# quadram-institute-bioscience/tatajuba

Hardware: AMD Instinct MI355X
Metric: reads/s (whole node), 150 bp synthetic FASTQ, homopolymer scan + context histogram (higher is better)
Workload: dtype u8/u64

## Files before the change

tatajuba_amd/csrc/hopo_device.hip:

```cpp

#include <hip/hip_runtime.h>
#include <rccl/rccl.h>
#include <dlfcn.h>
#include <mutex>
#include <string>
#include <new>
#include <stdint.h>
#include <stdio.h>
#include <stdlib.h>
#include <string.h>
#include <stdarg.h>
#include <limits.h>
#include <float.h>
#include <algorithm>
#include <vector>

#include "../../include/tatajuba_amd.h"
#include "../../include/tatajuba_variants.h"
#include "../../include/tatajuba_features.h"

typedef unsigned long long u64;
typedef unsigned int u32;


static thread_local char g_err[512] = "";

static int set_err (int code, const char *fmt, ...)
{
  va_list ap;
  va_start (ap, fmt);
  vsnprintf (g_err, sizeof (g_err), fmt, ap);
  va_end (ap);
  return code;
}

#define HIPCHK(call) do { hipError_t e_ = (call); if (e_ != hipSuccess) \
  return set_err (TJAMD_ERR_HIP, "%s failed: %s (%s:%d)", #call, hipGetErrorString (e_), __FILE__, __LINE__); } while (0)
#define HIPCHK_NULL(call) do { hipError_t e_ = (call); if (e_ != hipSuccess) { \
  set_err (TJAMD_ERR_HIP, "%s failed: %s (%s:%d)", #call, hipGetErrorString (e_), __FILE__, __LINE__); return NULL; } } while (0)

extern "C" const char *tjamd_last_error (void) { return g_err; }
extern "C" void tj_set_last_error (const char *msg) { (void) set_err (TJAMD_ERR_ARG, "%s", msg ? msg : "error"); }

extern "C" int tjamd_device_count (void)
{
  int n = 0;
  if (hipGetDeviceCount (&n) != hipSuccess) return 0;
  return n;
}


#define TJ_HL      64
#define TJ_HR      192

template <int BLOCK, int TILE, int CANDDIV = 2>
struct TileLds
{
  static constexpr int WIN = TJ_HL + TILE + TJ_HR;
  static constexpr int NCHUNK = WIN / 16;
  static constexpr int MASKW = WIN / 32 + 4;
  static constexpr int CODEW = WIN / 16 + 4;
  static constexpr int MAXCAND = TILE / CANDDIV;
  static constexpr int NLOAD = (NCHUNK + BLOCK - 1) / BLOCK;
  static constexpr int NRAW = NCHUNK + NLOAD * (BLOCK / 64);
  u32 code[CODEW];
  u32 start[MASKW];
  u32 sent[MASKW];
  u32 inval[MASKW];
  unsigned short cand[MAXCAND];
  u32 ncand;
  u32 grp[2];
  u32 odd[2];
};

struct DevCounters
{
  u64 n_rec;
  u64 n_fix_unused;
  u64 n_undefined;
  u64 n_null;
  u32 overflow;
  u32 fix_overflow;
  u32 pad[2];
  struct { u64 n_fix; u32 work, n_slow, work_slow, ticket, pad[2]; } lc[2];
};

#define TJ_TILE_GROUP 16

struct FixEntry { long long pos; long long len; };

struct FinCounts { u32 n_seg, n_kept, n_ctx, n_idx; int coverage; u32 overflow, sort_fallback, pad; };
struct FinPlan { long n1; long t; int nbits, nbins, log2t, ok; u32 kept_overflow, cov_direct; long n1_exact; u32 ovf_exact, pad2; };



__device__ __forceinline__ u32 zero_bytes (u32 t)
{
  return ~(((t & 0x7F7F7F7Fu) + 0x7F7F7F7Fu) | t | 0x7F7F7F7Fu);
}

__device__ __forceinline__ u32 gather_bit7 (u32 z)
{
  return ((z >> 7) | (z >> 14) | (z >> 21) | (z >> 28)) & 0xFu;
}

__device__ __forceinline__ void classify_word (u32 x, u32 prev_byte, u32 &code8, u32 &start4, u32 &sent4, u32 &inval4)
{
  u32 a1 = x >> 1, a2 = x >> 2, a3 = x >> 3, a4 = x >> 4, a6 = x >> 6, a7 = x >> 7;
  u32 v = ~a7 & a6 & ~a3 & ((~a4 & x & ~(a2 & ~a1)) | (a4 & a2 & ~a1));
  v &= 0x01010101u;
  u32 c = (a1 ^ a2) & (v * 3u);
  code8 = (c | (c >> 6) | (c >> 12) | (c >> 18)) & 0xFFu;
  u32 iv = v ^ 0x01010101u;
  inval4 = (iv | (iv >> 7) | (iv >> 14) | (iv >> 21)) & 0xFu;
  sent4 = gather_bit7 (zero_bytes (x ^ 0x0A0A0A0Au));
  start4 = gather_bit7 (zero_bytes (x ^ ((x << 8) | prev_byte))) ^ 0xFu;
}

__device__ __forceinline__ void classify_word_fast (u32 x, u32 prev_word, bool hi, u32 &code8, u32 &start4, u32 &sent4, u32 &bad)
{
  const u32 wts = hi ? 0x80402010u : 0x08040201u;
  const u32 c = ((x >> 1) ^ (x >> 2)) & 0x03030303u;
  code8 = __builtin_amdgcn_udot4 (c, 0x40100401u, 0u, false);
  const u32 s = ~(x >> 6) & 0x01010101u;
  sent4 = __builtin_amdgcn_udot4 (s, wts, sent4, false);
  bad = x ^ __builtin_amdgcn_perm (0x0A0A0A0Au, 0x54474341u, c | (s << 2));
  const u32 d = x ^ __builtin_amdgcn_alignbit (x, prev_word, 24);
  const u32 nz = (((d & 0x7F7F7F7Fu) + 0x7F7F7F7Fu) | d) & 0x80808080u;
  start4 = __builtin_amdgcn_udot4 (nz, wts, start4, false);
}

__device__ __forceinline__ u32 wave_inclusive_scan (u32 x)
{
  x += (u32) __builtin_amdgcn_update_dpp (0, (int) x, 0x111, 0xF, 0xF, true);
  x += (u32) __builtin_amdgcn_update_dpp (0, (int) x, 0x112, 0xF, 0xF, true);
  x += (u32) __builtin_amdgcn_update_dpp (0, (int) x, 0x114, 0xF, 0xF, true);
  x += (u32) __builtin_amdgcn_update_dpp (0, (int) x, 0x118, 0xF, 0xF, true);
  x += (u32) __builtin_amdgcn_update_dpp (0, (int) x, 0x142, 0xA, 0xF, true);
  x += (u32) __builtin_amdgcn_update_dpp (0, (int) x, 0x143, 0xC, 0xF, true);
  return x;
}

__device__ __forceinline__ void lds_barrier ()
{
  asm volatile ("s_waitcnt lgkmcnt(0)\n\ts_barrier" ::: "memory");
}

typedef __attribute__((address_space(1))) const void *gptr_t;
typedef __attribute__((address_space(3))) void *lptr_t;
__device__ __forceinline__ void lds_add_issue (u32 lds_addr, u32 value_uniform, u32 &raw_out)
{
  u64 saved; u32 tmp;
  asm volatile ("s_mov_b64 %0, exec\n\ts_mov_b64 exec, 1\n\tv_mov_b32 %1, %4\n\tds_add_rtn_u32 %2, %3, %1\n\ts_mov_b64 exec, %0"
                : "=&s"(saved), "=&v"(tmp), "=&v"(raw_out) : "v"(lds_addr), "s"(value_uniform) : "memory");
}
__device__ __forceinline__ u32 lds_collect (u32 raw)
{
  asm volatile ("s_waitcnt lgkmcnt(0)" : "+v"(raw) :: "memory");
  return (u32) __builtin_amdgcn_readfirstlane ((int) raw);
}

__device__ __forceinline__ u64 bits64 (const u32 *a, int bitpos)
{
  int w = bitpos >> 5, sh = bitpos & 31;
  u32 x0 = a[w], x1 = a[w + 1], x2 = a[w + 2];
  u32 lo = __funnelshift_r (x0, x1, sh);
  u32 hi = __funnelshift_r (x1, x2, sh);
  return ((u64) hi << 32) | lo;
}

__device__ __forceinline__ u32 bits32 (const u32 *a, int bitpos)
{
  const int w = bitpos >> 5;
  return __builtin_amdgcn_alignbit (a[w + 1], a[w], (u32) bitpos & 31u);
}

__device__ __forceinline__ u32 revcomp_k32 (u32 x, int k)
{
  const u32 y = __brev (~x);
  u32 z;
  asm ("v_bfi_b32 %0, %1, %2, %3" : "=v"(z) : "s"(0x55555555u), "v"(y >> 1), "v"(y << 1));
  return z >> (32 - 2 * k);
}

__device__ __forceinline__ u64 kmask (int k) { return (k >= 32) ? ~0ull : ((1ull << (2 * k)) - 1ull); }

__device__ __forceinline__ u64 revcomp_k (u64 x, int k)
{
  const u64 y = __brevll (~x);
  const u32 lo = (u32) y, hi = (u32) (y >> 32);
  u32 zl, zh;
  asm ("v_bfi_b32 %0, %1, %2, %3" : "=v"(zl) : "s"(0x55555555u), "v"(lo >> 1), "v"(lo << 1));
  asm ("v_bfi_b32 %0, %1, %2, %3" : "=v"(zh) : "s"(0x55555555u), "v"(hi >> 1), "v"(hi << 1));
  return (((u64) zh << 32) | zl) >> (64 - 2 * k);
}

__device__ __forceinline__ u32 stream_byte (const uint8_t *seq, long n, long p)
{
  return (p >= 0 && p < n) ? (u32) seq[p] : (u32) '\n';
}

__device__ __forceinline__ bool byte_is_acgtu (u32 b)
{
  u32 l = b | 0x20u;
  return l == 'a' || l == 'c' || l == 'g' || l == 't' || l == 'u';
}

__device__ __forceinline__ u32 byte_code (u32 b) { return byte_is_acgtu (b) ? (((b >> 1) ^ (b >> 2)) & 3u) : 0u; }

__device__ __forceinline__ u64 spread_pairs (u32 x)
{
  u64 v = x;
  v = (v | (v << 16)) & 0x0000FFFF0000FFFFull;
  v = (v | (v << 8)) & 0x00FF00FF00FF00FFull;
  v = (v | (v << 4)) & 0x0F0F0F0F0F0F0F0Full;
  v = (v | (v << 2)) & 0x3333333333333333ull;
  v = (v | (v << 1)) & 0x5555555555555555ull;
  return v | (v << 1);
}

__device__ __forceinline__ void canonicalise (u64 left, u64 right, u32 linv, u32 rinv, u32 cb, int k,
                                              u64 &c0, u64 &c1, u32 &base, u32 &flag)
{
  if (cb < 2u) { c0 = left; c1 = right; base = cb; flag = 1u; }
  else {
    if (linv | rinv) { left |= spread_pairs (linv); right |= spread_pairs (rinv); }
    c0 = revcomp_k (right, k); c1 = revcomp_k (left, k); base = 3u - cb; flag = 2u;
  }
}

__device__ __forceinline__ u64 make_meta (u32 base, long len, u32 flag)
{
  return (u64) base | (((u64) len & 0x3FFull) << TJ_META_LEN_SHIFT) | TJ_META_RAW_CONST | ((u64) flag << TJ_META_FLAG_SHIFT);
}

__device__ bool flanks_from_stream (const uint8_t *seq, long n, long gs, long ge, int k, u64 &left, u64 &right, u32 &linv, u32 &rinv)
{
  left = right = 0; linv = rinv = 0;
  for (int i = 0; i < k; i++) {
    u32 bl = stream_byte (seq, n, gs - k + i), br = stream_byte (seq, n, ge + 1 + i);
    if (bl == '\n' || br == '\n') return false;
    left |= (u64) byte_code (bl) << (2 * i);
    right |= (u64) byte_code (br) << (2 * i);
    linv |= (byte_is_acgtu (bl) ? 0u : 1u) << i;
    rinv |= (byte_is_acgtu (br) ? 0u : 1u) << i;
// ... 1391 lines not shown
  static_assert (RR % 4 == 0, "bins are kept four to a register");
  const u32 tid = threadIdx.x, lane = tid & 63u;
  const u32 wave = (u32) __builtin_amdgcn_readfirstlane ((int) (tid >> 6));
  if (tid < TJ_P) L.hist[tid] = 0;
  u32 cur_j = TJ_EMPTY, cur_chunk = TJ_NOCHUNK;
  lds_barrier ();
  const u32 n_blocks = min (*LG.next, LG.n_blocks);
  u32 b = blockIdx.x;
  if (b >= n_blocks) return;
  u64 w[RR][W];
  u32 n = min (LG.count[b], RB), nn = 0;
  auto load_block = [&] (u32 blk, u32 cnt) {
    const u64 *__restrict__ src = LG.log + ((u64) blk << TJ_LOGB_SHIFT);
    const u32 w0 = tid & ~63u;
#pragma unroll
    for (u32 r = 0; r < RR; r++) {
#pragma unroll
      for (int j = 0; j < W; j++) w[r][j] = 0;
      if (w0 + r * PL_BLOCK < cnt) {
        if constexpr (W == 1) w[r][0] = (src + r * PL_BLOCK)[tid];
        else { const ulonglong2 v = reinterpret_cast<const ulonglong2 *> (src + 2u * r * PL_BLOCK)[tid]; w[r][0] = v.x; w[r][1] = v.y; }
      }
    }
  };
  auto bucket_of = [&] (const u64 *rec) -> u32 {
    if constexpr (W == 1) return bucket_of_rec1 ((u32) rec[0], (u32) (rec[0] >> 32));
    else { u64 c0, c1; u32 base, len10, flag; unpack_raw<W> (rec, k, c0, c1, base, len10, flag); return bucket_of_key (c0, c1, base, len10); }
  };
  load_block (b, n);
  while (true) {
    const u32 bn = b + gridDim.x;
    const bool more = bn < n_blocks;
    if (more) nn = min (LG.count[bn], RB);
    u32 tq = tid;
    asm volatile ("" : "+v"(tq));
    u32 pk[RR / 4];
#pragma unroll
    for (u32 r = 0; r < RR / 4; r++) pk[r] = 0;
    if (n) {
#pragma unroll
      for (u32 r = 0; r < RR; r++) {
        const u32 bin = bucket_of (w[r]);
        pk[r >> 2] |= bin << (8u * (r & 3u));
        if (tid + r * PL_BLOCK < n) atomicAdd (&L.hist[bin], 1u);
      }
      lds_barrier ();
      if (wave < TJ_P / 64) {
        const uint4 h4 = *reinterpret_cast<const uint4 *> (&L.hist[4 * lane]);
        const u32 tot = h4.x + h4.y + h4.z + h4.w;
        const u32 e0 = wave_inclusive_scan (tot) - tot;
        if ((lane >> 4) == wave) *reinterpret_cast<uint4 *> (&L.offs[4 * lane]) = make_uint4 (e0, e0 + h4.x, e0 + h4.x + h4.y, e0 + h4.x + h4.y + h4.z);
        const u32 cnt = L.hist[tid], off = L.offs[tid];
        u64 a1 = 0, a2 = 0;
        u32 thr = off + cnt;
        if (cnt) {
          const u32 p0 = atomicAdd (&BK.cursors[tid * TJ_CSTRIDE], cnt);
          const u32 ch = (u32) TJ_CH0 << BK.ch_shift;
          bucket_claim_ahead_range (BK, tid, p0, cnt, ctr);
          const u32 j0 = chunk_of_pos (BK, p0), j1 = chunk_of_pos (BK, p0 + cnt - 1);
          if (j0 != cur_j) { cur_j = j0; cur_chunk = bucket_chunk_id (BK, tid, j0, true, ctr); }
          if (cur_chunk != TJ_NOCHUNK) a1 = (u64) (size_t) (BK.pool + ((u64) cur_chunk * ch + (p0 - j0 * ch)) * W) - (8ull * W) * off;
          if (j1 != j0) {
            thr = off + ((j0 + 1u) * ch - p0);
            cur_j = j0 + 1u; cur_chunk = bucket_chunk_id (BK, tid, j0 + 1u, true, ctr);
            if (cur_chunk != TJ_NOCHUNK) a2 = (u64) (size_t) (BK.pool + ((u64) cur_chunk * ch) * W) - (8ull * W) * thr;
          }
        }
        reinterpret_cast<uint4 *> (L.gbase)[tid] = make_uint4 ((u32) a1, (u32) (a1 >> 32) | (thr << 16), (u32) a2, (u32) (a2 >> 32));
      }
      lds_barrier ();
      if (tid < TJ_P) L.hist[tid] = 0;
#pragma unroll
      for (u32 r = 0; r < RR; r++)
        if (tid + r * PL_BLOCK < n) {
          const u32 bin = (pk[r >> 2] >> (8u * (r & 3u))) & 255u;
          const u32 d = atomicAdd (&L.offs[bin], 1u);
#pragma unroll
          for (int j = 0; j < W; j++) L.rec[d * W + j] = w[r][j];
          L.bin[d] = (unsigned char) bin;
        }
      lds_barrier ();
      for (u32 r0 = 0; r0 < RR; r0 += 4) {
        if (r0 * PL_BLOCK >= n) break;
        u32 cb[4]; uint4 e[4]; u64 cw[4][W];
#pragma unroll
        for (u32 h = 0; h < 4; h++) cb[h] = L.bin[tq + (r0 + h) * PL_BLOCK];
#pragma unroll
        for (u32 h = 0; h < 4; h++) {
          e[h] = reinterpret_cast<const uint4 *> (L.gbase)[cb[h]];
#pragma unroll
          for (int j = 0; j < W; j++) cw[h][j] = L.rec[(tq + (r0 + h) * PL_BLOCK) * W + j];
        }
#pragma unroll
        for (u32 h = 0; h < 4; h++) {
          const u32 i = tq + (r0 + h) * PL_BLOCK;
          const u64 a = (i < (e[h].y >> 16)) ? (((u64) (e[h].y & 0xFFFFu) << 32) | e[h].x) : (((u64) e[h].w << 32) | e[h].z);
          if (i < n && a != 0ull) {
            typedef __attribute__((address_space(1))) u64 *gwords_t;
            gwords_t q = (gwords_t) (a + (u64) (8u * W * i));
#pragma unroll
            for (int j = 0; j < W; j++) q[j] = cw[h][j];
          }
        }
      }
      lds_barrier ();
    }
    if (!more) break;
    load_block (bn, nn);
    n = nn; b = bn;
  }
}

template <int W>
__global__ void nrun_fixup_bins_kernel (const uint8_t *__restrict__ seq, long n_bytes, int k, int mprime,
                                        Buckets BK, DevCounters *ctr, const FixEntry *fix, u32 fix_cap, int par)
{
  nrun_fixup_entries<W> (seq, n_bytes, k, mprime, BK, ctr, fix, fix_cap, par, blockIdx.x * (u64) blockDim.x + threadIdx.x, (u64) gridDim.x * blockDim.x);
}

template <int W>
__global__ void bin_elems_kernel (const u64 *__restrict__ elems5, long n, int k, Buckets BK, DevCounters *ctr)
{
  for (long i = blockIdx.x * (long) blockDim.x + threadIdx.x; i < n; i += (long) gridDim.x * blockDim.x) {
    const u64 m = elems5[5 * i + 2];
    bucket_insert_slow<W> (elems5[5 * i], elems5[5 * i + 1], (u32) (m & 3ull), (u32) ((m >> TJ_META_LEN_SHIFT) & 0x3FFull),
                           (u32) ((m >> TJ_META_FLAG_SHIFT) & 3ull), k, BK, ctr);
  }
}

template <int W>
__global__ void unpack_buckets_kernel (Buckets BK, int k, u64 *__restrict__ out, u64 cap, u64 *n_out)
{
  const u32 b = blockIdx.x;
  const u32 n = BK.cursors[b * TJ_CSTRIDE];
  for (u32 i = threadIdx.x; i < n; i += blockDim.x) {
    u64 c0, c1; u32 base, len10, flag;
    const u64 at = bucket_slot (BK, b, i, false, nullptr);
    if (at == ~0ull) continue;
    unpack_raw<W> (BK.pool + at * W, k, c0, c1, base, len10, flag);
    if (flag == 3u) continue;
    const u64 o = atomicAdd (n_out, 1ull);
    if (o < cap) { u64 *q = out + 3 * o; q[0] = c0; q[1] = c1; q[2] = make_meta (base, len10, flag); }
  }
}

__global__ void init_table_kernel (u32 *table, u32 maxj, u32 *pool_next)
{
  const u32 b = blockIdx.x * blockDim.x + threadIdx.x;
  if (b < TJ_P) table[(u64) b * maxj] = b;
  if (b == 0) *pool_next = TJ_P;
}

__global__ void clear_buckets_kernel (u32 *cursors, DevCounters *ctr, u32 *table, u32 maxj, int ch_shift, FinCounts *fin, u32 *bins, int nbins,
                                      DevCounters *snap_ctr, u32 *snap_cursors, FinPlan *plan, u32 *__restrict__ fine = nullptr, int fine_bits = 0)
{
  const u32 b = blockIdx.x;
  if (snap_ctr) {
    if (threadIdx.x == 0) {
      snap_cursors[b] = cursors[b * TJ_CSTRIDE];
      if (b == 0) {
        snap_cursors[TJ_P] = cursors[TJ_P * TJ_CSTRIDE];
        if (plan) { plan->n1_exact = (long) fin->n_kept; plan->ovf_exact = fin->overflow; }
      }
    }
    if (b == 0) for (u32 i = threadIdx.x; i < sizeof (DevCounters) / 4; i += blockDim.x) reinterpret_cast<u32 *> (snap_ctr)[i] = reinterpret_cast<const u32 *> (ctr)[i];
    __syncthreads ();
  }
  if (b == 0) for (u32 i = threadIdx.x; i < sizeof (DevCounters) / 4; i += blockDim.x) if (i != offsetof (DevCounters, n_undefined) / 4 && i != offsetof (DevCounters, n_undefined) / 4 + 1) reinterpret_cast<u32 *> (ctr)[i] = 0;
  if (table) {
    u32 used = maxj;
    if (ch_shift >= 0) used = min (maxj, ((cursors[b * TJ_CSTRIDE] / TJ_CH0) >> ch_shift) + 3u);
    for (u32 j = threadIdx.x; j < used; j += blockDim.x) table[(u64) b * maxj + j] = j ? TJ_EMPTY : b;
  }
  if (fine) {
    const int gid = (int) (b * blockDim.x + threadIdx.x), gsz = (int) (gridDim.x * blockDim.x);
    if (plan->ok) {
      const int shift = fine_bits - plan->nbits, run = 1 << shift, nb = plan->nbins;
      for (int i = gid; i < nb; i += gsz) {
        u32 sum = 0;
        if (shift >= 2) {
          uint4 *f4 = reinterpret_cast<uint4 *> (fine) + (size_t) i * (run >> 2);
          for (int j = 0; j < (run >> 2); j++) { const uint4 v = f4[j]; sum += v.x + v.y + v.z + v.w; }
          for (int j = 0; j < (run >> 2); j++) f4[j] = make_uint4 (0, 0, 0, 0);
        }
        else {
          for (int j = 0; j < run; j++) sum += fine[(i << shift) + j];
          for (int j = 0; j < run; j++) fine[(i << shift) + j] = 0;
        }
        bins[i] = sum;
      }
    }
    else for (int i = gid; i < (1 << fine_bits); i += gsz) fine[i] = 0;
  }
  else if (bins) for (int i = (int) (b * blockDim.x + threadIdx.x); i < nbins; i += (int) (gridDim.x * blockDim.x)) bins[i] = 0;
  __syncthreads ();
  if (threadIdx.x == 0) { cursors[b * TJ_CSTRIDE] = 0; if (b == 0) { cursors[TJ_P * TJ_CSTRIDE] = TJ_P; fin->n_kept = 0; fin->overflow = 0; fin->pad = 0; } }
}

__global__ void table_relayout_kernel (const u32 *__restrict__ old, u32 old_maxj, u32 *__restrict__ neu, u32 new_maxj)
{
  const u32 b = blockIdx.x;
  for (u32 j = threadIdx.x; j < old_maxj; j += blockDim.x) neu[(u64) b * new_maxj + j] = old[(u64) b * old_maxj + j];
}


#define AG_BLOCK    1024
#define AG_NCH      512

#define AG1_S        8192
#define AG1_CLOSE_AT 4864
#define AG1_R        4
#define AG1_MARK     (~0ull)

#define BS_MAXBITS   16
__host__ __device__ static inline int cov_table_bits (long n1) { int b = 10; while ((1l << b) < 4 * n1 && b < 31) b++; return b; }
__host__ __device__ static inline int cov_plan_bits (long n1, int k, int *direct)
{
  const int hb = cov_table_bits (n1), kb = 2 * k < 31 ? 2 * k : 31;
  *direct = kb <= hb ? 1 : 0;
  return kb <= hb ? kb : hb;
}
__host__ __device__ static inline int fine_bin_bits (int k) { return BS_MAXBITS < 1 + 4 * k ? BS_MAXBITS : 1 + 4 * k; }
__device__ __forceinline__ u32 bin_of_record (u64 c0, u64 c1, u64 meta, int k, int nbits);
__host__ __device__ static inline int bin_bits_for (long n1, int k)
{
  int nbits = 6;
  while (nbits < BS_MAXBITS && nbits < 1 + 4 * k && (48l << nbits) < n1) nbits++;
  return nbits < 1 + 4 * k ? nbits : 1 + 4 * k;
}
__device__ __forceinline__ void flag_kept_overflow (FinCounts *fin)
{
  u32 old = atomicOr (&fin->overflow, 1u);
  asm volatile ("" :: "v"(old));
}

__device__ __forceinline__ void plan_tail (FinCounts *fin, int k, long cap, FinPlan *plan)
{
  if (!plan) return;
  __syncthreads ();
  if (threadIdx.x == 0) {
    const u32 done = atomicAdd (&fin->pad, 1u);
    if (done == gridDim.x - 1u) {
      const long n1 = (long) __hip_atomic_load (&fin->n_kept, __ATOMIC_RELAXED, __HIP_MEMORY_SCOPE_AGENT);
      const u32 ovf = __hip_atomic_load (&fin->overflow, __ATOMIC_RELAXED, __HIP_MEMORY_SCOPE_AGENT);
      plan->n1 = n1; plan->kept_overflow = ovf;
      plan->nbits = bin_bits_for (n1, k); plan->nbins = 1 << plan->nbits;
      int direct;
      plan->log2t = cov_plan_bits (n1, k, &direct); plan->t = 1l << plan->log2t; plan->cov_direct = (u32) direct;
      plan->ok = (n1 > 0 && n1 <= cap && !ovf) ? 1 : 0;
      fin->pad = 0;
    }
  }
}

__device__ __forceinline__ u32 batch_start (u32 t, u32 n, u32 batch)
{
  const u32 nb = (n + batch - 1u) / batch;
  return t < nb ? (nb - 1u - t) * batch : n;
}

struct Agg1Lds
{
  u64 key[AG1_S];
  u32 cnt[2 * AG1_S];
  u32 chunk[AG_NCH];
  u32 n_claimed, n_ovf, total;
  u32 next_batch;
  u32 wsum[AG_BLOCK / 64];
};

__global__ __launch_bounds__ (AG_BLOCK)
void aggregate1_kernel (Buckets BK, u64 *ovf, int k, int remove_biased, u64 *__restrict__ kept, u64 kept_cap, FinCounts *fin,
                        long plan_cap, FinPlan *plan, u32 *__restrict__ fine, int fine_bits)
{
  __shared__ Agg1Lds L;
  const int tid = threadIdx.x, lane = tid & 63, wave = tid >> 6;
  const u32 bkt = blockIdx.x;
  u32 n = BK.cursors[bkt * TJ_CSTRIDE];
  if (n) for (u32 j = (u32) tid; j <= chunk_of_pos (BK, n - 1u) && j < AG_NCH; j += AG_BLOCK) L.chunk[j] = bucket_chunk_id (BK, bkt, j, false, nullptr);
  auto chunk_id = [&] (u32 j) { return j < AG_NCH ? L.chunk[j] : bucket_chunk_id (BK, bkt, j, false, nullptr); };

  const u64 *src = BK.pool;
  u64 *dst = ovf;
  while (n > 0) {
    for (int i = tid; i < AG1_S; i += AG_BLOCK) { L.key[i] = 0; L.cnt[2 * i] = 0; L.cnt[2 * i + 1] = 0; }
    if (tid == 0) { L.n_claimed = 0; L.n_ovf = 0; L.next_batch = 0; }
    __syncthreads ();

    u64 wn[AG1_R];
    u32 vn = 0;
    auto fetch = [&] (u32 b0) {
      vn = 0;
#pragma unroll
      for (int r = 0; r < AG1_R; r++) wn[r] = 0;
      if (b0 >= n) return;
      const u32 ch = (u32) TJ_CH0 << BK.ch_shift;
      const u32 j0 = chunk_of_pos (BK, b0), bound = (j0 + 1u) * ch;
      if (b0 + 64u * AG1_R <= min (n, bound) && j0 < AG_NCH) {
        const u32 c0s = (u32) __builtin_amdgcn_readfirstlane ((int) L.chunk[j0]);
        if (c0s != TJ_NOCHUNK) {
          const u64 *q = src + ((u64) c0s * ch + (b0 - j0 * ch)) + (u32) lane;
#pragma unroll
          for (int r = 0; r < AG1_R; r++) wn[r] = q[64 * r];
          vn = (1u << AG1_R) - 1u;
          return;
        }
      }
      const u32 c0 = chunk_id (j0), c1 = (bound < n) ? chunk_id (j0 + 1u) : TJ_NOCHUNK;
      const u64 off0 = (u64) c0 * ch - (u64) j0 * ch, off1 = (u64) c1 * ch - (u64) bound;
#pragma unroll
      for (int r = 0; r < AG1_R; r++) {
        const u32 idx = b0 + (u32) r * 64u + (u32) lane;
        const bool hi = idx >= bound;
        if (idx < n && (hi ? c1 : c0) != TJ_NOCHUNK) { vn |= 1u << r; wn[r] = src[(hi ? off1 : off0) + idx]; }
      }
    };
    auto next_batch = [&] () {
      u32 b = 0;
      if (lane == 0) b = atomicAdd (&L.next_batch, 1u);
      return batch_start ((u32) __builtin_amdgcn_readfirstlane ((int) b), n, 64u * AG1_R);
    };
    u32 b_next = next_batch ();
    fetch (b_next);
    while (b_next < n) {
      const u32 b0 = b_next;
      (void) b0;
      asm volatile ("s_waitcnt vmcnt(0)" : "+v"(wn[0]), "+v"(wn[1]), "+v"(wn[2]), "+v"(wn[3]) :: "memory");
      static_assert (AG1_R == 4, "asm operand list");
      u64 w[AG1_R];
#pragma unroll
      for (int r = 0; r < AG1_R; r++) w[r] = wn[r];
      const u32 valid = vn;
      b_next = next_batch ();
      fetch (b_next);
      {
        auto home = [] (u64 key) {
          u32 h = (u32) key ^ __builtin_amdgcn_alignbit ((u32) (key >> 32), (u32) (key >> 32), 17);
          h *= 0x9E3779B1u; h ^= h >> 15;
          return h & (AG1_S / 2 - 1);
        };
        u32 todo = 0;
        u32 hp[AG1_R];
        ulonglong2 hk[AG1_R];
#pragma unroll
        for (int r = 0; r < AG1_R; r++) {
          hp[r] = home (w[r] & R1_KEY_MASK);
          hk[r] = *reinterpret_cast<const ulonglong2 *> (&L.key[2 * hp[r]]);
        }
        asm volatile ("" : "+v"(hk[0].x), "+v"(hk[0].y), "+v"(hk[1].x), "+v"(hk[1].y), "+v"(hk[2].x), "+v"(hk[2].y), "+v"(hk[3].x), "+v"(hk[3].y));
#pragma unroll
        for (int r = 0; r < AG1_R; r++) {
          const u64 cur = w[r];
          if (((valid >> r) & 1u) && ((cur >> R1_FLAG_SHIFT) & 3ull) != 3ull) {
            const u64 key = cur & R1_KEY_MASK;
            const bool hx = hk[r].x == key, hy = hk[r].y == key;
            if (hx | hy) atomicAdd (&L.cnt[4 * hp[r] + (hx ? 0u : 2u) + ((u32) (cur >> (R1_FLAG_SHIFT + 1)) & 1u)], 1u);
            else todo |= 1u << r;
          }
        }
        u32 probes = 0;
        u32 r = todo ? (u32) __ffs ((int) todo) - 1u : 0u;
        u64 cur = (r == 0u) ? w[0] : (r == 1u) ? w[1] : (r == 2u) ? w[2] : w[3];
        u32 pair = home (cur & R1_KEY_MASK);
        while (todo) {
          bool adv = false, left = false;
          {
            const u64 key = cur & R1_KEY_MASK;
            const u32 strand = (u32) (cur >> (R1_FLAG_SHIFT + 1)) & 1u;
            const ulonglong2 kk = *reinterpret_cast<const ulonglong2 *> (&L.key[2 * pair]);
            if (kk.x == key || kk.y == key) { atomicAdd (&L.cnt[4 * pair + (kk.x == key ? 0u : 2u) + strand], 1u); adv = true; }
            else {
              const bool e0 = (kk.x == 0ull) | (kk.x == AG1_MARK), e1 = (kk.y == 0ull) | (kk.y == AG1_MARK);
              if (e0 | e1) {
                const u32 slot = 2 * pair + (e0 ? 0u : 1u);
                if ((e0 ? kk.x : kk.y) == AG1_MARK) { left = true; adv = true; }
                else {
                  const bool closed = __hip_atomic_load (&L.n_claimed, __ATOMIC_RELAXED, __HIP_MEMORY_SCOPE_WORKGROUP) > AG1_CLOSE_AT;
                  const u64 old = atomicCAS ((unsigned long long *) &L.key[slot], 0ull, closed ? AG1_MARK : (unsigned long long) key);
                  if (old == 0ull) {
                    if (closed) left = true;
                    else { atomicAdd (&L.n_claimed, 1u); atomicAdd (&L.cnt[2 * slot + strand], 1u); }
                    adv = true;
                  }
                }
              }
              else if (++probes >= AG1_S / 2) { left = true; adv = true; }
              else pair = (pair + 1u) & (AG1_S / 2 - 1);
            }
          }
          if (left) {
            const u32 o = atomicAdd (&L.n_ovf, 1u);
            const u32 j = chunk_of_pos (BK, o), oc = chunk_id (j);
            if (oc != TJ_NOCHUNK) dst[(((u64) oc * TJ_CH0) << BK.ch_shift) + (o - ((j * TJ_CH0) << BK.ch_shift))] = cur;
          }
          if (adv) {
            todo &= todo - 1u; probes = 0;
            if (todo) {
              r = (u32) __ffs ((int) todo) - 1u;
              cur = (r == 1u) ? w[1] : (r == 2u) ? w[2] : w[3];
              pair = home (cur & R1_KEY_MASK);
            }
          }
        }
      }
    }
    __syncthreads ();

    u32 mine = 0;
    u64 metas[AG1_S / AG_BLOCK];
#pragma unroll
    for (int r = 0; r < AG1_S / AG_BLOCK; r++) {
      const int slot = tid + r * AG_BLOCK;
      metas[r] = 0;
      if (L.key[slot] && L.key[slot] != AG1_MARK) {
        const u32 cf = L.cnt[2 * slot], cr = L.cnt[2 * slot + 1];
        const u64 flag = (cf ? 1ull : 0ull) | (cr ? 2ull : 0ull);
        const u64 cnt = ((u64) cf + (u64) cr) & 0xFFFFFull;
        const int scnt = (cnt & 0x80000ull) ? (int) cnt - 0x100000 : (int) cnt;
        if (remove_biased ? (flag == 3ull) : (scnt > 1)) {
          const u64 key = L.key[slot];
          const u64 len10 = ((key >> 24) & 0xFFull) | (((key >> 56) & 3ull) << 8);
          metas[r] = ((key >> 58) & 1ull) | (len10 << TJ_META_LEN_SHIFT) | (cnt << TJ_META_COUNT_SHIFT) |
                     (0xffeull << TJ_META_MISM_SHIFT) | (flag << TJ_META_FLAG_SHIFT);
          mine++;
        }
      }
    }
    const u32 x = wave_inclusive_scan (mine);
    if (lane == 63) L.wsum[wave] = x;
    __syncthreads ();
    u32 wbase = 0, total = 0;
    for (int wv = 0; wv < AG_BLOCK / 64; wv++) { const u32 sm = L.wsum[wv]; if (wv < wave) wbase += sm; total += sm; }
    if (tid == 0) L.total = total ? atomicAdd (&fin->n_kept, total) : 0u;
    __syncthreads ();
    u64 at = (u64) L.total + wbase + x - mine;
#pragma unroll
    for (int r = 0; r < AG1_S / AG_BLOCK; r++)
      if (metas[r]) {
        const u64 key = L.key[tid + r * AG_BLOCK];
        if (at < kept_cap) {
          u64 *q = kept + 3 * at; q[0] = (key >> 32) & 0xFFFFFFull; q[1] = key & 0xFFFFFFull; q[2] = metas[r];
          if (fine) atomicAdd (&fine[bin_of_record ((key >> 32) & 0xFFFFFFull, key & 0xFFFFFFull, metas[r], k, fine_bits)], 1u);
        }
        else flag_kept_overflow (fin);
        at++;
      }
    __threadfence_block ();
    __syncthreads ();
    n = L.n_ovf;
    { const u64 *t = src; src = dst; dst = (u64 *) t; }
    __syncthreads ();
  }
  plan_tail (fin, k, plan_cap, plan);
}

#define AG2_S        6144
#define AG2_PAIRS    (AG2_S / 2)
#define AG2_CLOSE_AT 2560
#define AG2_R        4
#define AG2_VALID    (1ull << 63)
#define AG2_PENDING  (1ull << 63)
#define AG2_MARK     (1ull << 63)

struct Agg2Lds
{
  ulonglong2 kk[AG2_S];
  u32 cnt[2 * AG2_S];
  u32 chunk[AG_NCH];
  u32 n_claimed, n_ovf, total;
  u32 next_batch;
  u32 wsum[AG_BLOCK / 64];
};

__global__ __launch_bounds__ (AG_BLOCK)
void aggregate2_kernel (Buckets BK, u64 *ovf, int k, int remove_biased, u64 *__restrict__ kept, u64 kept_cap, FinCounts *fin,
                        long plan_cap, FinPlan *plan, u32 *__restrict__ fine, int fine_bits)
{
  __shared__ Agg2Lds L;
  const int tid = threadIdx.x, lane = tid & 63, wave = tid >> 6;
  const u32 bkt = blockIdx.x;
  u32 n = BK.cursors[bkt * TJ_CSTRIDE];
  const u64 m56 = (1ull << 56) - 1ull, fmask = ~(3ull << 61);
  if (n) for (u32 j = (u32) tid; j <= chunk_of_pos (BK, n - 1u) && j < AG_NCH; j += AG_BLOCK) L.chunk[j] = bucket_chunk_id (BK, bkt, j, false, nullptr);
  auto chunk_id = [&] (u32 j) { return j < AG_NCH ? L.chunk[j] : bucket_chunk_id (BK, bkt, j, false, nullptr); };
  const u64 *src = BK.pool;
  u64 *dst = ovf;

  while (n > 0) {
    for (int i = tid; i < AG2_S; i += AG_BLOCK) { L.kk[i] = make_ulonglong2 (0ull, 0ull); L.cnt[2 * i] = 0; L.cnt[2 * i + 1] = 0; }
    if (tid == 0) { L.n_claimed = 0; L.n_ovf = 0; L.next_batch = 0; }
    __syncthreads ();

    u64 wn[2 * AG2_R];
    u32 vn = 0;
    auto fetch = [&] (u32 b0) {
      vn = 0;
#pragma unroll
      for (int r = 0; r < 2 * AG2_R; r++) wn[r] = 0;
      if (b0 >= n) return;
      const u32 ch = (u32) TJ_CH0 << BK.ch_shift;
      const u32 j0 = chunk_of_pos (BK, b0), bound = (j0 + 1u) * ch;
      const u32 c0 = chunk_id (j0), c1 = (bound < n) ? chunk_id (j0 + 1u) : TJ_NOCHUNK;
      const u64 off0 = (u64) c0 * ch - (u64) j0 * ch, off1 = (u64) c1 * ch - (u64) bound;
#pragma unroll
      for (int r = 0; r < AG2_R; r++) {
        const u32 idx = b0 + (u32) r * 64u + (u32) lane;
        const bool hi = idx >= bound;
        if (idx < n && (hi ? c1 : c0) != TJ_NOCHUNK) {
          const ulonglong2 v = *reinterpret_cast<const ulonglong2 *> (src + 2 * ((hi ? off1 : off0) + idx));
          vn |= 1u << r; wn[2 * r] = v.x; wn[2 * r + 1] = v.y;
        }
      }
    };
    auto next_batch = [&] () {
      u32 b = 0;
      if (lane == 0) b = atomicAdd (&L.next_batch, 1u);
      return batch_start ((u32) __builtin_amdgcn_readfirstlane ((int) b), n, 64u * AG2_R);
    };
    u32 b_next = next_batch ();
    fetch (b_next);
    while (b_next < n) {
      asm volatile ("s_waitcnt vmcnt(0)" : "+v"(wn[0]), "+v"(wn[1]), "+v"(wn[2]), "+v"(wn[3]), "+v"(wn[4]), "+v"(wn[5]), "+v"(wn[6]), "+v"(wn[7]) :: "memory");
      static_assert (AG2_R == 4, "asm operand list");
      u64 w[2 * AG2_R];
#pragma unroll
      for (int r = 0; r < 2 * AG2_R; r++) w[r] = wn[r];
      const u32 valid = vn;
      b_next = next_batch ();
      fetch (b_next);
      {
        auto home = [] (u64 a, u64 b) {
          const u64 key1 = b & ~(3ull << 61);
          u32 h = (u32) a ^ __builtin_amdgcn_alignbit ((u32) (a >> 32), (u32) (a >> 32), 19) ^
                  __builtin_amdgcn_alignbit ((u32) key1, (u32) key1, 11) ^ __builtin_amdgcn_alignbit ((u32) (key1 >> 32), (u32) (key1 >> 32), 25);
          h *= 0x9E3779B1u; h ^= h >> 15;
          return __umulhi (h, (u32) AG2_PAIRS);
        };
        auto load_pair = [&] (u32 pair, ulonglong2 &s0, ulonglong2 &s1) {
          s0.x = __hip_atomic_load ((unsigned long long *) &L.kk[2 * pair].x, __ATOMIC_RELAXED, __HIP_MEMORY_SCOPE_WORKGROUP);
          s0.y = __hip_atomic_load ((unsigned long long *) &L.kk[2 * pair].y, __ATOMIC_RELAXED, __HIP_MEMORY_SCOPE_WORKGROUP);
          s1.x = __hip_atomic_load ((unsigned long long *) &L.kk[2 * pair + 1].x, __ATOMIC_RELAXED, __HIP_MEMORY_SCOPE_WORKGROUP);
          s1.y = __hip_atomic_load ((unsigned long long *) &L.kk[2 * pair + 1].y, __ATOMIC_RELAXED, __HIP_MEMORY_SCOPE_WORKGROUP);
        };
        u32 todo = 0, look = 0, cur[AG2_R];
#pragma unroll
        for (int q = 0; q < AG2_R; q++) {
          cur[q] = 0;
          if (((valid >> q) & 1u) && ((w[2 * q + 1] >> 61) & 3ull) != 3ull) { look |= 1u << q; cur[q] = home (w[2 * q], w[2 * q + 1]); }
        }
#pragma unroll
        for (int pass = 0; pass < 3; pass++) {
          if (pass && !look) break;
#pragma unroll
          for (int q = 0; q < AG2_R; q++)
            if ((look >> q) & 1u) {
              const u64 a0 = w[2 * q], a1 = w[2 * q + 1];
              ulonglong2 s0, s1;
              load_pair (cur[q], s0, s1);
              const u64 want = (a1 & fmask) | AG2_VALID;
              const bool m0 = (s0.x == a0) & (s0.y == want), m1 = (s1.x == a0) & (s1.y == want);
              if (m0 | m1) { atomicAdd (&L.cnt[2 * (2 * cur[q] + (m0 ? 0u : 1u)) + ((u32) (a1 >> 62) & 1u)], 1u); look &= ~(1u << q); }
              else {
                const u64 mine = a0 | AG2_PENDING;
                const bool o0 = (s0.x != 0ull) & (s0.x != AG2_MARK) & (s0.x != mine) & ((s0.x & AG2_PENDING) == 0ull) & ((s0.x != a0) | ((s0.y & AG2_VALID) != 0ull));
                const bool o1 = (s1.x != 0ull) & (s1.x != AG2_MARK) & (s1.x != mine) & ((s1.x & AG2_PENDING) == 0ull) & ((s1.x != a0) | ((s1.y & AG2_VALID) != 0ull));
                if (o0 & o1) cur[q] = (cur[q] + 1u == (u32) AG2_PAIRS) ? 0u : cur[q] + 1u;
                else { look &= ~(1u << q); todo |= 1u << q; }
              }
            }
        }
        todo |= look;
        u32 probes = 0;
        u32 r = todo ? (u32) __ffs ((int) todo) - 1u : 0u;
        u64 w0 = (r == 0u) ? w[0] : (r == 1u) ? w[2] : (r == 2u) ? w[4] : w[6];
        u64 w1 = (r == 0u) ? w[1] : (r == 1u) ? w[3] : (r == 2u) ? w[5] : w[7];
        u32 pair = (r == 0u) ? cur[0] : (r == 1u) ? cur[1] : (r == 2u) ? cur[2] : cur[3];
        while (todo) {
          bool adv = false, left = false;
          {
            const u64 key1 = w1 & fmask, want = key1 | AG2_VALID;
            const u32 strand = (u32) (w1 >> 62) & 1u;
            ulonglong2 s0, s1;
            load_pair (pair, s0, s1);
            const bool m0 = (s0.x == w0) & (s0.y == want), m1 = (s1.x == w0) & (s1.y == want);
            const bool again = (s0.x == (w0 | AG2_PENDING)) | (s1.x == (w0 | AG2_PENDING)) |
                               ((s0.x == w0) & !(s0.y & AG2_VALID)) | ((s1.x == w0) & !(s1.y & AG2_VALID));
            if (m0 | m1) { atomicAdd (&L.cnt[2 * (2 * pair + (m0 ? 0u : 1u)) + strand], 1u); adv = true; }
            else if (!again) {
              const bool e0 = (s0.x == 0ull) | (s0.x == AG2_MARK), e1 = (s1.x == 0ull) | (s1.x == AG2_MARK);
              if (e0 | e1) {
                const u32 slot = 2 * pair + (e0 ? 0u : 1u);
                if ((e0 ? s0.x : s1.x) == AG2_MARK) { left = true; adv = true; }
                else {
                  const bool closed = __hip_atomic_load (&L.n_claimed, __ATOMIC_RELAXED, __HIP_MEMORY_SCOPE_WORKGROUP) > AG2_CLOSE_AT;
                  const u64 old = atomicCAS ((unsigned long long *) &L.kk[slot].x, 0ull, closed ? AG2_MARK : (unsigned long long) (w0 | AG2_PENDING));
                  if (old == 0ull) {
                    if (closed) left = true;
                    else {
                      __hip_atomic_store ((unsigned long long *) &L.kk[slot].y, (unsigned long long) want, __ATOMIC_RELAXED, __HIP_MEMORY_SCOPE_WORKGROUP);
                      atomicAdd (&L.n_claimed, 1u);
                      __hip_atomic_store ((unsigned long long *) &L.kk[slot].x, (unsigned long long) w0, __ATOMIC_RELEASE, __HIP_MEMORY_SCOPE_WORKGROUP);
                      atomicAdd (&L.cnt[2 * slot + strand], 1u);
                    }
                    adv = true;
                  }
                }
              }
              else if (++probes >= AG2_PAIRS) { left = true; adv = true; }
              else pair = (pair + 1u == (u32) AG2_PAIRS) ? 0u : pair + 1u;
            }
          }
          if (left) {
            const u32 o = atomicAdd (&L.n_ovf, 1u);
            const u32 j = chunk_of_pos (BK, o), oc = chunk_id (j);
            if (oc != TJ_NOCHUNK) {
              const u64 at = (((u64) oc * TJ_CH0) << BK.ch_shift) + (o - ((j * TJ_CH0) << BK.ch_shift));
              dst[2 * at] = w0; dst[2 * at + 1] = w1;
            }
          }
          if (adv) {
            todo &= todo - 1u; probes = 0;
            if (todo) {
              r = (u32) __ffs ((int) todo) - 1u;
              w0 = (r == 1u) ? w[2] : (r == 2u) ? w[4] : w[6];
              w1 = (r == 1u) ? w[3] : (r == 2u) ? w[5] : w[7];
              pair = (r == 1u) ? cur[1] : (r == 2u) ? cur[2] : cur[3];
            }
          }
        }
      }
    }
    __syncthreads ();

    u32 mine = 0;
    u64 metas[AG2_S / AG_BLOCK];
#pragma unroll
    for (int r = 0; r < AG2_S / AG_BLOCK; r++) {
      const int slot = tid + r * AG_BLOCK;
      metas[r] = 0;
      if (L.kk[slot].x && L.kk[slot].x != AG2_MARK) {
        const u32 cf = L.cnt[2 * slot], cr = L.cnt[2 * slot + 1];
        const u64 flag = (cf ? 1ull : 0ull) | (cr ? 2ull : 0ull);
        const u64 cnt = ((u64) cf + (u64) cr) & 0xFFFFFull;
        const int scnt = (cnt & 0x80000ull) ? (int) cnt - 0x100000 : (int) cnt;
        if (remove_biased ? (flag == 3ull) : (scnt > 1)) {
          const u64 a = L.kk[slot].x, b = L.kk[slot].y;
          const u64 len10 = ((a >> 2) & 31ull) | (((b >> 56) & 31ull) << 5);
          metas[r] = ((a >> 1) & 1ull) | (len10 << TJ_META_LEN_SHIFT) | (cnt << TJ_META_COUNT_SHIFT) |
                     (0xffeull << TJ_META_MISM_SHIFT) | (flag << TJ_META_FLAG_SHIFT);
          mine++;
        }
      }
    }
    const u32 x = wave_inclusive_scan (mine);
    if (lane == 63) L.wsum[wave] = x;
    __syncthreads ();
    u32 wbase = 0, total = 0;
    for (int wv = 0; wv < AG_BLOCK / 64; wv++) { const u32 sm = L.wsum[wv]; if (wv < wave) wbase += sm; total += sm; }
    if (tid == 0) L.total = total ? atomicAdd (&fin->n_kept, total) : 0u;
    __syncthreads ();
    u64 at = (u64) L.total + wbase + x - mine;
#pragma unroll
    for (int r = 0; r < AG2_S / AG_BLOCK; r++)
      if (metas[r]) {
        const int slot = tid + r * AG_BLOCK;
        if (at < kept_cap) {
          u64 *q = kept + 3 * at; q[0] = (L.kk[slot].x >> 7) & m56; q[1] = L.kk[slot].y & m56; q[2] = metas[r];
          if (fine) atomicAdd (&fine[bin_of_record ((L.kk[slot].x >> 7) & m56, L.kk[slot].y & m56, metas[r], k, fine_bits)], 1u);
        }
        else flag_kept_overflow (fin);
        at++;
      }
    __threadfence_block ();
    __syncthreads ();
    n = L.n_ovf;
    { const u64 *t = src; src = dst; dst = (u64 *) t; }
    __syncthreads ();
  }
  plan_tail (fin, k, plan_cap, plan);
}

#define AG4_S        4096
#define AG4_CLOSE_AT 2560
#define AG4_R        2
#define AG4_PENDING  (1ull << 63)
#define AG4_MARK     (1ull << 63)

struct Agg4Lds
{
  u64 cw[AG4_S], c0[AG4_S], c1[AG4_S];
  u32 cnt[2 * AG4_S];
  u32 chunk[AG_NCH];
  u32 n_claimed, n_ovf, total;
  u32 next_batch;
  u32 wsum[AG_BLOCK / 64];
};

__global__ __launch_bounds__ (AG_BLOCK)
void aggregate4_kernel (Buckets BK, u64 *ovf, int k, int remove_biased, u64 *__restrict__ kept, u64 kept_cap, FinCounts *fin,
                        long plan_cap, FinPlan *plan, u32 *__restrict__ fine, int fine_bits)
{
  __shared__ Agg4Lds L;
  const int tid = threadIdx.x, lane = tid & 63, wave = tid >> 6;
  const u32 bkt = blockIdx.x;
  u32 n = BK.cursors[bkt * TJ_CSTRIDE];
  if (n) for (u32 j = (u32) tid; j <= chunk_of_pos (BK, n - 1u) && j < AG_NCH; j += AG_BLOCK) L.chunk[j] = bucket_chunk_id (BK, bkt, j, false, nullptr);
  auto chunk_id = [&] (u32 j) { return j < AG_NCH ? L.chunk[j] : bucket_chunk_id (BK, bkt, j, false, nullptr); };
  const u64 *src = BK.pool;
  u64 *dst = ovf;
  auto ld = [] (u64 *p) { return (u64) __hip_atomic_load ((unsigned long long *) p, __ATOMIC_RELAXED, __HIP_MEMORY_SCOPE_WORKGROUP); };

  while (n > 0) {
    for (int i = tid; i < AG4_S; i += AG_BLOCK) { L.cw[i] = 0; L.c0[i] = 0; L.c1[i] = 0; L.cnt[2 * i] = 0; L.cnt[2 * i + 1] = 0; }
    if (tid == 0) { L.n_claimed = 0; L.n_ovf = 0; L.next_batch = 0; }
    __syncthreads ();

    u64 wn[3 * AG4_R];
    u32 vn = 0;
    auto fetch = [&] (u32 b0) {
      vn = 0;
#pragma unroll
      for (int r = 0; r < 3 * AG4_R; r++) wn[r] = 0;
      if (b0 >= n) return;
      const u32 ch = (u32) TJ_CH0 << BK.ch_shift;
      const u32 j0 = chunk_of_pos (BK, b0), bound = (j0 + 1u) * ch;
      const u32 c0 = chunk_id (j0), c1 = (bound < n) ? chunk_id (j0 + 1u) : TJ_NOCHUNK;
      const u64 off0 = (u64) c0 * ch - (u64) j0 * ch, off1 = (u64) c1 * ch - (u64) bound;
#pragma unroll
      for (int r = 0; r < AG4_R; r++) {
        const u32 idx = b0 + (u32) r * 64u + (u32) lane;
        const bool hi = idx >= bound;
        if (idx < n && (hi ? c1 : c0) != TJ_NOCHUNK) {
          const u64 *p = src + 4 * ((hi ? off1 : off0) + idx);
          const ulonglong2 v = *reinterpret_cast<const ulonglong2 *> (p);
          vn |= 1u << r; wn[3 * r] = v.x; wn[3 * r + 1] = v.y; wn[3 * r + 2] = p[2];
        }
      }
    };
    auto next_batch = [&] () {
      u32 b = 0;
      if (lane == 0) b = atomicAdd (&L.next_batch, 1u);
      return batch_start ((u32) __builtin_amdgcn_readfirstlane ((int) b), n, 64u * AG4_R);
    };
    u32 b_next = next_batch ();
    fetch (b_next);
    while (b_next < n) {
      asm volatile ("s_waitcnt vmcnt(0)" : "+v"(wn[0]), "+v"(wn[1]), "+v"(wn[2]), "+v"(wn[3]), "+v"(wn[4]), "+v"(wn[5]) :: "memory");
      static_assert (AG4_R == 2, "asm operand list");
      u64 w[3 * AG4_R];
#pragma unroll
      for (int r = 0; r < 3 * AG4_R; r++) w[r] = wn[r];
      const u32 valid = vn;
      b_next = next_batch ();
      fetch (b_next);
      u32 todo = 0;
#pragma unroll
      for (int q = 0; q < AG4_R; q++) if (((valid >> q) & 1u) && ((w[3 * q + 2] >> 12) & 3ull) != 3ull) todo |= 1u << q;
      u32 probes = 0;
      while (todo) {
        const u32 r = (u32) __ffs ((int) todo) - 1u;
        const u64 c0 = r ? w[3] : w[0], c1 = r ? w[4] : w[1], m2 = r ? w[5] : w[2];
        const u32 k2 = (u32) m2 & 0xFFFu, strand = (u32) (m2 >> 13) & 1u;
        const u64 hk = hash_key (c0, c1, k2 & 3u, k2 >> 2);
        const u64 cw = 1ull | ((u64) k2 << 1) | ((hk >> 14) << 13);
        u32 slot = ((u32) hk + probes) & (AG4_S - 1);
        bool adv = false, left = false;
        const u64 a = ld (&L.cw[slot]);
        u64 x0 = ld (&L.c0[slot]), x1 = ld (&L.c1[slot]);
        if (a == cw) {
          bool eq = (x0 == c0) & (x1 == c1);
          if (!eq || (c0 | c1) == 0ull) { x0 = ld (&L.c0[slot]); x1 = ld (&L.c1[slot]); eq = (x0 == c0) & (x1 == c1); }
          if (eq) { atomicAdd (&L.cnt[2 * slot + strand], 1u); adv = true; }
          else if (++probes >= AG4_S) { left = true; adv = true; }
        }
        else if (a == AG4_MARK) { left = true; adv = true; }
        else if (a == 0ull) {
          const bool closed = __hip_atomic_load (&L.n_claimed, __ATOMIC_RELAXED, __HIP_MEMORY_SCOPE_WORKGROUP) > AG4_CLOSE_AT;
          const u64 old = atomicCAS ((unsigned long long *) &L.cw[slot], 0ull, closed ? AG4_MARK : (unsigned long long) (cw | AG4_PENDING));
          if (old == 0ull) {
            if (closed) left = true;
            else {
              __hip_atomic_store ((unsigned long long *) &L.c0[slot], (unsigned long long) c0, __ATOMIC_RELAXED, __HIP_MEMORY_SCOPE_WORKGROUP);
              __hip_atomic_store ((unsigned long long *) &L.c1[slot], (unsigned long long) c1, __ATOMIC_RELAXED, __HIP_MEMORY_SCOPE_WORKGROUP);
              atomicAdd (&L.n_claimed, 1u);
              __hip_atomic_store ((unsigned long long *) &L.cw[slot], (unsigned long long) cw, __ATOMIC_RELEASE, __HIP_MEMORY_SCOPE_WORKGROUP);
              atomicAdd (&L.cnt[2 * slot + strand], 1u);
            }
            adv = true;
          }
        }
        else if (a != (cw | AG4_PENDING)) {
          if (++probes >= AG4_S) { left = true; adv = true; }
        }
        if (left) {
          const u32 o = atomicAdd (&L.n_ovf, 1u);
          const u32 j = chunk_of_pos (BK, o), oc = chunk_id (j);
          if (oc != TJ_NOCHUNK) {
            u64 *q = dst + 4 * ((((u64) oc * TJ_CH0) << BK.ch_shift) + (o - ((j * TJ_CH0) << BK.ch_shift)));
            q[0] = c0; q[1] = c1; q[2] = m2; q[3] = 0;
          }
        }
        if (adv) { todo &= todo - 1u; probes = 0; }
      }
    }
    __syncthreads ();

    u32 mine = 0;
    u64 metas[AG4_S / AG_BLOCK];
#pragma unroll
    for (int r = 0; r < AG4_S / AG_BLOCK; r++) {
      const int slot = tid + r * AG_BLOCK;
      metas[r] = 0;
      const u64 cw = L.cw[slot];
      if (cw && cw != AG4_MARK) {
        const u32 cf = L.cnt[2 * slot], cr = L.cnt[2 * slot + 1];
        const u64 flag = (cf ? 1ull : 0ull) | (cr ? 2ull : 0ull);
        const u64 cnt = ((u64) cf + (u64) cr) & 0xFFFFFull;
        const int scnt = (cnt & 0x80000ull) ? (int) cnt - 0x100000 : (int) cnt;
        if (remove_biased ? (flag == 3ull) : (scnt > 1)) {
          const u32 k2 = (u32) (cw >> 1) & 0xFFFu;
          metas[r] = (u64) (k2 & 3u) | ((u64) (k2 >> 2) << TJ_META_LEN_SHIFT) | (cnt << TJ_META_COUNT_SHIFT) |
                     (0xffeull << TJ_META_MISM_SHIFT) | (flag << TJ_META_FLAG_SHIFT);
          mine++;
        }
      }
    }
    const u32 x = wave_inclusive_scan (mine);
    if (lane == 63) L.wsum[wave] = x;
    __syncthreads ();
    u32 wbase = 0, total = 0;
    for (int wv = 0; wv < AG_BLOCK / 64; wv++) { const u32 sm = L.wsum[wv]; if (wv < wave) wbase += sm; total += sm; }
    if (tid == 0) L.total = total ? atomicAdd (&fin->n_kept, total) : 0u;
    __syncthreads ();
    u64 at = (u64) L.total + wbase + x - mine;
#pragma unroll
    for (int r = 0; r < AG4_S / AG_BLOCK; r++)
      if (metas[r]) {
        const int slot = tid + r * AG_BLOCK;
        if (at < kept_cap) {
          u64 *q = kept + 3 * at; q[0] = L.c0[slot]; q[1] = L.c1[slot]; q[2] = metas[r];
          if (fine) atomicAdd (&fine[bin_of_record (L.c0[slot], L.c1[slot], metas[r], k, fine_bits)], 1u);
        }
        else flag_kept_overflow (fin);
        at++;
      }
    __threadfence_block ();
    __syncthreads ();
    n = L.n_ovf;
    { const u64 *t = src; src = dst; dst = (u64 *) t; }
    __syncthreads ();
  }
  plan_tail (fin, k, plan_cap, plan);
}


__device__ __forceinline__ u32 key_digit (u64 c0, u64 c1, u64 meta, int pass, int k)
{
  const int o = 8 * pass;
  const u32 v12 = (u32) ((((meta >> TJ_META_LEN_SHIFT) & 0x3FFull) ^ 0x200ull) << 2) | (u32) ((meta >> TJ_META_FLAG_SHIFT) & 3ull);
  const u64 base = meta & 1ull;
  u32 d = 0;
  int lo;
  lo = o;                      if (lo < 12)                       d |= (u32) (v12 >> lo);
  lo = o - 12;                 if (lo < 2 * k && lo > -8)         d |= (u32) (lo >= 0 ? (c1 >> lo) : (c1 << -lo));
  lo = o - 12 - 2 * k;         if (lo < 2 * k && lo > -8)         d |= (u32) (lo >= 0 ? (c0 >> lo) : (c0 << -lo));
  lo = o - 12 - 4 * k;         if (lo < 1 && lo > -8)             d |= (u32) (base << -lo);
  return (~d) & 0xFFu;
}

__host__ int key_passes (int k) { return (13 + 4 * k + 7) / 8; }

#define RS_ITEMS      1024
#define RS_WAVE_ITEMS 256

__device__ __forceinline__ u64 match_digit (u32 d, bool active)
{
  u64 peers = __ballot (active);
#pragma unroll
  for (int b = 0; b < 8; b++) {
    u64 bal = __ballot ((d >> b) & 1u);
    peers &= ((d >> b) & 1u) ? bal : ~bal;
  }
  return active ? peers : 0ull;
}

__global__ __launch_bounds__ (256)
void radix_count_kernel (const u64 *__restrict__ in, long n, int pass, int k, u32 *__restrict__ hist, int nblk)
{
  __shared__ u32 h[256];
  const int tid = threadIdx.x, lane = tid & 63;
  const u64 lt = (1ull << lane) - 1ull;
  h[tid] = 0;
  __syncthreads ();
  const long base = (long) blockIdx.x * RS_ITEMS;
  for (int i = tid; i < RS_ITEMS; i += 256) {
    long r = base + i;
    bool active = r < n;
    u32 d = 0;
    if (active) { const u64 *p = in + 3 * r; d = key_digit (p[0], p[1], p[2], pass, k); }
    u64 peers = match_digit (d, active);
    if (active && (peers & lt) == 0ull) atomicAdd (&h[d], (u32) __popcll (peers));
  }
  __syncthreads ();
  hist[(long) tid * nblk + blockIdx.x] = h[tid];
}

__global__ __launch_bounds__ (256)
void radix_scatter_kernel (const u64 *__restrict__ in, u64 *__restrict__ out, long n, int pass, int k,
                           const u32 *__restrict__ offs, int nblk)
{
  __shared__ u32 wcnt[4][256];
  const int tid = threadIdx.x, wave = tid >> 6, lane = tid & 63;
  for (int i = tid; i < 1024; i += 256) (&wcnt[0][0])[i] = 0;
  __syncthreads ();
  const long wbase = (long) blockIdx.x * RS_ITEMS + (long) wave * RS_WAVE_ITEMS;
  const u64 lt = (1ull << lane) - 1ull;

  for (int r = 0; r < RS_WAVE_ITEMS / 64; r++) {
    long idx = wbase + r * 64 + lane;
    bool active = idx < n;
    u32 d = 0;
    if (active) { const u64 *p = in + 3 * idx; d = key_digit (p[0], p[1], p[2], pass, k); }
    u64 peers = match_digit (d, active);
    if (active && (peers & lt) == 0ull) atomicAdd (&wcnt[wave][d], (u32) __popcll (peers));
  }
  __syncthreads ();
  {
    u32 run = offs[(long) tid * nblk + blockIdx.x];
    for (int w = 0; w < 4; w++) { u32 c = wcnt[w][tid]; wcnt[w][tid] = run; run += c; }
  }
  __syncthreads ();
  for (int r = 0; r < RS_WAVE_ITEMS / 64; r++) {
    long idx = wbase + r * 64 + lane;
    bool active = idx < n;
    u32 d = 0;
    u64 a = 0, b = 0, m = 0;
    if (active) { const u64 *p = in + 3 * idx; a = p[0]; b = p[1]; m = p[2]; d = key_digit (a, b, m, pass, k); }
    u64 peers = match_digit (d, active);
    int leader = active ? (__ffsll ((long long) peers) - 1) : 0;
    u32 old = 0;
    if (active && lane == leader) old = atomicAdd (&wcnt[wave][d], (u32) __popcll (peers));
    old = __shfl (old, leader);
    if (active) {
      u64 *q = out + 3 * ((u64) old + (u64) __popcll (peers & lt));
      q[0] = a; q[1] = b; q[2] = m;
    }
  }
}


#define BS_RANK_MAX  256

__device__ __forceinline__ u32 bin_of_record (u64 c0, u64 c1, u64 meta, int k, int nbits)
{
  const int kb = nbits - 1;
  const u64 v = (2 * k >= kb) ? (c0 >> (2 * k - kb)) : ((c0 << (kb - 2 * k)) | (c1 >> (4 * k - kb)));
  const u32 x = ((u32) (meta & 1ull) << kb) | (u32) v;
  return ((1u << nbits) - 1u) - x;
}

__device__ __forceinline__ bool record_before (u64 a0, u64 a1, u64 am, u32 ai, u64 b0, u64 b1, u64 bm, u32 bi)
{
  const u32 ab = (u32) am & 1u, bb = (u32) bm & 1u;
  if (ab != bb) return ab > bb;
  if (a0 != b0) return a0 > b0;
  if (a1 != b1) return a1 > b1;
  const u32 al = ((u32) (am >> TJ_META_LEN_SHIFT) & 0x3FFu) ^ 0x200u, bl = ((u32) (bm >> TJ_META_LEN_SHIFT) & 0x3FFu) ^ 0x200u;
  if (al != bl) return al > bl;
  return ai < bi;
}

__device__ __forceinline__ u32 bin_reserve (u32 *__restrict__ cursors, u32 bin, bool active, int grouped)
{
  if (!grouped) return active ? atomicAdd (&cursors[bin], 1u) : 0u;
  const int lane = threadIdx.x & 63;
  u64 todo = __ballot (active);
  u32 pos = 0;
  while (todo) {
    const int leader = __ffsll ((long long) todo) - 1;
    const u32 lb = (u32) __builtin_amdgcn_readlane ((int) bin, leader);
    const u64 grp = __ballot (active && bin == lb) & todo;
    u32 base = 0;
    if (lane == leader) base = atomicAdd (&cursors[lb], (u32) __popcll (grp));
    base = (u32) __builtin_amdgcn_readlane ((int) base, leader);
    if ((grp >> lane) & 1ull) pos = base + (u32) __popcll (grp & ((1ull << lane) - 1ull));
    todo &= ~grp;
  }
  return pos;
}

__global__ __launch_bounds__ (256)
void bin_count_kernel (const u64 *__restrict__ in, long n, int k, int nbits, u32 *__restrict__ bins, uint4 *__restrict__ cov, long cov_vec, int grouped,
                       const FinPlan *__restrict__ plan = nullptr)
{
  if (plan) { if (!plan->ok) return; n = plan->n1; nbits = plan->nbits; cov_vec = plan->t / 2; }
  for (long i = (long) blockIdx.x * 256 + threadIdx.x; i < cov_vec; i += (long) gridDim.x * 256) cov[i] = make_uint4 (0, 0, 0, 0);
  for (long i0 = (long) blockIdx.x * 256; i0 < n; i0 += (long) gridDim.x * 256) {
    const long i = i0 + threadIdx.x;
    u32 bin = 0;
    if (i < n) { const u64 *p = in + 3 * i; bin = bin_of_record (p[0], p[1], p[2], k, nbits); }
    (void) bin_reserve (bins, bin, i < n, grouped);
  }
}

#define BS_MAXBINS (1 << BS_MAXBITS)
#define WGS_CHUNK  16384

#define WGS_PAD(i) ((i) + ((i) >> 5))
struct WgScanLds { u32 a[WGS_CHUNK + WGS_CHUNK / 32 + 1]; u32 wsum[16]; u32 vmax; };

__device__ __forceinline__ u32 wg_exclusive_scan (const u32 *__restrict__ in, int n_all, u32 *__restrict__ out, u32 *__restrict__ out2, WgScanLds &L, u32 &vmax)
{
  const int tid = threadIdx.x, lane = tid & 63, wave = tid >> 6;
  if (tid == 0) L.vmax = 0;
  u32 carry = 0;
  for (int base = 0; base < n_all; base += WGS_CHUNK) {
    const int n = min (WGS_CHUNK, n_all - base);
    const int per = (n + 1023) / 1024;
    for (int i = tid; i < n; i += 1024) L.a[WGS_PAD (i)] = in[base + i];
    __syncthreads ();
    u32 sum = 0, mx = 0;
    for (int j = 0; j < per; j++) { const int b = tid * per + j; if (b < n) { const u32 v = L.a[WGS_PAD (b)]; sum += v; mx = max (mx, v); } }
    const u32 incl = wave_inclusive_scan (sum);
    if (lane == 63) L.wsum[wave] = incl;
    for (int o = 32; o > 0; o >>= 1) mx = max (mx, (u32) __shfl_down ((int) mx, o));
    if (lane == 0 && mx) atomicMax (&L.vmax, mx);
    __syncthreads ();
    u32 run = carry + incl - sum, total = 0;
    for (int w = 0; w < 16; w++) { const u32 x = L.wsum[w]; if (w < wave) run += x; total += x; }
    for (int j = 0; j < per; j++) { const int b = tid * per + j; if (b < n) { const u32 v = L.a[WGS_PAD (b)]; L.a[WGS_PAD (b)] = run; run += v; } }
    __syncthreads ();
    for (int i = tid; i < n; i += 1024) { const u32 v = L.a[WGS_PAD (i)]; out[base + i] = v; if (out2) out2[base + i] = v; }
    carry += total;
    __syncthreads ();
  }
  vmax = L.vmax;
  return carry;
}

__global__ __launch_bounds__ (1024)
void bin_scan_kernel (u32 *__restrict__ bins, int nbins, u32 *__restrict__ binstart, u32 rank_max, FinCounts *fin, const FinPlan *__restrict__ plan = nullptr)
{
  __shared__ WgScanLds L;
  u32 vmax;
  if (plan) { if (!plan->ok) return; nbins = plan->nbins; }
  const u32 total = wg_exclusive_scan (bins, nbins, binstart, bins, L, vmax);
  if (threadIdx.x == 0) { binstart[nbins] = total; fin->sort_fallback = vmax > rank_max ? 1u : 0u; }
}

__global__ __launch_bounds__ (256)
void bin_scatter_kernel (const u64 *__restrict__ in, u64 *__restrict__ out, long n, int k, int nbits, u32 *__restrict__ cursors,
                         const FinPlan *__restrict__ plan = nullptr, uint4 *__restrict__ cov = nullptr)
{
  if (plan) { if (!plan->ok) return; n = plan->n1; nbits = plan->nbits; }
  if (cov) for (long i = (long) blockIdx.x * 256 + threadIdx.x; i < plan->t / 2; i += (long) gridDim.x * 256) cov[i] = make_uint4 (0, 0, 0, 0);
  for (long i = (long) blockIdx.x * 256 + threadIdx.x; i < n; i += (long) gridDim.x * 256) {
    const u64 *p = in + 3 * i;
    const u64 a = p[0], b = p[1], m = p[2];
    u64 *q = out + 3 * (u64) atomicAdd (&cursors[bin_of_record (a, b, m, k, nbits)], 1u);
    q[0] = a; q[1] = b; q[2] = m;
  }
}


#define SC_ITEMS 4096

__device__ __forceinline__ u32 block_exclusive_scan_256 (u32 v, u32 *s_tmp, u32 &total)
{
  const int tid = threadIdx.x, lane = tid & 63, wave = tid >> 6;
  u32 x = v;
#pragma unroll
  for (int o = 1; o < 64; o <<= 1) { u32 y = __shfl_up (x, o); if (lane >= o) x += y; }
  if (lane == 63) s_tmp[wave] = x;
  __syncthreads ();
  u32 wbase = 0;
  for (int w = 0; w < wave; w++) wbase += s_tmp[w];
  total = s_tmp[0] + s_tmp[1] + s_tmp[2] + s_tmp[3];
  __syncthreads ();
  return wbase + x - v;
}

__global__ __launch_bounds__ (256)
void scan_reduce_kernel (const u32 *__restrict__ in, long n, u32 *__restrict__ bsum)
{
  __shared__ u32 s_tmp[4];
  const long base = (long) blockIdx.x * SC_ITEMS + (long) threadIdx.x * 16;
  u32 s = 0;
  for (int i = 0; i < 16; i++) if (base + i < n) s += in[base + i];
  u32 total;
  block_exclusive_scan_256 (s, s_tmp, total);
  if (threadIdx.x == 0) bsum[blockIdx.x] = total;
}

__global__ __launch_bounds__ (256)
void scan_apply_kernel (const u32 *__restrict__ in, u32 *__restrict__ out, long n, const u32 *__restrict__ boff, u32 *total_out)
{
  __shared__ u32 s_tmp[4];
  const long base = (long) blockIdx.x * SC_ITEMS + (long) threadIdx.x * 16;
  u32 v[16], s = 0;
  for (int i = 0; i < 16; i++) { v[i] = (base + i < n) ? in[base + i] : 0u; s += v[i]; }
  u32 total;
  u32 ex = block_exclusive_scan_256 (s, s_tmp, total) + (boff ? boff[blockIdx.x] : 0u);
  for (int i = 0; i < 16; i++) { if (base + i < n) out[base + i] = ex; ex += v[i]; }
  if (total_out && base <= n - 1 && n - 1 < base + 16) *total_out = ex;
}


__device__ __forceinline__ bool same_key (const u64 *a, const u64 *b)
{
  const u64 km = (3ull << TJ_META_BASE_SHIFT) | (0x3FFull << TJ_META_LEN_SHIFT);
  return a[0] == b[0] && a[1] == b[1] && ((a[2] ^ b[2]) & km) == 0ull;
}

__device__ __forceinline__ bool same_context (const u64 *a, const u64 *b)
{
  return a[0] == b[0] && a[1] == b[1] && ((a[2] ^ b[2]) & 3ull) == 0ull;
}

__device__ __forceinline__ int meta_count (u64 meta)
{
  int c = (int) ((meta >> TJ_META_COUNT_SHIFT) & 0xFFFFFull);
  return (c & 0x80000) ? c - 0x100000 : c;
}

__device__ __forceinline__ int meta_len (u64 meta)
{
  int l = (int) ((meta >> TJ_META_LEN_SHIFT) & 0x3FFull);
  return (l & 0x200) ? l - 0x400 : l;
}

__device__ __forceinline__ bool same_context_rows (const u64 *rec, long i, long j) { return same_context (rec + 3 * i, rec + 3 * j); }

__global__ void seg_heads_kernel (const u64 *__restrict__ rec, long n, u32 *__restrict__ flags, int context_only)
{
  for (long i = blockIdx.x * (long) blockDim.x + threadIdx.x; i < n; i += (long) gridDim.x * blockDim.x) {
    bool head = (i == 0);
    if (!head) head = context_only ? !same_context (rec + 3 * i, rec + 3 * (i - 1)) : !same_key (rec + 3 * i, rec + 3 * (i - 1));
    flags[i] = head ? 1u : 0u;
  }
}

__global__ void seg_headpos_kernel (const u32 *__restrict__ flags, const u32 *__restrict__ segid, long n, u32 *__restrict__ headpos)
{
  for (long i = blockIdx.x * (long) blockDim.x + threadIdx.x; i < n; i += (long) gridDim.x * blockDim.x)
    if (flags[i]) headpos[segid[i]] = (u32) i;
}

__global__ void ctx_decide_kernel (const u64 *__restrict__ kept, long n1, const u32 *__restrict__ ctxpos, const u32 *n_ctx_p,
                                   int min_coverage, u32 *__restrict__ keep)
{
  const u32 n_ctx = *n_ctx_p;
  for (u32 j = blockIdx.x * blockDim.x + threadIdx.x; j < n_ctx; j += gridDim.x * blockDim.x) {
    const long s = ctxpos[j], e = (j + 1 < n_ctx) ? (long) ctxpos[j + 1] : n1;
    int depth = 0;
    for (long i = s; i < e; i++) depth += meta_count (kept[3 * i + 2]);
    keep[j] = depth >= min_coverage;
  }
}

__global__ void ctx_write_kernel (long n1, const u32 *__restrict__ ctxpos, const u32 *n_ctx_p, const u32 *__restrict__ keep,
                                  const u32 *__restrict__ outpos, int *__restrict__ idx_initial, int *__restrict__ idx_final)
{
  const u32 n_ctx = *n_ctx_p;
  for (u32 j = blockIdx.x * blockDim.x + threadIdx.x; j < n_ctx; j += gridDim.x * blockDim.x)
    if (keep[j]) {
      idx_initial[outpos[j]] = (int) ctxpos[j];
      idx_final[outpos[j]] = (j + 1 < n_ctx) ? (int) ctxpos[j + 1] : (int) n1;
    }
}

__device__ __forceinline__ u64 cov_word (u32 key31, int w) { return ((u64) (key31 + 1u) << 32) | (u64) (u32) w; }

__device__ __forceinline__ void cov_direct_add (u32 key31, int w, u64 *__restrict__ tab)
{
  atomicAdd ((unsigned long long *) &tab[key31], (unsigned long long) (long long) w + (1ull << 33));
}

__device__ __forceinline__ void cov_add_from (u32 key31, u32 slot, int w, u64 *__restrict__ tab, int log2t)
{
  const u32 tmask = (1u << log2t) - 1u;
  for (u32 probe = 0; probe <= tmask; probe++) {
    const u64 old = atomicCAS ((unsigned long long *) &tab[slot], 0ull, (unsigned long long) cov_word (key31, w));
    if (old == 0ull) break;
    if ((u32) (old >> 32) == key31 + 1u) { atomicAdd (reinterpret_cast<u32 *> (&tab[slot]), (u32) w); break; }
    slot = (slot + 1u) & tmask;
  }
}

__device__ __forceinline__ void cov_add (u32 key31, int w, u64 *__restrict__ tab, int log2t)
{
  cov_add_from (key31, (key31 * 2654435761u) >> (32 - log2t), w, tab, log2t);
}

__device__ __forceinline__ void cov_add2 (u32 ka, u32 kb, int w, u64 *__restrict__ tab, int log2t)
{
  const u32 tmask = (1u << log2t) - 1u;
  const u32 pa = (ka * 2654435761u) >> (32 - log2t), pb = (kb * 2654435761u) >> (32 - log2t);
  const u64 oa = atomicCAS ((unsigned long long *) &tab[pa], 0ull, (unsigned long long) cov_word (ka, w));
  const u64 ob = atomicCAS ((unsigned long long *) &tab[pb], 0ull, (unsigned long long) cov_word (kb, w));
  if (oa != 0ull) {
    if ((u32) (oa >> 32) == ka + 1u) atomicAdd (reinterpret_cast<u32 *> (&tab[pa]), (u32) w);
    else cov_add_from (ka, (pa + 1u) & tmask, w, tab, log2t);
  }
  if (ob != 0ull) {
    if ((u32) (ob >> 32) == kb + 1u) atomicAdd (reinterpret_cast<u32 *> (&tab[pb]), (u32) w);
    else cov_add_from (kb, (pb + 1u) & tmask, w, tab, log2t);
  }
}

__device__ __forceinline__ void cov_add2_issue (u32 ka, u32 kb, int w, u64 *__restrict__ tab, int log2t, u64 &oa, u64 &ob)
{
  const u32 pa = (ka * 2654435761u) >> (32 - log2t), pb = (kb * 2654435761u) >> (32 - log2t);
  oa = atomicCAS ((unsigned long long *) &tab[pa], 0ull, (unsigned long long) cov_word (ka, w));
  ob = atomicCAS ((unsigned long long *) &tab[pb], 0ull, (unsigned long long) cov_word (kb, w));
}
__device__ __forceinline__ void cov_add2_finish (u32 ka, u32 kb, int w, u64 *__restrict__ tab, int log2t, u64 oa, u64 ob)
{
  const u32 tmask = (1u << log2t) - 1u;
  const u32 pa = (ka * 2654435761u) >> (32 - log2t), pb = (kb * 2654435761u) >> (32 - log2t);
  if (oa != 0ull) {
    if ((u32) (oa >> 32) == ka + 1u) atomicAdd (reinterpret_cast<u32 *> (&tab[pa]), (u32) w);
    else cov_add_from (ka, (pa + 1u) & tmask, w, tab, log2t);
  }
  if (ob != 0ull) {
    if ((u32) (ob >> 32) == kb + 1u) atomicAdd (reinterpret_cast<u32 *> (&tab[pb]), (u32) w);
    else cov_add_from (kb, (pb + 1u) & tmask, w, tab, log2t);
  }
}

__global__ void cov_insert_kernel (const u64 *__restrict__ kept, long n1, u64 *__restrict__ tab, int log2t)
{
  for (long i = blockIdx.x * (long) blockDim.x + threadIdx.x; i < 2 * n1; i += (long) gridDim.x * blockDim.x) {
    const long r = (i < n1) ? i : i - n1;
    cov_add ((u32) (kept[3 * r + (i < n1 ? 0 : 1)] & 0x7FFFFFFFull), meta_count (kept[3 * r + 2]), tab, log2t);
  }
}

__device__ __forceinline__ void cov_max_part (const u64 *__restrict__ tab, long t, int *result, int *s_best)
{
  int best = INT_MIN;
  for (long i = blockIdx.x * (long) blockDim.x + threadIdx.x; i < t; i += (long) gridDim.x * blockDim.x) {
    const u64 v = tab[i];
    if (v >> 32) best = max (best, (int) (u32) v);
  }
  for (int o = 32; o > 0; o >>= 1) best = max (best, __shfl_down (best, o));
  if ((threadIdx.x & 63) == 0) s_best[threadIdx.x >> 6] = best;
  __syncthreads ();
  if (threadIdx.x == 0) {
    for (int w = 1; w < (int) blockDim.x / 64; w++) best = max (best, s_best[w]);
    if (best != INT_MIN) atomicMax (result, best);
  }
}

__global__ __launch_bounds__ (256)
void cov_max_kernel (const u64 *__restrict__ tab, long t, int *result)
{
  __shared__ int s_best[4];
  cov_max_part (tab, t, result, s_best);
}

#define BSI_WAVES 1

template <int J>
__device__ __forceinline__ u32 lane_xor (u32 v, int lane)
{
  if constexpr (J == 1) return (u32) __builtin_amdgcn_update_dpp (0, (int) v, 0xB1, 0xF, 0xF, false);
  else if constexpr (J == 2) return (u32) __builtin_amdgcn_update_dpp (0, (int) v, 0x4E, 0xF, 0xF, false);
  else if constexpr (J == 4 || J == 8) {
    const u32 up = (u32) __builtin_amdgcn_update_dpp (0, (int) v, 0x100 + J, 0xF, 0xF, false);
    const u32 dn = (u32) __builtin_amdgcn_update_dpp (0, (int) v, 0x110 + J, 0xF, 0xF, false);
    return (lane & J) ? dn : up;
  }
  else if constexpr (J == 16) { const auto r = __builtin_amdgcn_permlane16_swap (v, v, false, false); return (lane & 16) ? r[0] : r[1]; }
  else { const auto r = __builtin_amdgcn_permlane32_swap (v, v, false, false); return (lane & 32) ? r[0] : r[1]; }
}

__global__ __launch_bounds__ (64 * BSI_WAVES)
void bin_sort_index_kernel (const u64 *__restrict__ in, u64 *__restrict__ out, const u32 *__restrict__ binstart, int nbins, const FinCounts *fin,
                            int min_coverage, u64 *__restrict__ cov_tab, int log2t,
                            u32 *__restrict__ binctx, u32 *__restrict__ tstart, u32 *__restrict__ tend, const FinPlan *__restrict__ plan = nullptr,
                            int cov_direct = 0)
{
  __shared__ alignas (16) u32 hd[BSI_WAVES][BS_RANK_MAX];
  __shared__ u32 sz[BSI_WAVES][BS_RANK_MAX];
  const int lane = threadIdx.x & 63, wave = threadIdx.x >> 6;
  const int bin0 = (int) blockIdx.x * BSI_WAVES + wave;
  u32 st0 = 0, en0 = 0;
  if (bin0 < nbins) { st0 = binstart[bin0]; en0 = binstart[bin0 + 1]; }
  if (plan) { if (!plan->ok) return; nbins = plan->nbins; log2t = plan->log2t; cov_direct = (int) plan->cov_direct; }
  if (fin->sort_fallback) return;
  u32 *H = hd[wave], *E = sz[wave];
  for (int bin = bin0; bin < nbins; bin += gridDim.x * BSI_WAVES) {
    const u32 st = (bin == bin0) ? st0 : binstart[bin], s = ((bin == bin0) ? en0 : binstart[bin + 1]) - st;
    if (s == 0) { if (lane == 0) binctx[bin] = 0; continue; }
    const u64 *R = in + 3 * (u64) st;
    u32 nkeep = 0;
    if (s <= 64u) {
      const bool valid = (u32) lane < s;
      u64 a0 = 0, a1 = 0, am = 0;
      if (valid) { a0 = R[3 * lane]; a1 = R[3 * lane + 1]; am = R[3 * lane + 2]; }
      const int w = meta_count (am);
      u64 cas_a = 0, cas_b = 0;
      if (!cov_direct && valid) cov_add2_issue ((u32) (a0 & 0x7FFFFFFFull), (u32) (a1 & 0x7FFFFFFFull), w, cov_tab, log2t, cas_a, cas_b);
      u32 kh = valid ? 2u | ((u32) am & 1u) : 0u;
      u32 kl = ((((u32) (am >> TJ_META_LEN_SHIFT) & 0x3FFu) ^ 0x200u) << 6) | (63u - (u32) lane);
      u32 x0 = (u32) a0, x1 = (u32) (a0 >> 32), y0 = (u32) a1, y1 = (u32) (a1 >> 32), m0 = (u32) am, m1 = (u32) (am >> 32);
      auto step = [&] (auto jc, int kk) {
        constexpr int J = decltype (jc)::value;
        const u32 ox0 = lane_xor<J> (x0, lane), ox1 = lane_xor<J> (x1, lane), oy0 = lane_xor<J> (y0, lane), oy1 = lane_xor<J> (y1, lane);
        const u32 om0 = lane_xor<J> (m0, lane), om1 = lane_xor<J> (m1, lane), okh = lane_xor<J> (kh, lane), okl = lane_xor<J> (kl, lane);
        const u64 mx = ((u64) x1 << 32) | x0, my = ((u64) y1 << 32) | y0, ox = ((u64) ox1 << 32) | ox0, oy = ((u64) oy1 << 32) | oy0;
        const bool mine_first = (kh > okh) | ((kh == okh) & ((mx > ox) | ((mx == ox) & ((my > oy) | ((my == oy) & (kl > okl))))));
        const bool want_first = ((lane & kk) == 0) == ((lane & J) == 0);
        const bool take = mine_first != want_first;
        x0 = take ? ox0 : x0; x1 = take ? ox1 : x1; y0 = take ? oy0 : y0; y1 = take ? oy1 : y1;
        m0 = take ? om0 : m0; m1 = take ? om1 : m1; kh = take ? okh : kh; kl = take ? okl : kl;
      };
#pragma unroll
      for (int kk = 2; kk <= 64; kk <<= 1) {
        if (kk >= 64) step (std::integral_constant<int, 32> (), kk);
        if (kk >= 32) step (std::integral_constant<int, 16> (), kk);
        if (kk >= 16) step (std::integral_constant<int, 8> (), kk);
        if (kk >= 8) step (std::integral_constant<int, 4> (), kk);
        if (kk >= 4) step (std::integral_constant<int, 2> (), kk);
        step (std::integral_constant<int, 1> (), kk);
      }
      const bool have = kh >= 2u;
      const u64 b0 = ((u64) x1 << 32) | x0, b1 = ((u64) y1 << 32) | y0, bm = ((u64) m1 << 32) | m0;
      if (have) { u64 *q = out + 3 * ((u64) st + (u32) lane); q[0] = b0; q[1] = b1; q[2] = bm; }
      const u32 px0 = (u32) __builtin_amdgcn_update_dpp (0, (int) x0, 0x138, 0xF, 0xF, false), px1 = (u32) __builtin_amdgcn_update_dpp (0, (int) x1, 0x138, 0xF, 0xF, false);
      const u32 py0 = (u32) __builtin_amdgcn_update_dpp (0, (int) y0, 0x138, 0xF, 0xF, false), py1 = (u32) __builtin_amdgcn_update_dpp (0, (int) y1, 0x138, 0xF, 0xF, false);
      const u32 pkh = (u32) __builtin_amdgcn_update_dpp (0, (int) kh, 0x138, 0xF, 0xF, false);
      const bool head = have & ((lane == 0) | (px0 != x0) | (px1 != x1) | (py0 != y0) | (py1 != y1) | (pkh != kh));
      const u64 heads = __ballot (head);
      const int cnt = have ? meta_count (bm) : 0;
      const u32 incl = wave_inclusive_scan ((u32) cnt);
      const u64 above = (lane == 63) ? 0ull : (heads >> (lane + 1));
      const u32 next_head = above ? (u32) lane + (u32) __ffsll ((long long) above) : s;
      const u32 last_incl = (u32) __builtin_amdgcn_ds_bpermute ((int) ((next_head - 1u) << 2), (int) incl);
      const int depth = (int) (last_incl - (incl - (u32) cnt));
      const bool keep = head & (depth >= min_coverage);
      const u64 keeps = __ballot (keep);
      if (keep) {
        const u32 o = (u32) __popcll (keeps & ((1ull << lane) - 1ull));
        tstart[st + o] = st + (u32) lane;
        tend[st + o] = st + next_head;
      }
      nkeep = (u32) __popcll (keeps);
      if (cov_direct) {
        if (head) { cov_direct_add ((u32) (b0 & 0x7FFFFFFFull), depth, cov_tab); cov_direct_add ((u32) (b1 & 0x7FFFFFFFull), depth, cov_tab); }
      }
      else if (valid) {
        asm volatile ("" : "+v"(cas_a), "+v"(cas_b));
        cov_add2_finish ((u32) (a0 & 0x7FFFFFFFull), (u32) (a1 & 0x7FFFFFFFull), w, cov_tab, log2t, cas_a, cas_b);
      }
      if (lane == 0) binctx[bin] = nkeep;
      asm volatile ("s_waitcnt lgkmcnt(0)" ::: "memory");
      __builtin_amdgcn_wave_barrier ();
      continue;
    }
    for (u32 t0 = 0; t0 < s; t0 += 64) {
      const u32 t = t0 + lane;
      bool keep = false;
      if (t < s) {
        const u64 a0 = R[3 * t], a1 = R[3 * t + 1], am = R[3 * t + 2];
        u32 rank = 0, ctx_before = 0, ctx_size = 0;
        int depth = 0;
        const u32 abase = (u32) am & 1u, alen = ((u32) (am >> TJ_META_LEN_SHIFT) & 0x3FFu) ^ 0x200u;
        for (u32 j0 = 0; j0 < s; j0 += 4) {
          u64 b0[4], b1[4], bm[4];
#pragma unroll
          for (int i = 0; i < 4; i++) {
            const u32 jj = (j0 + (u32) i < s) ? j0 + (u32) i : s - 1u;
            b0[i] = R[3 * jj]; b1[i] = R[3 * jj + 1]; bm[i] = R[3 * jj + 2];
          }
#pragma unroll
          for (int i = 0; i < 4; i++) {
            const u32 j = j0 + (u32) i;
            const bool live = j < s;
            const u32 bbase = (u32) bm[i] & 1u, blen = ((u32) (bm[i] >> TJ_META_LEN_SHIFT) & 0x3FFu) ^ 0x200u;
            const bool e0 = b0[i] == a0, e1 = b1[i] == a1, eb = bbase == abase;
            const bool before = live & ((bbase > abase) | (eb & ((b0[i] > a0) | (e0 & ((b1[i] > a1) | (e1 & ((blen > alen) | ((blen == alen) & (j < t)))))))));
            const bool same = live & e0 & e1 & (((u32) (bm[i] ^ am) & 3u) == 0u);
            rank += before ? 1u : 0u;
            ctx_size += same ? 1u : 0u;
            depth += same ? meta_count (bm[i]) : 0;
            ctx_before += (same & before) ? 1u : 0u;
          }
        }
        u64 *q = out + 3 * ((u64) st + rank);
        q[0] = a0; q[1] = a1; q[2] = am;
        keep = (ctx_before == 0u) && depth >= min_coverage;
        H[t] = rank | (keep ? 0x80000000u : 0u);
        E[t] = ctx_size;
        if (ctx_before == 0u) {
          if (cov_direct) { cov_direct_add ((u32) (a0 & 0x7FFFFFFFull), depth, cov_tab); cov_direct_add ((u32) (a1 & 0x7FFFFFFFull), depth, cov_tab); }
          else cov_add2 ((u32) (a0 & 0x7FFFFFFFull), (u32) (a1 & 0x7FFFFFFFull), depth, cov_tab, log2t);
        }
      }
      nkeep += (u32) __popcll (__ballot (keep));
    }
    asm volatile ("s_waitcnt lgkmcnt(0)" ::: "memory");
    __builtin_amdgcn_wave_barrier ();
    for (u32 t = lane; t < s; t += 64) {
      const u32 h = H[t];
      if (h & 0x80000000u) {
        const u32 rank = h & 0x7FFFFFFFu;
        u32 o = 0;
        for (u32 j = 0; j < s; j += 4) {
          const uint4 g = *reinterpret_cast<const uint4 *> (&H[j]);
          o += ((g.x & 0x80000000u) && (g.x & 0x7FFFFFFFu) < rank) ? 1u : 0u;
          o += (j + 1u < s && (g.y & 0x80000000u) && (g.y & 0x7FFFFFFFu) < rank) ? 1u : 0u;
          o += (j + 2u < s && (g.z & 0x80000000u) && (g.z & 0x7FFFFFFFu) < rank) ? 1u : 0u;
          o += (j + 3u < s && (g.w & 0x80000000u) && (g.w & 0x7FFFFFFFu) < rank) ? 1u : 0u;
        }
        tstart[st + o] = st + rank;
        tend[st + o] = st + rank + E[t];
      }
    }
    if (lane == 0) binctx[bin] = nkeep;
    asm volatile ("s_waitcnt lgkmcnt(0)" ::: "memory");
    __builtin_amdgcn_wave_barrier ();
  }
}

__global__ __launch_bounds__ (1024)
void bin_ctx_scan_kernel (const u32 *__restrict__ binctx, int nbins, u32 *__restrict__ binout, FinCounts *fin, const FinPlan *__restrict__ plan = nullptr)
{
  __shared__ WgScanLds L;
  u32 vmax;
  if (plan) { if (!plan->ok) return; nbins = plan->nbins; }
  const u32 total = wg_exclusive_scan (binctx, nbins, binout, nullptr, L, vmax);
  if (threadIdx.x == 0 && !fin->sort_fallback) { fin->n_idx = total; fin->coverage = INT_MIN; }
}

__global__ __launch_bounds__ (256)
void bin_ctx_write_kernel (const u32 *__restrict__ binstart, const u32 *__restrict__ binctx, const u32 *__restrict__ binout, int nbins,
                           const u32 *__restrict__ tstart, const u32 *__restrict__ tend, int *__restrict__ idx_initial, int *__restrict__ idx_final,
                           const u64 *__restrict__ cov_tab, long t, FinCounts *fin, const FinPlan *__restrict__ plan = nullptr)
{
  __shared__ int s_best[4];
  if (plan) { if (!plan->ok) return; nbins = plan->nbins; t = plan->t; }
  if (fin->sort_fallback) return;
  const int lane = threadIdx.x & 63, wave = threadIdx.x >> 6;
  for (int bin = blockIdx.x * 4 + wave; bin < nbins; bin += gridDim.x * 4) {
    const u32 cnt = binctx[bin], st = binstart[bin], o0 = binout[bin];
    for (u32 o = lane; o < cnt; o += 64) { idx_initial[o0 + o] = (int) tstart[st + o]; idx_final[o0 + o] = (int) tend[st + o]; }
  }
  cov_max_part (cov_tab, t, &fin->coverage, s_best);
}

#define MG_RANK_MAX 256
#define TJ_META_SAMPLE_SHIFT 52

__global__ __launch_bounds__ (256)
void merge_scatter_kernel (const u64 *__restrict__ in, u64 *__restrict__ out, long n, int k, int nbits, u32 *__restrict__ cursors,
                           const long *__restrict__ starts, int n_samples)
{
  for (long i0 = (long) blockIdx.x * 256; i0 < n; i0 += (long) gridDim.x * 256) {
    const long i = i0 + threadIdx.x;
    const bool active = i < n;
    u64 a = 0, b = 0, m = 0;
    int lo = 0;
    if (active) {
      int hi = n_samples;
      while (hi - lo > 1) { const int mid = (lo + hi) >> 1; if (starts[mid] <= i) lo = mid; else hi = mid; }
      const u64 *p = in + 3 * i;
      a = p[0]; b = p[1]; m = p[2];
    }
    const u32 pos = bin_reserve (cursors, active ? bin_of_record (a, b, m, k, nbits) : 0u, active, 1);
    if (active) {
      u64 *q = out + 3 * (u64) pos;
      q[0] = a; q[1] = b; q[2] = (m & ((1ull << TJ_META_SAMPLE_SHIFT) - 1ull)) | ((u64) lo << TJ_META_SAMPLE_SHIFT);
    }
  }
}

__device__ __forceinline__ bool merge_same_key (u64 a0, u64 a1, u64 am, u64 b0, u64 b1, u64 bm)
{
  const u64 km = (3ull << TJ_META_BASE_SHIFT) | (0x3FFull << TJ_META_LEN_SHIFT);
  return a0 == b0 && a1 == b1 && ((am ^ bm) & km) == 0ull;
}

__global__ __launch_bounds__ (64)
void bin_merge_kernel (const u64 *__restrict__ rec, const u32 *__restrict__ binstart, int nbins, const FinCounts *fin,
                       u32 *__restrict__ binctx, u32 *__restrict__ tpos, u32 *__restrict__ ttot)
{
  __shared__ u64 R[3 * MG_RANK_MAX];
  __shared__ alignas (16) u32 H[MG_RANK_MAX];
  if (fin->sort_fallback) return;
  const int lane = threadIdx.x;
  for (int bin = blockIdx.x; bin < nbins; bin += gridDim.x) {
    const u32 st = binstart[bin], s = binstart[bin + 1] - st;
    if (s == 0) { if (lane == 0) binctx[bin] = 0; continue; }
    for (u32 t = lane; t < s; t += 64) {
      const u64 *p = rec + 3 * (u64) (st + t);
      const u64 v0 = p[0], v1 = p[1], v2 = p[2];
      R[3 * t] = v0; R[3 * t + 1] = v1;
      R[3 * t + 2] = (v2 & ~(0x3FFull << TJ_META_LEN_SHIFT)) | ((((v2 >> TJ_META_LEN_SHIFT) & 0x3FFull) ^ 0x200ull) << TJ_META_LEN_SHIFT);
    }
    asm volatile ("s_waitcnt vmcnt(0) lgkmcnt(0)" ::: "memory");
    __builtin_amdgcn_wave_barrier ();
    const u64 lmask = 0x3FFull << TJ_META_LEN_SHIFT;
    u32 nrep = 0;
    for (u32 t0 = 0; t0 < s; t0 += 64) {
      const u32 t = t0 + lane;
      bool rep = false;
      if (t < s) {
        const u64 a0 = R[3 * t], a1 = R[3 * t + 1], al = R[3 * t + 2] & lmask;
        rep = true;
        u32 tot = 0, r = 0, fl = 0;
        for (u32 j0 = 0; j0 < s; j0 += 4) {
          u64 b0[4], b1[4], bm[4];
#pragma unroll
          for (int i = 0; i < 4; i++) {
            const u32 jj = (j0 + (u32) i < s) ? j0 + (u32) i : s - 1u;
            b0[i] = R[3 * jj]; b1[i] = R[3 * jj + 1]; bm[i] = R[3 * jj + 2];
          }
#pragma unroll
          for (int i = 0; i < 4; i++) {
            const u32 j = j0 + (u32) i;
            const bool live = j < s;
            const u64 bl = bm[i] & lmask;
            const bool same = live & (b0[i] == a0) & (b1[i] == a1) & (bl == al);
            const bool before = live & ((b0[i] > a0) | ((b0[i] == a0) & ((b1[i] > a1) | ((b1[i] == a1) & (bl > al)))));
            r += before ? 1u : 0u;
            rep = rep & !(same & (j < t));
            tot += same ? (u32) meta_count (bm[i]) : 0u;
            fl |= same ? (u32) (bm[i] >> TJ_META_FLAG_SHIFT) & 7u : 0u;
          }
        }
        H[t] = r | (rep ? 0x80000000u : 0u);
        ttot[st + t] = rep ? ((tot & 0xFFFFFu) | (fl << 28)) : 0xFFFFFFFFu;
      }
      nrep += (u32) __popcll (__ballot (rep));
    }
    asm volatile ("s_waitcnt lgkmcnt(0)" ::: "memory");
    __builtin_amdgcn_wave_barrier ();
    for (u32 t = lane; t < s; t += 64) {
      const u32 r = H[t] & 0x7FFFFFFFu;
      u32 d = 0;
      for (u32 j = 0; j < s; j += 4) {
        const uint4 h = *reinterpret_cast<const uint4 *> (&H[j]);
        d += ((h.x & 0x80000000u) && (h.x & 0x7FFFFFFFu) < r) ? 1u : 0u;
        d += (j + 1u < s && (h.y & 0x80000000u) && (h.y & 0x7FFFFFFFu) < r) ? 1u : 0u;
        d += (j + 2u < s && (h.z & 0x80000000u) && (h.z & 0x7FFFFFFFu) < r) ? 1u : 0u;
        d += (j + 3u < s && (h.w & 0x80000000u) && (h.w & 0x7FFFFFFFu) < r) ? 1u : 0u;
      }
      tpos[st + t] = d;
    }
    if (lane == 0) binctx[bin] = nrep;
    asm volatile ("s_waitcnt lgkmcnt(0)" ::: "memory");
    __builtin_amdgcn_wave_barrier ();
  }
}

__global__ __launch_bounds__ (256)
void bin_merge_write_kernel (const u64 *__restrict__ rec, const u32 *__restrict__ binstart, const u32 *__restrict__ binout, int nbins, const FinCounts *fin,
                             const u32 *__restrict__ tpos, const u32 *__restrict__ ttot, int n_samples,
                             u64 *__restrict__ keys, int *__restrict__ counts, long cap)
{
  if (fin->sort_fallback) return;
  const int lane = threadIdx.x & 63, wave = threadIdx.x >> 6;
  for (int bin = blockIdx.x * 4 + wave; bin < nbins; bin += gridDim.x * 4) {
    const u32 st = binstart[bin], s = binstart[bin + 1] - st, o0 = binout[bin];
    for (u32 t0 = 0; t0 < s; t0 += 64) {
      const u32 t = t0 + lane;
      if (t < s) {
        const long u = (long) o0 + tpos[st + t];
        if (u < cap) {
          const u64 a0 = rec[3 * (u64) (st + t)], a1 = rec[3 * (u64) (st + t) + 1], am = rec[3 * (u64) (st + t) + 2];
          const u32 tot = ttot[st + t];
          if (tot != 0xFFFFFFFFu) {
            for (int q = 0; q < n_samples; q++) counts[u * n_samples + q] = 0;
            u64 m = am & ((1ull << TJ_META_SAMPLE_SHIFT) - 1ull);
            m = (m & ~(0xFFFFFull << TJ_META_COUNT_SHIFT)) | (((u64) tot & 0xFFFFFull) << TJ_META_COUNT_SHIFT);
            m = (m & ~(7ull << TJ_META_FLAG_SHIFT)) | ((u64) ((tot >> 28) & 7u) << TJ_META_FLAG_SHIFT);
            keys[3 * u] = a0; keys[3 * u + 1] = a1; keys[3 * u + 2] = m;
          }
        }
      }
      __builtin_amdgcn_wave_barrier ();
      asm volatile ("s_waitcnt vmcnt(0)" ::: "memory");
      if (t < s) {
        const long u = (long) o0 + tpos[st + t];
        if (u < cap) {
          const u64 am = rec[3 * (u64) (st + t) + 2];
          counts[u * n_samples + (int) (am >> TJ_META_SAMPLE_SHIFT)] = meta_count (am);
        }
      }
    }
  }
}

__global__ void set_int_kernel (int *p, int v) { *p = v; }


__global__ void merge_tag_kernel (const u64 *__restrict__ in, u64 *__restrict__ out, long n, const long *__restrict__ starts, int n_samples)
{
  for (long i = blockIdx.x * (long) blockDim.x + threadIdx.x; i < n; i += (long) gridDim.x * blockDim.x) {
    int lo = 0, hi = n_samples;
    while (hi - lo > 1) { const int mid = (lo + hi) >> 1; if (starts[mid] <= i) lo = mid; else hi = mid; }
    out[3 * i] = in[3 * i]; out[3 * i + 1] = in[3 * i + 1];
    out[3 * i + 2] = (in[3 * i + 2] & ((1ull << TJ_META_SAMPLE_SHIFT) - 1ull)) | ((u64) lo << TJ_META_SAMPLE_SHIFT);
  }
}

__global__ void merge_write_kernel (const u64 *__restrict__ rec, long n, const u32 *__restrict__ flags, const u32 *__restrict__ segid,
                                    int n_samples, u64 *__restrict__ keys, int *__restrict__ counts, u32 *__restrict__ totals, u32 *__restrict__ orflags, long cap)
{
  for (long i = blockIdx.x * (long) blockDim.x + threadIdx.x; i < n; i += (long) gridDim.x * blockDim.x) {
    const u32 seg = segid[i] + flags[i] - 1u;
    if ((long) seg >= cap) continue;
    const u64 meta = rec[3 * i + 2];
    const int sample = (int) (meta >> TJ_META_SAMPLE_SHIFT);
    const int cnt = meta_count (meta);
    counts[(long) seg * n_samples + sample] = cnt;
    atomicAdd (&totals[seg], (u32) cnt);
    atomicOr (&orflags[seg], (u32) (meta >> TJ_META_FLAG_SHIFT) & 7u);
    if (flags[i]) { keys[3 * (long) seg] = rec[3 * i]; keys[3 * (long) seg + 1] = rec[3 * i + 1]; keys[3 * (long) seg + 2] = meta; }
  }
}

__global__ void merge_totals_kernel (u64 *__restrict__ keys, const u32 *__restrict__ totals, const u32 *__restrict__ orflags, const u32 *n_seg_p, long cap)
{
  const long n_seg = min ((long) *n_seg_p, cap);
  for (long j = blockIdx.x * (long) blockDim.x + threadIdx.x; j < n_seg; j += (long) gridDim.x * blockDim.x) {
    u64 m = keys[3 * j + 2] & ((1ull << TJ_META_SAMPLE_SHIFT) - 1ull);
    m = (m & ~(0xFFFFFull << TJ_META_COUNT_SHIFT)) | (((u64) totals[j] & 0xFFFFFull) << TJ_META_COUNT_SHIFT);
    m = (m & ~(7ull << TJ_META_FLAG_SHIFT)) | ((u64) (orflags[j] & 7u) << TJ_META_FLAG_SHIFT);
    keys[3 * j + 2] = m;
  }
}



struct DevBuf
{
  void *p = nullptr;
  size_t cap = 0;
};

#define TJ_SCAN_PIECE_TARGET (1ull << 30)

struct DevState { alignas (256) DevCounters ctr; alignas (256) FinCounts fin; alignas (256) u32 cursors[TJ_P + 1]; alignas (256) FinPlan plan;
                  alignas (256) DevCounters snap_ctr; alignas (256) u32 snap_cursors[TJ_P + 1]; alignas (256) u32 pad[4]; };

struct StageTimer
{
  hipEvent_t e0 = nullptr, e1 = nullptr;
  bool timed = false;
  hipError_t create () { const hipError_t e = hipEventCreate (&e0); return e != hipSuccess ? e : hipEventCreate (&e1); }
  void destroy () { if (e0) (void) hipEventDestroy (e0); if (e1) (void) hipEventDestroy (e1); }
  hipError_t begin (hipStream_t stream) { return hipEventRecord (e0, stream); }
  hipError_t end (hipStream_t stream) { return hipEventRecord (e1, stream); }
  bool elapsed (int device, float &ms) const
  { return timed && hipSetDevice (device) == hipSuccess && hipEventSynchronize (e1) == hipSuccess && hipEventElapsedTime (&ms, e0, e1) == hipSuccess; }
  double ms (int device) const { float f = 0.f; return elapsed (device, f) ? (double) f : -1.0; }
};
enum { T_SCAN, T_FIN, T_MERGE, T_TRACT, T_UNION, T_UNION_STATS, T_REF, T_LOCATE, T_LOCATED_TRACTS, T_VARIANTS, T_ANNOTATION, T_TRACT_FEATURES, TJ_N_TIMERS };

struct tjamd_counter
{
  int device = 0, k = 0, W = 4, n_cu = 256;
  hipStream_t own_stream = nullptr, stream = nullptr;
  DevCounters *d_ctr = nullptr, *h_ctr = nullptr;
  DevCounters *d_lctr = nullptr;
  u32 *d_cursors = nullptr, *h_cursors = nullptr;
  DevBuf pool, table, stage, fix, loc, prefix, rawlist, slow;
  DevBuf log, logmeta;
  int log_mode = 1;
  bool log_next_clean[2] = {false, false};
  hipEvent_t ev_p1 = nullptr;
#define TJ_PIECE_EVENTS 64
  hipEvent_t ev_pa[TJ_PIECE_EVENTS] = {}, ev_pb[TJ_PIECE_EVENTS] = {};
  int n_piece_ev = 0;
  StageTimer timer[TJ_N_TIMERS];
  DevBuf ts_cov, ts_aux;
  long union_cand = -1;
  DevBuf ut_tot, ut_lev, ut_fb, ut_slots;
  DevBuf lc_work;
  bool part_timed = false;
  int fast_mode = 1;
  u32 pool_chunks = 0, maxj = 0;
  int ch_shift = -1;
  u64 bucket_bound = 0;
  u64 chunk_bound = 0;
  long n_raw_known = 0;
  u64 raw_bound = 0;
  long n_undefined = 0;
  double slack = 1.0;
  DevBuf alt, hist, flags, segid, headpos, keep, outpos, scan_tmp, kept, idx_i, idx_f, cov, bins, binstart, binctx, ovf, grp_jt, grp_hist, fine;
  u32 bin_rank_max = BS_RANK_MAX;
  FinCounts *d_fin = nullptr, *h_fin = nullptr;
  struct DevState *d_state = nullptr, *h_state = nullptr;
  void *h_kept = nullptr; size_t h_kept_cap = 0;
  bool bins_zeroed = false;
  bool fine_dirty = false;
  bool bins_counted = false;
  long n_kept = 0; int n_idx = 0, coverage = 0, status = -1;
  hipEvent_t ev_done = nullptr;
  hipEvent_t ev_agg = nullptr;
  hipStream_t order_stream = nullptr;
  int fin_pending = 0;
  int fin_rb = 0, fin_mc = 0; bool fin_speculative = false, fin_plan_ahead = false; u64 fin_kept_cap = 0;
  hipEvent_t marks[8] = {nullptr, nullptr, nullptr, nullptr, nullptr, nullptr, nullptr, nullptr};
  unsigned mark_seq = 0;
  long last_scan_launches = 0;
  unsigned scan_seq = 0;
  size_t piece_target = TJ_SCAN_PIECE_TARGET;
  int scan_grid_cap = 0;
  bool buckets_clean = false;
  long plan_mismatches = 0;
  bool ctr_clean = false;
};

static int ensure (DevBuf &b, size_t bytes, hipStream_t stream, size_t keep_bytes = 0)
{
  if (bytes <= b.cap) return TJAMD_OK;
  size_t want = std::max (bytes, b.cap + b.cap / 2);
  void *np = nullptr;
  hipError_t e = hipMalloc (&np, want);
  if (e != hipSuccess && want > bytes) { want = bytes; e = hipMalloc (&np, want); }
  if (e != hipSuccess) return set_err (TJAMD_ERR_HIP, "hipMalloc of %zu bytes failed: %s", want, hipGetErrorString (e));
  if (b.p) {
    if (keep_bytes) HIPCHK (hipMemcpyAsync (np, b.p, keep_bytes, hipMemcpyDeviceToDevice, stream));
    HIPCHK (hipStreamSynchronize (stream));
    HIPCHK (hipFree (b.p));
  }
  b.p = np; b.cap = want;
  return TJAMD_OK;
}

static void release (DevBuf &b) { if (b.p) (void) hipFree (b.p); b.p = nullptr; b.cap = 0; }

extern "C" tjamd_counter *tjamd_counter_create (int device, int kmer_size)
{
  int n = tjamd_device_count ();
  if (n <= 0) { set_err (TJAMD_ERR_NO_DEVICE, "no HIP device visible: the homopolymer-tract engine needs an MI355X (no CPU fallback)"); return NULL; }
  if (device < 0 || device >= n) { set_err (TJAMD_ERR_ARG, "device %d out of range [0,%d)", device, n); return NULL; }
  if (kmer_size < 2 || kmer_size > 32) { set_err (TJAMD_ERR_ARG, "kmer_size %d outside [2,32] (reference clamp: src/main.c:184-185)", kmer_size); return NULL; }
  HIPCHK_NULL (hipSetDevice (device));
  tjamd_counter *c = new tjamd_counter ();
  c->device = device; c->k = kmer_size;
  c->W = (kmer_size <= 12) ? 1 : (kmer_size <= 28) ? 2 : 4;
  hipDeviceProp_t prop;
  HIPCHK_NULL (hipGetDeviceProperties (&prop, device));
  c->n_cu = prop.multiProcessorCount > 0 ? prop.multiProcessorCount : 256;
  const char *bm = getenv ("TATAJUBA_AMD_BIN_MAX");
  if (bm && atoi (bm) >= 1 && atoi (bm) <= BS_RANK_MAX) c->bin_rank_max = (u32) atoi (bm);
  const char *pc = getenv ("TATAJUBA_AMD_SCAN_PIECE");
  if (pc && atol (pc) >= 4096) c->piece_target = (size_t) atol (pc);
  const char *sk = getenv ("TATAJUBA_AMD_SINK");
  if (sk && !strcmp (sk, "fused")) c->log_mode = 0;
  if (sk && !strcmp (sk, "log")) c->log_mode = 2;
  const char *fm = getenv ("TATAJUBA_AMD_FAST");
  if (fm && atoi (fm) >= 0 && atoi (fm) <= 2) c->fast_mode = atoi (fm);
  const char *sg = getenv ("TATAJUBA_AMD_SCAN_GRID");
  if (sg && atoi (sg) >= 1) c->scan_grid_cap = atoi (sg);
  const char *sl = getenv ("TATAJUBA_AMD_BUCKET_SLACK");
  if (sl && atof (sl) >= 1.0) c->slack = atof (sl);
  HIPCHK_NULL (hipStreamCreateWithFlags (&c->own_stream, hipStreamNonBlocking));
  c->stream = c->own_stream;
  HIPCHK_NULL (hipMalloc ((void **) &c->d_state, sizeof (DevState)));
  HIPCHK_NULL (hipMalloc ((void **) &c->d_lctr, sizeof (DevCounters)));
  HIPCHK_NULL (hipHostMalloc ((void **) &c->h_state, sizeof (DevState), hipHostMallocDefault));
  c->d_ctr = &c->d_state->ctr; c->d_fin = &c->d_state->fin;
  HIPCHK_NULL (hipMalloc ((void **) &c->d_cursors, (size_t) (TJ_P + 1) * TJ_CSTRIDE * 4));
  HIPCHK_NULL (hipMemsetAsync (c->d_cursors, 0, (size_t) (TJ_P + 1) * TJ_CSTRIDE * 4, c->stream));
  c->h_ctr = &c->h_state->ctr; c->h_fin = &c->h_state->fin; c->h_cursors = c->h_state->cursors;
  memset (c->h_state, 0, sizeof (DevState));
  HIPCHK_NULL (hipMemsetAsync (c->d_state, 0, sizeof (DevState), c->stream));
  HIPCHK_NULL (hipMemsetAsync (c->d_lctr, 0, sizeof (DevCounters), c->stream));
  for (StageTimer &t : c->timer) HIPCHK_NULL (t.create ());
  HIPCHK_NULL (hipEventCreate (&c->ev_p1));
  HIPCHK_NULL (hipEventCreateWithFlags (&c->ev_done, hipEventDisableTiming));
  HIPCHK_NULL (hipEventCreateWithFlags (&c->ev_agg, hipEventDisableTiming));
  HIPCHK_NULL (hipStreamSynchronize (c->stream));
  return c;
}

extern "C" void tjamd_counter_destroy (tjamd_counter *c)
{
  if (!c) return;
  (void) hipSetDevice (c->device);
  (void) hipStreamSynchronize (c->stream);
  DevBuf *all[] = {&c->log, &c->logmeta, &c->pool, &c->table, &c->stage, &c->fix, &c->loc, &c->prefix, &c->rawlist, &c->slow, &c->alt, &c->hist, &c->flags, &c->segid, &c->headpos,
                   &c->keep, &c->outpos, &c->scan_tmp, &c->kept, &c->idx_i, &c->idx_f, &c->cov, &c->bins, &c->binstart, &c->binctx, &c->ovf, &c->grp_jt, &c->grp_hist, &c->fine,
                   &c->ts_cov, &c->ts_aux, &c->ut_tot, &c->ut_lev, &c->ut_fb, &c->ut_slots, &c->lc_work};
  for (DevBuf *b : all) release (*b);
  for (hipEvent_t ev : c->marks) if (ev) (void) hipEventDestroy (ev);
  if (c->d_state) (void) hipFree (c->d_state);
  if (c->d_lctr) (void) hipFree (c->d_lctr);
  if (c->d_cursors) (void) hipFree (c->d_cursors);
  if (c->h_state) (void) hipHostFree (c->h_state);
  if (c->h_kept) (void) hipHostFree (c->h_kept);
  for (StageTimer &t : c->timer) t.destroy ();
  if (c->ev_p1) (void) hipEventDestroy (c->ev_p1);
  for (int i = 0; i < TJ_PIECE_EVENTS; i++) { if (c->ev_pa[i]) (void) hipEventDestroy (c->ev_pa[i]); if (c->ev_pb[i]) (void) hipEventDestroy (c->ev_pb[i]); }
  if (c->ev_done) (void) hipEventDestroy (c->ev_done);
  if (c->ev_agg) (void) hipEventDestroy (c->ev_agg);
  if (c->own_stream) (void) hipStreamDestroy (c->own_stream);
  delete c;
}

extern "C" int tjamd_counter_device (const tjamd_counter *c) { return c ? c->device : -1; }

extern "C" int tjamd_counter_set_stream (tjamd_counter *c, void *hip_stream)
{
  if (!c) return set_err (TJAMD_ERR_ARG, "null counter");
  HIPCHK (hipSetDevice (c->device));
  HIPCHK (hipStreamSynchronize (c->stream));
  c->stream = hip_stream ? (hipStream_t) hip_stream : c->own_stream;
  return TJAMD_OK;
}

extern "C" int tjamd_counter_set_order_stream (tjamd_counter *c, void *hip_stream)
{
  if (!c) return set_err (TJAMD_ERR_ARG, "null counter");
  HIPCHK (hipSetDevice (c->device));
  HIPCHK (hipStreamSynchronize (c->stream));
  if (c->order_stream) HIPCHK (hipStreamSynchronize (c->order_stream));
  c->order_stream = (hipStream_t) hip_stream;
  return TJAMD_OK;
}

static Buckets make_buckets (const tjamd_counter *c)
{
  Buckets B;
  B.pool = (u64 *) c->pool.p; B.table = (u32 *) c->table.p; B.cursors = c->d_cursors; B.pool_next = c->d_cursors + TJ_P * TJ_CSTRIDE;
  B.pool_chunks = c->pool_chunks; B.maxj = c->maxj; B.ch_shift = (u32) std::max (c->ch_shift, 0);
  return B;
}

static int clear_buckets (tjamd_counter *c, bool snapshot = false)
{
  if (!c->buckets_clean || snapshot) {
    const bool fused = snapshot && c->fine_dirty && c->bins.p != nullptr;
    hipLaunchKernelGGL (clear_buckets_kernel, dim3 (TJ_P), dim3 (256), 0, c->stream, c->d_cursors, c->d_ctr,
                        (u32 *) (c->maxj ? c->table.p : nullptr), c->maxj, c->ch_shift, c->d_fin, (u32 *) c->bins.p, c->bins.p ? BS_MAXBINS : 0,
                        snapshot ? &c->d_state->snap_ctr : (DevCounters *) nullptr, snapshot ? c->d_state->snap_cursors : (u32 *) nullptr,
                        snapshot ? &c->d_state->plan : (FinPlan *) nullptr, fused ? (u32 *) c->fine.p : (u32 *) nullptr, fine_bin_bits (c->k));
    HIPCHK (hipGetLastError ());
    c->buckets_clean = true;
    c->ctr_clean = true;
    c->bins_zeroed = c->bins.p != nullptr && !fused;
    if (fused) { c->fine_dirty = false; c->bins_counted = true; }
  }
  c->n_raw_known = 0; c->raw_bound = 0; c->bucket_bound = 0; c->chunk_bound = TJ_P; c->ch_shift = -1;
  return TJAMD_OK;
}

extern "C" int tjamd_counter_reset (tjamd_counter *c)
{
  if (!c) return set_err (TJAMD_ERR_ARG, "null counter");
  HIPCHK (hipSetDevice (c->device));
  if (!(c->ctr_clean && c->fin_pending == 0 && c->n_undefined == 0)) HIPCHK (hipMemsetAsync (c->d_ctr, 0, sizeof (DevCounters), c->stream));
  int rc = clear_buckets (c);
  c->ctr_clean = true;
  if (rc) return rc;
  c->n_undefined = 0;
  c->n_kept = 0; c->n_idx = 0; c->coverage = 0; c->status = -1;
  return TJAMD_OK;
}

extern "C" void *tjamd_host_alloc (size_t bytes)
{
  void *p = nullptr;
  if (hipHostMalloc (&p, bytes, hipHostMallocPortable) != hipSuccess) { set_err (TJAMD_ERR_HIP, "hipHostMalloc of %zu bytes failed", bytes); return NULL; }
  return p;
}

extern "C" void tjamd_host_free (void *p) { if (p) (void) hipHostFree (p); }

extern "C" void *tjamd_device_alloc (tjamd_counter *c, size_t bytes)
{
  void *p = nullptr;
  if (!c || hipSetDevice (c->device) != hipSuccess || hipMalloc (&p, bytes ? bytes : 1) != hipSuccess) { set_err (TJAMD_ERR_HIP, "hipMalloc of %zu bytes failed", bytes); return NULL; }
  return p;
}
extern "C" void tjamd_device_free (tjamd_counter *c, void *p) { if (c && p && hipSetDevice (c->device) == hipSuccess) (void) hipFree (p); }
extern "C" int tjamd_device_download (tjamd_counter *c, void *host, const void *dev, size_t bytes)
{
  if (!c || (bytes && (!host || !dev))) return set_err (TJAMD_ERR_ARG, "bad arguments");
  HIPCHK (hipSetDevice (c->device));
  HIPCHK (hipStreamSynchronize (c->stream));
  if (bytes) HIPCHK (hipMemcpy (host, dev, bytes, hipMemcpyDeviceToHost));
  return TJAMD_OK;
}

extern "C" int tjamd_sync (tjamd_counter *c)
{
  if (!c) return set_err (TJAMD_ERR_ARG, "null counter");
  HIPCHK (hipSetDevice (c->device));
  HIPCHK (hipStreamSynchronize (c->stream));
  return TJAMD_OK;
}

extern "C" int tjamd_mark (tjamd_counter *c)
{
  if (!c) return -set_err (TJAMD_ERR_ARG, "null counter");
  if (hipSetDevice (c->device) != hipSuccess) return -set_err (TJAMD_ERR_HIP, "hipSetDevice failed");
  const int slot = (int) (c->mark_seq++ & 7u);
  if (!c->marks[slot] && hipEventCreateWithFlags (&c->marks[slot], hipEventDisableTiming) != hipSuccess) return -set_err (TJAMD_ERR_HIP, "hipEventCreate failed");
  if (hipEventRecord (c->marks[slot], c->stream) != hipSuccess) return -set_err (TJAMD_ERR_HIP, "hipEventRecord failed");
  return slot;
}

extern "C" int tjamd_wait_mark (tjamd_counter *c, int mark)
{
  if (!c || mark < 0 || mark > 7 || !c->marks[mark]) return set_err (TJAMD_ERR_ARG, "bad mark");
  HIPCHK (hipSetDevice (c->device));
  HIPCHK (hipEventSynchronize (c->marks[mark]));
  return TJAMD_OK;
}

__global__ void pack_cursors_kernel (const u32 *__restrict__ cursors, u32 *__restrict__ packed)
{
  if (threadIdx.x <= TJ_P) packed[threadIdx.x] = cursors[threadIdx.x * TJ_CSTRIDE];
}

static int queue_counter_copies (tjamd_counter *c)
{
  hipLaunchKernelGGL (pack_cursors_kernel, dim3 (1), dim3 (320), 0, c->stream, (const u32 *) c->d_cursors, c->d_state->cursors);
  HIPCHK (hipGetLastError ());
  HIPCHK (hipMemcpyAsync (c->h_state, c->d_state, sizeof (DevState), hipMemcpyDeviceToHost, c->stream));
  return TJAMD_OK;
}

static int apply_counter_copies (tjamd_counter *c, bool from_snapshot = false)
{
  long total = 0;
  u64 mx = 0;
  struct View { const DevCounters *h_ctr; const u32 *h_cursors; } v = {c->h_ctr, c->h_cursors};
  if (from_snapshot) { v.h_ctr = &c->h_state->snap_ctr; v.h_cursors = c->h_state->snap_cursors; }
  for (int b = 0; b < TJ_P; b++) { total += v.h_cursors[b]; mx = std::max<u64> (mx, v.h_cursors[b]); }
  if (v.h_ctr->overflow == 2u)
    return set_err (TJAMD_ERR_HIP, "a chunk of raw record storage was claimed but its id was never published (waited %u polls): "
                    "the claiming workgroup did not make progress -- please report; scanning again usually succeeds", (unsigned) TJ_SPIN_MAX);
  if (v.h_ctr->overflow)
    return set_err (TJAMD_ERR_CAPACITY, "raw record storage exhausted (%u of %u chunks handed out, fullest bucket %llu records): "
                    "raise TATAJUBA_AMD_BUCKET_SLACK (now %.1f) and scan again", v.h_cursors[TJ_P], c->pool_chunks, (unsigned long long) mx, c->slack);
  if (v.h_ctr->fix_overflow) return set_err (TJAMD_ERR_CAPACITY, "too many non-ACGTU tract candidates in one batch (%llu)",
                                             (unsigned long long) std::max (v.h_ctr->lc[0].n_fix, v.h_ctr->lc[1].n_fix));
  c->n_raw_known = total - (long) v.h_ctr->n_null;
  c->raw_bound = (u64) c->n_raw_known;
  c->bucket_bound = mx;
  c->chunk_bound = v.h_cursors[TJ_P];
  c->n_undefined = (long) v.h_ctr->n_undefined;
  return TJAMD_OK;
}

static int sync_counters (tjamd_counter *c)
{
  int rc = queue_counter_copies (c);
  if (rc) return rc;
  HIPCHK (hipStreamSynchronize (c->stream));
  return apply_counter_copies (c);
}

static void choose_chunk_size (tjamd_counter *c, u64 records)
{
  if (c->ch_shift >= 0) return;
  const u64 units = records / (16384ull * TJ_CH0);
  int sft = 3;
  static_assert ((TJ_CH0 << 3) > (int) TJ_LOGB, "a run of one log block crosses at most one chunk boundary");
  while ((1ull << sft) < units) sft++;
  c->ch_shift = sft;
}

static int ensure_table (tjamd_counter *c, u64 need_maxj)
{
  if (need_maxj > c->maxj) {
    const u32 nmaxj = (u32) std::max<u64> (need_maxj, (u64) c->maxj + c->maxj / 2);
    void *np = nullptr;
    hipError_t e = hipMalloc (&np, (size_t) TJ_P * nmaxj * 4);
    if (e != hipSuccess) return set_err (TJAMD_ERR_HIP, "hipMalloc of the chunk table failed: %s", hipGetErrorString (e));
    HIPCHK (hipMemsetAsync (np, 0xFF, (size_t) TJ_P * nmaxj * 4, c->stream));
    if (!c->table.p || !c->maxj) {
      hipLaunchKernelGGL (init_table_kernel, dim3 (1), dim3 (TJ_P), 0, c->stream, (u32 *) np, nmaxj, c->d_cursors + TJ_P * TJ_CSTRIDE);
      HIPCHK (hipGetLastError ());
    }
    if (c->table.p) {
      if (c->maxj) {
        hipLaunchKernelGGL (table_relayout_kernel, dim3 (TJ_P), dim3 (256), 0, c->stream, (const u32 *) c->table.p, c->maxj, (u32 *) np, nmaxj);
        HIPCHK (hipGetLastError ());
      }
      HIPCHK (hipStreamSynchronize (c->stream));
      HIPCHK (hipFree (c->table.p));
    }
    c->table.p = np; c->table.cap = (size_t) TJ_P * nmaxj * 4; c->maxj = nmaxj;
  }
  return TJAMD_OK;
}

// ... 104 lines not shown
      hipLaunchKernelGGL (scan_bins_kernel<WW>, dim3 (capped (grid)), dim3 (TJ_SB_BLOCK), 0, c->stream, seq, (long) n_bytes, n_tiles, c->k, mprime, BK, c->d_ctr, fix, (u32) TJ_FIX_CAP, par, plain); \
      hipLaunchKernelGGL (nrun_fixup_bins_kernel<WW>, dim3 (64), dim3 (256), 0, c->stream, seq, (long) n_bytes, c->k, mprime, BK, c->d_ctr, (const FixEntry *) fix, (u32) TJ_FIX_CAP, par); \
    } \
  } while (0)
  switch (c->W) {
    case 1: TJ_LAUNCH_SCAN (1); break;
    case 2: TJ_LAUNCH_SCAN (2); break;
    default: TJ_LAUNCH_SCAN (4); break;
  }
#undef TJ_LAUNCH_SCAN
  HIPCHK (hipGetLastError ());
  if (last) HIPCHK (c->timer[T_SCAN].end (c->stream));
  if (first) c->n_piece_ev = 0;
  const bool mid_events = use_log && !last && c->n_piece_ev < TJ_PIECE_EVENTS;
  if (mid_events) {
    const int i = c->n_piece_ev;
    if (!c->ev_pa[i]) { HIPCHK (hipEventCreate (&c->ev_pa[i])); HIPCHK (hipEventCreate (&c->ev_pb[i])); }
    HIPCHK (hipEventRecord (c->ev_pa[i], c->stream));
  }
  if (use_log) {
    if (c->W == 1) hipLaunchKernelGGL (partition_log_kernel<1>, dim3 (capped ((long) c->n_cu * PL_WG_PER_CU)), dim3 (PL_BLOCK), 0, c->stream, LG, BK, c->d_ctr, c->k);
    else hipLaunchKernelGGL (partition_log_kernel<2>, dim3 (capped ((long) c->n_cu * PL_WG_PER_CU)), dim3 (PL_BLOCK), 0, c->stream, LG, BK, c->d_ctr, c->k);
    HIPCHK (hipGetLastError ());
  }
  if (mid_events) { HIPCHK (hipEventRecord (c->ev_pb[c->n_piece_ev], c->stream)); c->n_piece_ev++; }
  if (last) { HIPCHK (hipEventRecord (c->ev_p1, c->stream)); c->part_timed = use_log; }
  c->timer[T_SCAN].timed = true;
  c->last_scan_launches = first ? 1 : c->last_scan_launches + 1;
  c->status = -1;
  return TJAMD_OK;
}


__global__ __launch_bounds__ (1024)
void find_cut_kernel (const uint8_t *__restrict__ seq, unsigned long long first_from, unsigned long long step, unsigned long long n, unsigned long long *out)
{
  __shared__ unsigned long long best;
  const unsigned long long from = first_from + (unsigned long long) blockIdx.x * step;
  if (threadIdx.x == 0) best = ~0ull;
  __syncthreads ();
  for (unsigned long long base = from & ~15ull; base < n; base += 1024ull * 16ull) {
    const unsigned long long p = base + 16ull * threadIdx.x + 15ull;
    if (p >= from && p < n && seq[p] == (uint8_t) '\n') atomicMin (&best, p);
    __syncthreads ();
    if (best != ~0ull) break;
    __syncthreads ();
  }
  if (threadIdx.x == 0) out[blockIdx.x] = best;
}

extern "C" int tjamd_scan_device (tjamd_counter *c, const void *d_stream, size_t n_bytes, int min_tract_size)
{
  int rc = check_scan_args (c, min_tract_size);
  if (rc) return rc;
  if (n_bytes == 0) return TJAMD_OK;
  if (!d_stream || ((uintptr_t) d_stream & 15u)) return set_err (TJAMD_ERR_ARG, "device stream pointer must be non-null and 16-byte aligned");
  HIPCHK (hipSetDevice (c->device));
  const size_t piece_target = c->piece_target, piece_max = piece_target + piece_target / 2;
  if (n_bytes <= piece_max) return scan_device_piece (c, d_stream, n_bytes, min_tract_size, true, true);
  const uint8_t *seq = (const uint8_t *) d_stream;
  const size_t n_cuts = (n_bytes - 1) / piece_target;
  std::vector<unsigned long long> cuts (n_cuts);
  rc = ensure (c->prefix, 64 + 8 * n_cuts, c->stream);
  if (rc) return rc;
  hipLaunchKernelGGL (find_cut_kernel, dim3 ((unsigned) n_cuts), dim3 (1024), 0, c->stream, seq, (unsigned long long) piece_target, (unsigned long long) piece_target,
                      (unsigned long long) n_bytes, (unsigned long long *) c->prefix.p);
  HIPCHK (hipMemcpyAsync (cuts.data (), c->prefix.p, 8 * n_cuts, hipMemcpyDeviceToHost, c->stream));
  HIPCHK (hipStreamSynchronize (c->stream));
  size_t off = 0, next_cut = 0;
  bool first = true;
  while (off < n_bytes) {
    size_t end = n_bytes;
    if (n_bytes - off > piece_max) {
      while (next_cut < n_cuts && (cuts[next_cut] == ~0ull || cuts[next_cut] + 1 < off + piece_target / 2)) next_cut++;
      if (next_cut < n_cuts && cuts[next_cut] + 1 < n_bytes) end = (size_t) cuts[next_cut] + 1;
    }
    rc = scan_device_piece (c, seq + off, end - off, min_tract_size, first, end == n_bytes);
    if (rc) return rc;
    if (end < n_bytes && (rc = sync_counters (c))) return rc;
    off = end;
    first = false;
  }
  return TJAMD_OK;
}

extern "C" int tjamd_scan_host (tjamd_counter *c, const void *h_stream, size_t n_bytes, int min_tract_size)
{
  if (!c) return set_err (TJAMD_ERR_ARG, "null counter");
  if (n_bytes == 0) return TJAMD_OK;
  if (!h_stream) return set_err (TJAMD_ERR_ARG, "null host stream");
  HIPCHK (hipSetDevice (c->device));
  int rc = ensure (c->stage, (n_bytes + 255) & ~(size_t) 255, c->stream);
  if (rc) return rc;
  HIPCHK (hipMemcpyAsync (c->stage.p, h_stream, n_bytes, hipMemcpyHostToDevice, c->stream));
  return tjamd_scan_device (c, c->stage.p, n_bytes, min_tract_size);
}

extern "C" long tjamd_scan_host_located (tjamd_counter *c, const void *h_stream, size_t n_bytes, int min_tract_size,
                                          tjamd_located_record *out, long capacity)
{
  int rc = (min_tract_size == 0 && c) ? TJAMD_OK : check_scan_args (c, min_tract_size);
  if (rc) return -rc;
  if (n_bytes == 0) return 0;
  if (hipSetDevice (c->device) != hipSuccess) return -set_err (TJAMD_ERR_HIP, "hipSetDevice failed");
  const int mprime = min_tract_size == 0 ? 0 : std::max (min_tract_size, 2);
  const long bound = (long) (n_bytes / (size_t) (mprime ? mprime : 1)) + 1;
  rc = ensure (c->stage, (n_bytes + 255) & ~(size_t) 255, c->stream);
  if (!rc) rc = ensure (c->loc, (size_t) bound * 32, c->stream);
  if (!rc) rc = ensure (c->fix, (size_t) TJ_FIX_CAP * sizeof (FixEntry), c->stream);
  if (rc) return -rc;
  if (hipMemcpyAsync (c->stage.p, h_stream, n_bytes, hipMemcpyHostToDevice, c->stream) != hipSuccess ||
      hipMemsetAsync (c->d_lctr, 0, sizeof (DevCounters), c->stream) != hipSuccess) return -set_err (TJAMD_ERR_HIP, "copy to device failed");
  const long n_tiles = (long) ((n_bytes + 4095) / 4096);
  hipLaunchKernelGGL (scan_list_kernel, dim3 ((unsigned) std::min<long> (n_tiles, 2048)), dim3 (256), 0, c->stream, (const uint8_t *) c->stage.p, (long) n_bytes,
                      n_tiles, c->k, mprime, (u64 *) c->loc.p, (u64) bound, c->d_lctr, (FixEntry *) c->fix.p, (u32) TJ_FIX_CAP, 0);
  hipLaunchKernelGGL (nrun_fixup_list_kernel, dim3 (64), dim3 (256), 0, c->stream, (const uint8_t *) c->stage.p, (long) n_bytes, c->k, mprime,
                      (u64 *) c->loc.p, (u64) bound, c->d_lctr, (const FixEntry *) c->fix.p, (u32) TJ_FIX_CAP, 0);
  if (hipGetLastError () != hipSuccess) return -set_err (TJAMD_ERR_HIP, "located scan launch failed");
  if (hipMemcpyAsync (c->h_ctr, c->d_lctr, sizeof (DevCounters), hipMemcpyDeviceToHost, c->stream) != hipSuccess ||
      hipStreamSynchronize (c->stream) != hipSuccess) return -set_err (TJAMD_ERR_HIP, "located scan failed: %s", hipGetErrorString (hipGetLastError ()));
  const DevCounters h = *c->h_ctr;
  if (h.overflow || h.fix_overflow) return -set_err (TJAMD_ERR_CAPACITY, "located scan overflow");
  c->n_undefined += (long) h.n_undefined;
  const long n = (long) h.n_rec;
  if (n > capacity) return -set_err (TJAMD_ERR_CAPACITY, "located scan produced %ld records, caller capacity %ld", n, capacity);
  if (n) {
    if (hipMemcpy (out, c->loc.p, (size_t) n * 32, hipMemcpyDeviceToHost) != hipSuccess) return -set_err (TJAMD_ERR_HIP, "download failed");
    std::sort (out, out + n, [] (const tjamd_located_record &a, const tjamd_located_record &b) { return a.pos < b.pos; });
  }
  return n;
}

extern "C" long tjamd_raw_count (tjamd_counter *c)
{
  if (!c) return -set_err (TJAMD_ERR_ARG, "null counter");
  if (hipSetDevice (c->device) != hipSuccess) return -set_err (TJAMD_ERR_HIP, "hipSetDevice failed");
  int rc = sync_counters (c);
  return rc ? -rc : c->n_raw_known;
}

extern "C" long tjamd_debug_bucket_counts (tjamd_counter *c, unsigned *out, int n)
{
  if (tjamd_raw_count (c) < 0) return -1;
  for (int b = 0; b < n && b < TJ_P; b++) out[b] = c->h_cursors[b];
  return TJ_P;
}

extern "C" long tjamd_debug_slow_tiles (tjamd_counter *c)
{
  if (tjamd_raw_count (c) < 0) return -1;
  return (long) c->h_ctr->lc[(c->scan_seq - 1u) & 1u].n_slow;
}

extern "C" long tjamd_undefined_runs (tjamd_counter *c)
{
  if (tjamd_raw_count (c) < 0) return -1;
  return c->n_undefined;
}

extern "C" long tjamd_download_raw (tjamd_counter *c, tjamd_record *out, long capacity)
{
  long n = tjamd_raw_count (c);
  if (n < 0) return n;
  if (n > capacity) return -set_err (TJAMD_ERR_CAPACITY, "%ld raw records, caller capacity %ld", n, capacity);
  if (n == 0) return 0;
  int rc = ensure (c->prefix, 64, c->stream);
  if (!rc) rc = ensure (c->rawlist, (size_t) n * 24, c->stream);
  if (rc) return -rc;
  if (hipMemsetAsync (c->prefix.p, 0, 8, c->stream) != hipSuccess) return -set_err (TJAMD_ERR_HIP, "memset failed");
  const Buckets BK = make_buckets (c);
  switch (c->W) {
    case 1: hipLaunchKernelGGL (unpack_buckets_kernel<1>, dim3 (TJ_P), dim3 (256), 0, c->stream, BK, c->k, (u64 *) c->rawlist.p, (u64) n, (u64 *) c->prefix.p); break;
    case 2: hipLaunchKernelGGL (unpack_buckets_kernel<2>, dim3 (TJ_P), dim3 (256), 0, c->stream, BK, c->k, (u64 *) c->rawlist.p, (u64) n, (u64 *) c->prefix.p); break;
    default: hipLaunchKernelGGL (unpack_buckets_kernel<4>, dim3 (TJ_P), dim3 (256), 0, c->stream, BK, c->k, (u64 *) c->rawlist.p, (u64) n, (u64 *) c->prefix.p); break;
  }
  u64 n_out = 0;
  if (hipGetLastError () != hipSuccess || hipStreamSynchronize (c->stream) != hipSuccess ||
      hipMemcpy (&n_out, c->prefix.p, 8, hipMemcpyDeviceToHost) != hipSuccess ||
      hipMemcpy (out, c->rawlist.p, (size_t) n * 24, hipMemcpyDeviceToHost) != hipSuccess) return -set_err (TJAMD_ERR_HIP, "raw download failed");
  if ((long) n_out != n) return -set_err (TJAMD_ERR_STATE, "raw download found %llu records, cursors say %ld", (unsigned long long) n_out, n);
  return n;
}

extern "C" int tjamd_upload_raw (tjamd_counter *c, const hopo_element *elems, long n)
{
  if (!c || (n && !elems) || n < 0) return set_err (TJAMD_ERR_ARG, "bad arguments");
  if (n == 0) return TJAMD_OK;
  HIPCHK (hipSetDevice (c->device));
  int rc = sync_counters (c);
  if (!rc) rc = ensure_buckets (c, (u64) n, 0);
  c->raw_bound += (u64) n;
  if (!rc) rc = ensure (c->stage, (size_t) n * 40, c->stream);
  if (rc) return rc;
  HIPCHK (hipMemcpyAsync (c->stage.p, elems, (size_t) n * 40, hipMemcpyHostToDevice, c->stream));
  const unsigned grid = (unsigned) std::min<long> ((n + 255) / 256, 2048);
  const Buckets BK = make_buckets (c);
  switch (c->W) {
    case 1: hipLaunchKernelGGL (bin_elems_kernel<1>, dim3 (grid), dim3 (256), 0, c->stream, (const u64 *) c->stage.p, n, c->k, BK, c->d_ctr); break;
    case 2: hipLaunchKernelGGL (bin_elems_kernel<2>, dim3 (grid), dim3 (256), 0, c->stream, (const u64 *) c->stage.p, n, c->k, BK, c->d_ctr); break;
    default: hipLaunchKernelGGL (bin_elems_kernel<4>, dim3 (grid), dim3 (256), 0, c->stream, (const u64 *) c->stage.p, n, c->k, BK, c->d_ctr); break;
  }
  HIPCHK (hipGetLastError ());
  c->status = -1;
  return sync_counters (c);
}


static int exclusive_scan (tjamd_counter *c, const u32 *in, u32 *out, long n, u32 *total_out, u32 *tmp, size_t tmp_words)
{
  if (n <= 0) return TJAMD_OK;
  long nblk = (n + SC_ITEMS - 1) / SC_ITEMS;
  if (nblk == 1) {
    hipLaunchKernelGGL (scan_apply_kernel, dim3 (1), dim3 (256), 0, c->stream, in, out, n, (const u32 *) nullptr, total_out);
    HIPCHK (hipGetLastError ());
    return TJAMD_OK;
  }
  if ((size_t) nblk > tmp_words) return set_err (TJAMD_ERR_STATE, "scan scratch too small");
  hipLaunchKernelGGL (scan_reduce_kernel, dim3 ((unsigned) nblk), dim3 (256), 0, c->stream, in, n, tmp);
  HIPCHK (hipGetLastError ());
  int rc = exclusive_scan (c, tmp, tmp, nblk, nullptr, tmp + nblk, tmp_words - (size_t) nblk);
  if (rc) return rc;
  hipLaunchKernelGGL (scan_apply_kernel, dim3 ((unsigned) nblk), dim3 (256), 0, c->stream, in, out, n, (const u32 *) tmp, total_out);
  HIPCHK (hipGetLastError ());
  return TJAMD_OK;
}

static size_t scan_tmp_words (long n)
{
  size_t w = 8;
  while (n > SC_ITEMS) { n = (n + SC_ITEMS - 1) / SC_ITEMS; w += (size_t) n; }
  return w;
}

static int radix_sort_records (tjamd_counter *c, u64 *&a, u64 *&b, long n)
{
  const int passes = key_passes (c->k);
  const int nblk = (int) ((n + RS_ITEMS - 1) / RS_ITEMS);
  const long nh = 256l * nblk;
  int rc = ensure (c->hist, (size_t) nh * 4, c->stream);
  if (!rc) rc = ensure (c->scan_tmp, std::max (scan_tmp_words (nh), scan_tmp_words (n)) * 4, c->stream);
  if (rc) return rc;
  for (int p = 0; p < passes; p++) {
    hipLaunchKernelGGL (radix_count_kernel, dim3 (nblk), dim3 (256), 0, c->stream, (const u64 *) a, n, p, c->k, (u32 *) c->hist.p, nblk);
    HIPCHK (hipGetLastError ());
    rc = exclusive_scan (c, (const u32 *) c->hist.p, (u32 *) c->hist.p, nh, nullptr, (u32 *) c->scan_tmp.p, c->scan_tmp.cap / 4);
    if (rc) return rc;
    hipLaunchKernelGGL (radix_scatter_kernel, dim3 (nblk), dim3 (256), 0, c->stream, (const u64 *) a, b, n, p, c->k, (const u32 *) c->hist.p, nblk);
    HIPCHK (hipGetLastError ());
    std::swap (a, b);
  }
  return TJAMD_OK;
}

static unsigned grid_for (long n) { return (unsigned) std::max<long> (1, std::min<long> ((n + 255) / 256, 4096)); }



static int finalise_radix (tjamd_counter *c, long n1, int min_coverage)
{
  int rc = ensure (c->alt, (size_t) n1 * 24, c->stream);
  if (!rc) rc = ensure (c->flags, (size_t) n1 * 4, c->stream);
  if (!rc) rc = ensure (c->segid, (size_t) n1 * 4, c->stream);
  if (!rc) rc = ensure (c->headpos, (size_t) n1 * 4, c->stream);
  if (!rc) rc = ensure (c->keep, (size_t) n1 * 4, c->stream);
  if (!rc) rc = ensure (c->outpos, (size_t) n1 * 4, c->stream);
  if (!rc) rc = ensure (c->scan_tmp, scan_tmp_words (n1) * 4, c->stream);
  if (rc) return rc;
  u64 *a = (u64 *) c->kept.p, *b = (u64 *) c->alt.p;
  rc = radix_sort_records (c, a, b, n1);
  if (rc) return rc;
  if (a != (u64 *) c->kept.p) std::swap (c->kept, c->alt);

  const u64 *kept = (const u64 *) c->kept.p;
  u32 *flags = (u32 *) c->flags.p, *segid = (u32 *) c->segid.p, *headpos = (u32 *) c->headpos.p;
  u32 *keep = (u32 *) c->keep.p, *outpos = (u32 *) c->outpos.p;
  hipLaunchKernelGGL (seg_heads_kernel, dim3 (grid_for (n1)), dim3 (256), 0, c->stream, kept, n1, flags, 1);
  HIPCHK (hipGetLastError ());
  rc = exclusive_scan (c, flags, segid, n1, &c->d_fin->n_ctx, (u32 *) c->scan_tmp.p, c->scan_tmp.cap / 4);
  if (rc) return rc;
  hipLaunchKernelGGL (seg_headpos_kernel, dim3 (grid_for (n1)), dim3 (256), 0, c->stream, (const u32 *) flags, (const u32 *) segid, n1, headpos);
  HIPCHK (hipGetLastError ());
  hipLaunchKernelGGL (ctx_decide_kernel, dim3 (grid_for (n1)), dim3 (256), 0, c->stream, kept, n1, (const u32 *) headpos,
                      (const u32 *) &c->d_fin->n_ctx, min_coverage, keep);
  HIPCHK (hipGetLastError ());
  HIPCHK (hipMemcpyAsync (c->h_fin, c->d_fin, sizeof (FinCounts), hipMemcpyDeviceToHost, c->stream));
  HIPCHK (hipStreamSynchronize (c->stream));
  const long n_ctx = c->h_fin->n_ctx;
  rc = exclusive_scan (c, keep, outpos, n_ctx, &c->d_fin->n_idx, (u32 *) c->scan_tmp.p, c->scan_tmp.cap / 4);
  if (!rc) rc = ensure (c->idx_i, (size_t) n_ctx * 4, c->stream);
  if (!rc) rc = ensure (c->idx_f, (size_t) n_ctx * 4, c->stream);
  if (rc) return rc;
  hipLaunchKernelGGL (ctx_write_kernel, dim3 (grid_for (n_ctx)), dim3 (256), 0, c->stream, n1, (const u32 *) headpos, (const u32 *) &c->d_fin->n_ctx,
                      (const u32 *) keep, (const u32 *) outpos, (int *) c->idx_i.p, (int *) c->idx_f.p);
  HIPCHK (hipGetLastError ());

  const int log2t = cov_table_bits (n1);
  const long t = 1l << log2t;
  rc = ensure (c->cov, (size_t) t * 8, c->stream);
  if (rc) return rc;
  u64 *ctab = (u64 *) c->cov.p;
  HIPCHK (hipMemsetAsync (c->cov.p, 0, (size_t) t * 8, c->stream));
  hipLaunchKernelGGL (set_int_kernel, dim3 (1), dim3 (1), 0, c->stream, &c->d_fin->coverage, INT_MIN);
  hipLaunchKernelGGL (cov_insert_kernel, dim3 (grid_for (2 * n1)), dim3 (256), 0, c->stream, kept, n1, ctab, log2t);
  HIPCHK (hipGetLastError ());
  hipLaunchKernelGGL (cov_max_kernel, dim3 (std::min<unsigned> (grid_for (t), 256u)), dim3 (256), 0, c->stream, (const u64 *) ctab, t, &c->d_fin->coverage);
  HIPCHK (hipGetLastError ());
  HIPCHK (c->timer[T_FIN].end (c->stream));
  c->timer[T_FIN].timed = true;
  HIPCHK (hipMemcpyAsync (c->h_fin, c->d_fin, sizeof (FinCounts), hipMemcpyDeviceToHost, c->stream));
  HIPCHK (hipStreamSynchronize (c->stream));
  return TJAMD_OK;
}

static int finalise_binned (tjamd_counter *c, long n1, int min_coverage, long cap = 0, bool wait = true)
{
  const bool planned = n1 == 0;
  const bool aside = planned && !wait && c->order_stream != nullptr && c->order_stream != c->stream;
  const hipStream_t st = aside ? c->order_stream : c->stream;
  const FinPlan *plan = planned ? &c->d_state->plan : nullptr;
  if (planned) n1 = cap;
  const int nbits = bin_bits_for (n1, c->k);
  const int nbins = planned ? BS_MAXBINS : 1 << nbits;
  int cov_direct = 0;
  const int log2t = planned ? cov_table_bits (n1) : cov_plan_bits (n1, c->k, &cov_direct);
  const long t = 1l << log2t;
  const bool fused = planned && c->bins_counted;
  c->bins_counted = false;
  int rc = ensure (c->alt, (size_t) n1 * 24, c->stream);
  if (!rc && !c->bins.p) { rc = ensure (c->bins, (size_t) (BS_MAXBINS + 1) * 4, c->stream); c->bins_zeroed = false; }
  if (!rc) rc = ensure (c->binstart, (size_t) (nbins + 1) * 4, c->stream);
  if (!rc) rc = ensure (c->binctx, (size_t) nbins * 8, c->stream);
  if (!rc) rc = ensure (c->headpos, (size_t) n1 * 4, c->stream);
  if (!rc) rc = ensure (c->outpos, (size_t) n1 * 4, c->stream);
  if (!rc) rc = ensure (c->idx_i, (size_t) n1 * 4, c->stream);
  if (!rc) rc = ensure (c->idx_f, (size_t) n1 * 4, c->stream);
  if (!rc) rc = ensure (c->cov, (size_t) t * 8, c->stream);
  if (rc) return rc;
  u32 *bins = (u32 *) c->bins.p, *binstart = (u32 *) c->binstart.p, *binctx = (u32 *) c->binctx.p, *binout = binctx + nbins;
  u32 *tstart = (u32 *) c->headpos.p, *tend = (u32 *) c->outpos.p;
  u64 *ctab = (u64 *) c->cov.p;
  if (!fused && !c->bins_zeroed) HIPCHK (hipMemsetAsync (bins, 0, (size_t) BS_MAXBINS * 4, c->stream));
  c->bins_zeroed = false;
  if (aside) { HIPCHK (hipEventRecord (c->ev_agg, c->stream)); HIPCHK (hipStreamWaitEvent (st, c->ev_agg, 0)); }
  const unsigned g1 = planned ? std::min<unsigned> (grid_for (n1), 2048u) : grid_for (n1);
  if (!fused) hipLaunchKernelGGL (bin_count_kernel, dim3 (g1), dim3 (256), 0, st, (const u64 *) c->kept.p, n1, c->k, nbits, bins,
                                  (uint4 *) c->cov.p, (long) (t / 2), 0, plan);
  hipLaunchKernelGGL (bin_scan_kernel, dim3 (1), dim3 (1024), 0, st, bins, nbins, binstart, c->bin_rank_max, c->d_fin, plan);
  hipLaunchKernelGGL (bin_scatter_kernel, dim3 (g1), dim3 (256), 0, st, (const u64 *) c->kept.p, (u64 *) c->alt.p, n1, c->k, nbits, bins, plan,
                      fused ? (uint4 *) c->cov.p : (uint4 *) nullptr);
  hipLaunchKernelGGL (bin_sort_index_kernel, dim3 ((unsigned) std::min (nbins / BSI_WAVES + 1, 16384)), dim3 (64 * BSI_WAVES), 0, st,
                      (const u64 *) c->alt.p, (u64 *) c->kept.p, (const u32 *) binstart, nbins, (const FinCounts *) c->d_fin, min_coverage,
                      ctab, log2t, binctx, tstart, tend, plan, cov_direct);
  hipLaunchKernelGGL (bin_ctx_scan_kernel, dim3 (1), dim3 (1024), 0, st, (const u32 *) binctx, nbins, binout, c->d_fin, plan);
  hipLaunchKernelGGL (bin_ctx_write_kernel, dim3 (256), dim3 (256), 0, st, (const u32 *) binstart, (const u32 *) binctx, (const u32 *) binout, nbins,
                      (const u32 *) tstart, (const u32 *) tend, (int *) c->idx_i.p, (int *) c->idx_f.p, (const u64 *) ctab, t, c->d_fin, plan);
  HIPCHK (hipGetLastError ());
  HIPCHK (c->timer[T_FIN].end (st));
  c->timer[T_FIN].timed = true;
  if (planned) HIPCHK (hipMemcpyAsync (c->h_state, c->d_state, sizeof (DevState), hipMemcpyDeviceToHost, st));
  else HIPCHK (hipMemcpyAsync (c->h_fin, c->d_fin, sizeof (FinCounts), hipMemcpyDeviceToHost, c->stream));
  if (wait) HIPCHK (hipStreamSynchronize (c->stream));
  else HIPCHK (hipEventRecord (c->ev_done, st));
  return TJAMD_OK;
}

static int finalise_impl (tjamd_counter *c, int remove_biased, int min_coverage, int *status, int phase);

extern "C" int tjamd_finalise (tjamd_counter *c, int remove_biased, int min_coverage, int *status)
{
  int rc = finalise_impl (c, remove_biased, min_coverage, status, 0);
  return rc;
}
extern "C" int tjamd_finalise_begin (tjamd_counter *c, int remove_biased, int min_coverage)
{
  const int rc = finalise_impl (c, remove_biased, min_coverage, nullptr, 1);
  if (!rc && c->fin_pending == 0) c->fin_pending = 3;
  return rc;
}
extern "C" int tjamd_finalise_end (tjamd_counter *c, int *status)
{
  if (!c) return set_err (TJAMD_ERR_ARG, "null counter");
  if (!c->fin_pending) return set_err (TJAMD_ERR_STATE, "tjamd_finalise_end without tjamd_finalise_begin");
  if (c->fin_pending == 3) { c->fin_pending = 0; if (status) *status = c->status; return TJAMD_OK; }
  return finalise_impl (c, c->fin_rb, c->fin_mc, status, 2);
}

static int finalise_impl (tjamd_counter *c, int remove_biased, int min_coverage, int *status, int phase)
{
  if (!c) return set_err (TJAMD_ERR_ARG, "null counter");
  HIPCHK (hipSetDevice (c->device));
  bool speculative = c->fin_speculative, plan_ahead = c->fin_plan_ahead;
  u64 kept_cap = c->fin_kept_cap;
  int rc = TJAMD_OK;
  if (phase == 2) goto second_half;
  c->fin_pending = 0;
  {
  c->n_kept = 0; c->n_idx = 0; c->coverage = 0; c->timer[T_FIN].timed = false;
  speculative = (c->raw_bound / 2 + 1) * 24 <= (8ull << 30);
  kept_cap = c->raw_bound / 2 + 1;
  if (!speculative) {
    rc = sync_counters (c);
    if (rc) return rc;
    if (c->n_raw_known == 0) { c->status = 1; if (status) *status = 1; return TJAMD_OK; }
    if (c->n_raw_known >= (1l << 31)) return set_err (TJAMD_ERR_CAPACITY, "%ld raw records exceed the reference's int n_elem", c->n_raw_known);
    kept_cap = (u64) c->n_raw_known / 2 + 1;
  }

  rc = ensure (c->kept, (size_t) kept_cap * 24, c->stream);
  if (!rc) rc = ensure (c->ovf, c->pool.cap, c->stream);
  if (rc) return rc;
  HIPCHK (c->timer[T_FIN].begin (c->stream));
  const Buckets BK = make_buckets (c);
  long plan_cap = (long) std::min<u64> (kept_cap, std::max<u64> (kept_cap / 8, 1u << 16));
  if (const char *pc = getenv ("TATAJUBA_AMD_PLAN_CAP")) plan_cap = std::max (1l, std::min (plan_cap, atol (pc)));
  plan_ahead = speculative && getenv ("TATAJUBA_AMD_NO_PLAN") == nullptr;
  FinPlan *const d_plan = plan_ahead ? &c->d_state->plan : nullptr;
  u32 *fine = nullptr;
  if (plan_ahead && getenv ("TATAJUBA_AMD_NO_FUSED_BINS") == nullptr) {
    const bool fresh = c->fine.p == nullptr;
    rc = ensure (c->fine, (size_t) BS_MAXBINS * 4, c->stream);
    if (rc) return rc;
    if (fresh || c->fine_dirty) HIPCHK (hipMemsetAsync (c->fine.p, 0, (size_t) BS_MAXBINS * 4, c->stream));
    if (!c->bins.p) { rc = ensure (c->bins, (size_t) (BS_MAXBINS + 1) * 4, c->stream); c->bins_zeroed = false; if (rc) return rc; }
    fine = (u32 *) c->fine.p;
    c->fine_dirty = true;
  }
  const int fbits = fine_bin_bits (c->k);
  switch (c->W) {
    case 1: hipLaunchKernelGGL (aggregate1_kernel, dim3 (TJ_P), dim3 (AG_BLOCK), 0, c->stream, BK, (u64 *) c->ovf.p, c->k, remove_biased, (u64 *) c->kept.p, kept_cap, c->d_fin, plan_cap, d_plan, fine, fbits); break;
    case 2: hipLaunchKernelGGL (aggregate2_kernel, dim3 (TJ_P), dim3 (AG_BLOCK), 0, c->stream, BK, (u64 *) c->ovf.p, c->k, remove_biased, (u64 *) c->kept.p, kept_cap, c->d_fin, plan_cap, d_plan, fine, fbits); break;
    default: hipLaunchKernelGGL (aggregate4_kernel, dim3 (TJ_P), dim3 (AG_BLOCK), 0, c->stream, BK, (u64 *) c->ovf.p, c->k, remove_biased, (u64 *) c->kept.p, kept_cap, c->d_fin, plan_cap, d_plan, fine, fbits); break;
  }
  HIPCHK (hipGetLastError ());
  rc = plan_ahead ? TJAMD_OK : queue_counter_copies (c);
  if (!rc) rc = clear_buckets (c, plan_ahead);
  if (rc) return rc;
  c->fin_rb = remove_biased; c->fin_mc = min_coverage; c->fin_speculative = speculative; c->fin_plan_ahead = plan_ahead; c->fin_kept_cap = kept_cap;
  if (plan_ahead) { rc = finalise_binned (c, 0, min_coverage, plan_cap, phase != 1); if (rc) return rc; }
  else HIPCHK (hipStreamSynchronize (c->stream));
  }
  if (phase == 1) { c->fin_pending = plan_ahead ? 1 : 2; return TJAMD_OK; }
second_half:
  if (phase == 2) {
    if (c->fin_pending == 1) HIPCHK (hipEventSynchronize (c->ev_done));
    c->fin_pending = 0;
  }
  if (speculative) {
    rc = apply_counter_copies (c, plan_ahead);
    const long n = c->n_raw_known;
    c->n_raw_known = 0; c->raw_bound = 0; c->bucket_bound = 0; c->chunk_bound = TJ_P;
    if (rc) return rc;
    if (n == 0) { c->status = 1; if (status) *status = 1; return TJAMD_OK; }
    if (n >= (1l << 31)) return set_err (TJAMD_ERR_CAPACITY, "%ld raw records exceed the reference's int n_elem", n);
  }
  if (plan_ahead) {
    FinPlan &pl = c->h_state->plan;
    if (pl.n1 != pl.n1_exact || pl.kept_overflow != pl.ovf_exact) {
      c->plan_mismatches++;
      pl.n1 = pl.n1_exact; pl.kept_overflow = pl.ovf_exact; pl.ok = 0;
    }
  }
  if (plan_ahead ? c->h_state->plan.kept_overflow : c->h_fin->overflow) return set_err (TJAMD_ERR_CAPACITY, "kept list overflow");
  const long n1 = plan_ahead ? c->h_state->plan.n1 : (long) c->h_fin->n_kept;
  if (n1 == 0) {
    HIPCHK (c->timer[T_FIN].end (c->stream)); c->timer[T_FIN].timed = true;
    c->status = 2; if (status) *status = 2; return TJAMD_OK;
  }

  c->n_kept = n1;
  if (!(plan_ahead && c->h_state->plan.ok)) rc = finalise_binned (c, n1, min_coverage);
  if (!rc && c->h_fin->sort_fallback) rc = finalise_radix (c, n1, min_coverage);
  if (rc) return rc;
  c->n_idx = (int) c->h_fin->n_idx;
  if (c->n_idx == 0) { c->status = 3; if (status) *status = 3; return TJAMD_OK; }
  c->coverage = c->h_fin->coverage;
  c->status = 0;
  if (status) *status = 0;
  return TJAMD_OK;
}

extern "C" long tjamd_kept_count (tjamd_counter *c) { return c ? c->n_kept : -1; }
extern "C" int tjamd_n_idx (tjamd_counter *c) { return c ? c->n_idx : -1; }
extern "C" int tjamd_coverage (tjamd_counter *c) { return c ? c->coverage : -1; }
extern "C" const void *tjamd_kept_device_ptr (tjamd_counter *c) { return c ? c->kept.p : NULL; }

extern "C" long tjamd_download_kept (tjamd_counter *c, hopo_element *out, long capacity)
{
  if (!c) return -set_err (TJAMD_ERR_ARG, "null counter");
  if (c->status < 0) return -set_err (TJAMD_ERR_STATE, "counter not finalised");
  const long n1 = c->n_kept;
  if (n1 > capacity) return -set_err (TJAMD_ERR_CAPACITY, "%ld kept records, caller capacity %ld", n1, capacity);
  if (n1 == 0) return 0;
  if (hipSetDevice (c->device) != hipSuccess) return -set_err (TJAMD_ERR_HIP, "hipSetDevice failed");
  if ((size_t) n1 * 24 > c->h_kept_cap) {
    if (c->h_kept) (void) hipHostFree (c->h_kept);
    c->h_kept = nullptr; c->h_kept_cap = 0;
    const size_t want = (size_t) n1 * 24 + ((size_t) n1 * 24 >> 2) + 4096;
    if (hipHostMalloc (&c->h_kept, want, hipHostMallocDefault) != hipSuccess) { c->h_kept = nullptr; return -set_err (TJAMD_ERR_HIP, "hipHostMalloc of %zu bytes failed", want); }
    c->h_kept_cap = want;
  }
  const tjamd_record *tmp = (const tjamd_record *) c->h_kept;
  if (hipMemcpyAsync (c->h_kept, c->kept.p, (size_t) n1 * 24, hipMemcpyDeviceToHost, c->stream) != hipSuccess ||
      hipStreamSynchronize (c->stream) != hipSuccess) return -set_err (TJAMD_ERR_HIP, "download failed");
  for (long i = 0; i < n1; i++) {
    out[i].context[0] = tmp[i].ctx0; out[i].context[1] = tmp[i].ctx1;
    memcpy ((char *) &out[i] + 16, &tmp[i].meta, 8);
    out[i].read_offset = -1;
    out[i].loc_ref_id = out[i].loc_pos = out[i].loc_last = -1;
  }
  return n1;
}

extern "C" long tjamd_download_idx (tjamd_counter *c, int *idx_initial, int *idx_final, long capacity)
{
  if (!c) return -set_err (TJAMD_ERR_ARG, "null counter");
  if (c->status < 0) return -set_err (TJAMD_ERR_STATE, "counter not finalised");
  const long n = c->n_idx;
  if (n > capacity) return -set_err (TJAMD_ERR_CAPACITY, "%ld index ranges, caller capacity %ld", n, capacity);
  if (n == 0) return 0;
  if (hipSetDevice (c->device) != hipSuccess) return -set_err (TJAMD_ERR_HIP, "hipSetDevice failed");
  if (hipMemcpy (idx_initial, c->idx_i.p, (size_t) n * 4, hipMemcpyDeviceToHost) != hipSuccess ||
      hipMemcpy (idx_final, c->idx_f.p, (size_t) n * 4, hipMemcpyDeviceToHost) != hipSuccess) return -set_err (TJAMD_ERR_HIP, "download failed");
  return n;
}

extern "C" double tjamd_last_scan_ms (tjamd_counter *c)
{
  float ms = 0.f;
  if (!c || !c->timer[T_SCAN].elapsed (c->device, ms)) return -1.0;
  for (int i = 0; i < c->n_piece_ev; i++) { float p = 0.f; if (hipEventElapsedTime (&p, c->ev_pa[i], c->ev_pb[i]) == hipSuccess) ms -= p; }
  return (double) ms;
}

extern "C" double tjamd_last_merge_ms (tjamd_counter *c) { return c ? c->timer[T_MERGE].ms (c->device) : -1.0; }

extern "C" int tjamd_counter_uses_log (const tjamd_counter *c) { return (c && c->W <= c->log_mode && c->fast_mode) ? 1 : 0; }

extern "C" double tjamd_last_partition_ms (tjamd_counter *c)
{
  if (!c || !c->timer[T_SCAN].timed) return -1.0;
  if (!c->part_timed) return 0.0;
  float ms = 0.f;
  if (hipSetDevice (c->device) != hipSuccess || hipEventSynchronize (c->ev_p1) != hipSuccess || hipEventElapsedTime (&ms, c->timer[T_SCAN].e1, c->ev_p1) != hipSuccess) return -1.0;
  for (int i = 0; i < c->n_piece_ev; i++) { float p = 0.f; if (hipEventElapsedTime (&p, c->ev_pa[i], c->ev_pb[i]) == hipSuccess) ms += p; }
  return (double) ms;
}

extern "C" double tjamd_last_finalise_ms (tjamd_counter *c) { return c ? c->timer[T_FIN].ms (c->device) : -1.0; }

extern "C" long tjamd_last_scan_launches (tjamd_counter *c) { return c ? c->last_scan_launches : -1; }
extern "C" long tjamd_plan_mismatches (tjamd_counter *c) { return c ? c->plan_mismatches : -1; }

static long merge_samples_radix (tjamd_counter *c, const void *d_records, long n, int n_samples, void *d_out_keys, void *d_out_counts, long capacity);


__device__ __forceinline__ int flank_hamming (u64 a, u64 b)
{
  const u64 d = a ^ b;
  return __popcll ((d | (d >> 1)) & 0x5555555555555555ull);
}

__global__ void group_back_kernel (const u64 *__restrict__ kept, long n, int maxd, int *__restrict__ back)
{
  for (long i = blockIdx.x * (long) blockDim.x + threadIdx.x; i < n; i += (long) gridDim.x * blockDim.x) {
    const u64 c0 = kept[3 * i], c1 = kept[3 * i + 1], base = kept[3 * i + 2] & 3ull;
    long j = i - 1;
    while (j >= 0 && (kept[3 * j + 2] & 3ull) == base && flank_hamming (kept[3 * j], c0) + flank_hamming (kept[3 * j + 1], c1) < maxd) j--;
    back[i] = (int) j;
  }
}

__global__ void group_resolve_kernel (const int *__restrict__ back, long n, u32 *__restrict__ head)
{
  for (long i = blockIdx.x * (long) blockDim.x + threadIdx.x; i < n; i += (long) gridDim.x * blockDim.x) {
    if (back[i] != (int) i - 1) continue;
    head[i] = 1u;
    long start = i;
    for (long j = i + 1; j < n && back[j] != (int) j - 1; j++) {
      if (start > (long) back[j]) head[j] = 0u;
      else { head[j] = 1u; start = j; }
    }
  }
}

struct GroupOut { int first, n_elem, n_context, mode; long long integral; };

__global__ void group_summary_kernel (const u64 *__restrict__ kept, long n, const u32 *__restrict__ head, const u32 *__restrict__ gid_excl,
                                      int *__restrict__ group_of, GroupOut *__restrict__ groups)
{
  for (long i = blockIdx.x * (long) blockDim.x + threadIdx.x; i < n; i += (long) gridDim.x * blockDim.x) {
    if (!head[i]) continue;
    const int g = (int) gid_excl[i];
    GroupOut o = {(int) i, 0, 0, (int) i, 0};
    int mode_count = 0;
    for (long j = i; j < n && (j == i || !head[j]); j++) {
      const u64 m = kept[3 * j + 2];
      const int cnt = meta_count (m);
      if (j == i || kept[3 * j] != kept[3 * (j - 1)] || kept[3 * j + 1] != kept[3 * (j - 1) + 1]) o.n_context++;
      if (j == i || mode_count < cnt) { mode_count = cnt; o.mode = (int) j; }
      o.integral += cnt; o.n_elem++;
      group_of[j] = g;
    }
    groups[g] = o;
  }
}


__device__ __forceinline__ u32 name_symbol (u64 c0, u64 c1, u32 base, int k, int t)
{
  if (t < k) return (u32) (c0 >> (2 * t)) & 3u;
  if (t == k + 1) return base;
  if (t < k + 3) return 4u;
  return (u32) (c1 >> (2 * (t - k - 3))) & 3u;
}

__device__ int name_edit_distance (const u64 *__restrict__ kept, long a, long b, int k, int free_end)
{
  const u64 a0 = kept[3 * a], a1 = kept[3 * a + 1], b0 = kept[3 * b], b1 = kept[3 * b + 1];
  const u32 ab = (u32) (kept[3 * a + 2] & 3ull), bb = (u32) (kept[3 * b + 2] & 3ull);
  const int n = 2 * k + 3;
  unsigned char row[2 * 32 + 4];
  for (int y = 0; y <= n; y++) row[y] = (unsigned char) y;
  int early = n;
  for (int x = 1; x <= n; x++) {
// ... 2271 lines not shown
```

Before: 11.37 billion.

## Write kept records into per-fine-bin slabs during aggregation, skipping bin scatter

During aggregation, each kept record's fine-bin atomicAdd now returns a rank, and the record is also written into a fixed-capacity slab for that fine bin. Bin sort then gathers records straight from the slabs through an LDS index list, so the separate bin_scatter pass over all kept records is no longer launched. The coverage-table clear moves into extra blocks of bin_scan, and a copy of the fine counts is saved when bins are reduced. In exchange the code adds a larger alt buffer, an extra record write per kept record, and indirect gathers in the sort. If any slab overflows it falls back to the normal binned path.

```diff
diff --git a/tatajuba_amd/csrc/hopo_device.hip b/tatajuba_amd/csrc/hopo_device.hip
--- a/tatajuba_amd/csrc/hopo_device.hip
+++ b/tatajuba_amd/csrc/hopo_device.hip
@@ -89,8 +89,8 @@
 
 struct FixEntry { long long pos; long long len; };
 
-struct FinCounts { u32 n_seg, n_kept, n_ctx, n_idx; int coverage; u32 overflow, sort_fallback, pad; };
-struct FinPlan { long n1; long t; int nbits, nbins, log2t, ok; u32 kept_overflow, cov_direct; long n1_exact; u32 ovf_exact, pad2; };
+struct FinCounts { u32 n_seg, n_kept, n_ctx, n_idx; int coverage; u32 overflow, sort_fallback, pad; u32 slab_overflow; };
+struct FinPlan { long n1; long t; int nbits, nbins, log2t, ok; u32 kept_overflow, cov_direct; long n1_exact; u32 ovf_exact, slab_ovf; };
 
 
 
@@ -1788,7 +1788,8 @@
 }
 
 __global__ void clear_buckets_kernel (u32 *cursors, DevCounters *ctr, u32 *table, u32 maxj, int ch_shift, FinCounts *fin, u32 *bins, int nbins,
-                                      DevCounters *snap_ctr, u32 *snap_cursors, FinPlan *plan, u32 *__restrict__ fine = nullptr, int fine_bits = 0)
+                                      DevCounters *snap_ctr, u32 *snap_cursors, FinPlan *plan, u32 *__restrict__ fine = nullptr, int fine_bits = 0,
+                                      u32 *__restrict__ fine_copy = nullptr)
 {
   const u32 b = blockIdx.x;
   if (snap_ctr) {
@@ -1796,7 +1797,7 @@
       snap_cursors[b] = cursors[b * TJ_CSTRIDE];
       if (b == 0) {
         snap_cursors[TJ_P] = cursors[TJ_P * TJ_CSTRIDE];
-        if (plan) { plan->n1_exact = (long) fin->n_kept; plan->ovf_exact = fin->overflow; }
+        if (plan) { plan->n1_exact = (long) fin->n_kept; plan->ovf_exact = fin->overflow; plan->slab_ovf = fin->slab_overflow; }
       }
     }
     if (b == 0) for (u32 i = threadIdx.x; i < sizeof (DevCounters) / 4; i += blockDim.x) reinterpret_cast<u32 *> (snap_ctr)[i] = reinterpret_cast<const u32 *> (ctr)[i];
@@ -1816,11 +1817,12 @@
         u32 sum = 0;
         if (shift >= 2) {
           uint4 *f4 = reinterpret_cast<uint4 *> (fine) + (size_t) i * (run >> 2);
-          for (int j = 0; j < (run >> 2); j++) { const uint4 v = f4[j]; sum += v.x + v.y + v.z + v.w; }
+          uint4 *c4 = reinterpret_cast<uint4 *> (fine_copy) + (size_t) i * (run >> 2);
+          for (int j = 0; j < (run >> 2); j++) { const uint4 v = f4[j]; sum += v.x + v.y + v.z + v.w; if (fine_copy) c4[j] = v; }
           for (int j = 0; j < (run >> 2); j++) f4[j] = make_uint4 (0, 0, 0, 0);
         }
         else {
-          for (int j = 0; j < run; j++) sum += fine[(i << shift) + j];
+          for (int j = 0; j < run; j++) { const u32 v = fine[(i << shift) + j]; sum += v; if (fine_copy) fine_copy[(i << shift) + j] = v; }
           for (int j = 0; j < run; j++) fine[(i << shift) + j] = 0;
         }
         bins[i] = sum;
@@ -1830,7 +1832,7 @@
   }
   else if (bins) for (int i = (int) (b * blockDim.x + threadIdx.x); i < nbins; i += (int) (gridDim.x * blockDim.x)) bins[i] = 0;
   __syncthreads ();
-  if (threadIdx.x == 0) { cursors[b * TJ_CSTRIDE] = 0; if (b == 0) { cursors[TJ_P * TJ_CSTRIDE] = TJ_P; fin->n_kept = 0; fin->overflow = 0; fin->pad = 0; } }
+  if (threadIdx.x == 0) { cursors[b * TJ_CSTRIDE] = 0; if (b == 0) { cursors[TJ_P * TJ_CSTRIDE] = TJ_P; fin->n_kept = 0; fin->overflow = 0; fin->pad = 0; fin->slab_overflow = 0; } }
 }
 
 __global__ void table_relayout_kernel (const u32 *__restrict__ old, u32 old_maxj, u32 *__restrict__ neu, u32 new_maxj)
@@ -1849,6 +1851,7 @@
 #define AG1_MARK     (~0ull)
 
 #define BS_MAXBITS   16
+#define TJ_SLAB_MIN  16u
 __host__ __device__ static inline int cov_table_bits (long n1) { int b = 10; while ((1l << b) < 4 * n1 && b < 31) b++; return b; }
 __host__ __device__ static inline int cov_plan_bits (long n1, int k, int *direct)
 {
@@ -1868,6 +1871,24 @@
 {
   u32 old = atomicOr (&fin->overflow, 1u);
   asm volatile ("" :: "v"(old));
+}
+
+__device__ __forceinline__ u32 emit_count (u64 c0, u64 c1, u64 meta, int k, u32 *__restrict__ fine, int fine_bits, u32 &bin)
+{
+  bin = bin_of_record (c0, c1, meta, k, fine_bits);
+  return atomicAdd (&fine[bin], 1u);
+}
+template <int N>
+__device__ __forceinline__ void emit_ranks_arrived (u32 (&rank)[N])
+{
+  asm volatile ("s_waitcnt vmcnt(0)" ::: "memory");
+#pragma unroll
+  for (int i = 0; i < N; i++) asm volatile ("" : "+v"(rank[i]));
+}
+__device__ __forceinline__ void emit_slab (u64 c0, u64 c1, u64 meta, u32 bin, u32 rank, u64 *__restrict__ slab, u32 slab_cap, FinCounts *fin)
+{
+  if (rank < slab_cap) { u64 *q = slab + 3 * ((u64) bin * slab_cap + rank); q[0] = c0; q[1] = c1; q[2] = meta; }
+  else { u32 old = atomicOr (&fin->slab_overflow, 1u); asm volatile ("" :: "v"(old)); }
 }
 
 __device__ __forceinline__ void plan_tail (FinCounts *fin, int k, long cap, FinPlan *plan)
@@ -1907,7 +1928,7 @@
 
 __global__ __launch_bounds__ (AG_BLOCK)
 void aggregate1_kernel (Buckets BK, u64 *ovf, int k, int remove_biased, u64 *__restrict__ kept, u64 kept_cap, FinCounts *fin,
-                        long plan_cap, FinPlan *plan, u32 *__restrict__ fine, int fine_bits)
+                        long plan_cap, FinPlan *plan, u32 *__restrict__ fine, int fine_bits, u64 *__restrict__ slab, u32 slab_cap)
 {
   __shared__ Agg1Lds L;
   const int tid = threadIdx.x, lane = tid & 63, wave = tid >> 6;
@@ -2070,17 +2091,29 @@
     if (tid == 0) L.total = total ? atomicAdd (&fin->n_kept, total) : 0u;
     __syncthreads ();
     u64 at = (u64) L.total + wbase + x - mine;
-#pragma unroll
-    for (int r = 0; r < AG1_S / AG_BLOCK; r++)
+    u32 ebin[AG1_S / AG_BLOCK], erank[AG1_S / AG_BLOCK];
+#pragma unroll
+    for (int r = 0; r < AG1_S / AG_BLOCK; r++) {
+      ebin[r] = ~0u; erank[r] = 0;
       if (metas[r]) {
         const u64 key = L.key[tid + r * AG_BLOCK];
         if (at < kept_cap) {
           u64 *q = kept + 3 * at; q[0] = (key >> 32) & 0xFFFFFFull; q[1] = key & 0xFFFFFFull; q[2] = metas[r];
-          if (fine) atomicAdd (&fine[bin_of_record ((key >> 32) & 0xFFFFFFull, key & 0xFFFFFFull, metas[r], k, fine_bits)], 1u);
+          if (fine) erank[r] = emit_count ((key >> 32) & 0xFFFFFFull, key & 0xFFFFFFull, metas[r], k, fine, fine_bits, ebin[r]);
         }
         else flag_kept_overflow (fin);
         at++;
       }
+    }
+    if (slab) {
+      emit_ranks_arrived (erank);
+#pragma unroll
+      for (int r = 0; r < AG1_S / AG_BLOCK; r++)
+        if (ebin[r] != ~0u) {
+          const u64 key = L.key[tid + r * AG_BLOCK];
+          emit_slab ((key >> 32) & 0xFFFFFFull, key & 0xFFFFFFull, metas[r], ebin[r], erank[r], slab, slab_cap, fin);
+        }
+    }
     __threadfence_block ();
     __syncthreads ();
     n = L.n_ovf;
@@ -2110,7 +2143,7 @@
 
 __global__ __launch_bounds__ (AG_BLOCK)
 void aggregate2_kernel (Buckets BK, u64 *ovf, int k, int remove_biased, u64 *__restrict__ kept, u64 kept_cap, FinCounts *fin,
-                        long plan_cap, FinPlan *plan, u32 *__restrict__ fine, int fine_bits)
+                        long plan_cap, FinPlan *plan, u32 *__restrict__ fine, int fine_bits, u64 *__restrict__ slab, u32 slab_cap)
 {
   __shared__ Agg2Lds L;
   const int tid = threadIdx.x, lane = tid & 63, wave = tid >> 6;
@@ -2296,17 +2329,29 @@
     if (tid == 0) L.total = total ? atomicAdd (&fin->n_kept, total) : 0u;
     __syncthreads ();
     u64 at = (u64) L.total + wbase + x - mine;
-#pragma unroll
-    for (int r = 0; r < AG2_S / AG_BLOCK; r++)
+    u32 ebin[AG2_S / AG_BLOCK], erank[AG2_S / AG_BLOCK];
+#pragma unroll
+    for (int r = 0; r < AG2_S / AG_BLOCK; r++) {
+      ebin[r] = ~0u; erank[r] = 0;
       if (metas[r]) {
         const int slot = tid + r * AG_BLOCK;
         if (at < kept_cap) {
           u64 *q = kept + 3 * at; q[0] = (L.kk[slot].x >> 7) & m56; q[1] = L.kk[slot].y & m56; q[2] = metas[r];
-          if (fine) atomicAdd (&fine[bin_of_record ((L.kk[slot].x >> 7) & m56, L.kk[slot].y & m56, metas[r], k, fine_bits)], 1u);
+          if (fine) erank[r] = emit_count ((L.kk[slot].x >> 7) & m56, L.kk[slot].y & m56, metas[r], k, fine, fine_bits, ebin[r]);
         }
         else flag_kept_overflow (fin);
         at++;
       }
+    }
+    if (slab) {
+      emit_ranks_arrived (erank);
+#pragma unroll
+      for (int r = 0; r < AG2_S / AG_BLOCK; r++)
+        if (ebin[r] != ~0u) {
+          const int slot = tid + r * AG_BLOCK;
+          emit_slab ((L.kk[slot].x >> 7) & m56, L.kk[slot].y & m56, metas[r], ebin[r], erank[r], slab, slab_cap, fin);
+        }
+    }
     __threadfence_block ();
     __syncthreads ();
     n = L.n_ovf;
@@ -2334,7 +2379,7 @@
 
 __global__ __launch_bounds__ (AG_BLOCK)
 void aggregate4_kernel (Buckets BK, u64 *ovf, int k, int remove_biased, u64 *__restrict__ kept, u64 kept_cap, FinCounts *fin,
-                        long plan_cap, FinPlan *plan, u32 *__restrict__ fine, int fine_bits)
+                        long plan_cap, FinPlan *plan, u32 *__restrict__ fine, int fine_bits, u64 *__restrict__ slab, u32 slab_cap)
 {
   __shared__ Agg4Lds L;
   const int tid = threadIdx.x, lane = tid & 63, wave = tid >> 6;
@@ -2469,17 +2514,29 @@
     if (tid == 0) L.total = total ? atomicAdd (&fin->n_kept, total) : 0u;
     __syncthreads ();
     u64 at = (u64) L.total + wbase + x - mine;
-#pragma unroll
-    for (int r = 0; r < AG4_S / AG_BLOCK; r++)
+    u32 ebin[AG4_S / AG_BLOCK], erank[AG4_S / AG_BLOCK];
+#pragma unroll
+    for (int r = 0; r < AG4_S / AG_BLOCK; r++) {
+      ebin[r] = ~0u; erank[r] = 0;
       if (metas[r]) {
         const int slot = tid + r * AG_BLOCK;
         if (at < kept_cap) {
           u64 *q = kept + 3 * at; q[0] = L.c0[slot]; q[1] = L.c1[slot]; q[2] = metas[r];
-          if (fine) atomicAdd (&fine[bin_of_record (L.c0[slot], L.c1[slot], metas[r], k, fine_bits)], 1u);
+          if (fine) erank[r] = emit_count (L.c0[slot], L.c1[slot], metas[r], k, fine, fine_bits, ebin[r]);
         }
         else flag_kept_overflow (fin);
         at++;
       }
+    }
+    if (slab) {
+      emit_ranks_arrived (erank);
+#pragma unroll
+      for (int r = 0; r < AG4_S / AG_BLOCK; r++)
+        if (ebin[r] != ~0u) {
+          const int slot = tid + r * AG_BLOCK;
+          emit_slab (L.c0[slot], L.c1[slot], metas[r], ebin[r], erank[r], slab, slab_cap, fin);
+        }
+    }
     __threadfence_block ();
     __syncthreads ();
     n = L.n_ovf;
@@ -2675,11 +2732,16 @@
 }
 
 __global__ __launch_bounds__ (1024)
-void bin_scan_kernel (u32 *__restrict__ bins, int nbins, u32 *__restrict__ binstart, u32 rank_max, FinCounts *fin, const FinPlan *__restrict__ plan = nullptr)
+void bin_scan_kernel (u32 *__restrict__ bins, int nbins, u32 *__restrict__ binstart, u32 rank_max, FinCounts *fin, const FinPlan *__restrict__ plan = nullptr,
+                      uint4 *__restrict__ cov = nullptr)
 {
   __shared__ WgScanLds L;
   u32 vmax;
   if (plan) { if (!plan->ok) return; nbins = plan->nbins; }
+  if (blockIdx.x > 0) {
+    if (cov) for (long i = (long) (blockIdx.x - 1u) * 1024 + threadIdx.x; i < plan->t / 2; i += (long) (gridDim.x - 1u) * 1024) cov[i] = make_uint4 (0, 0, 0, 0);
+    return;
+  }
   const u32 total = wg_exclusive_scan (bins, nbins, binstart, bins, L, vmax);
   if (threadIdx.x == 0) { binstart[nbins] = total; fin->sort_fallback = vmax > rank_max ? 1u : 0u; }
 }
@@ -2911,30 +2973,51 @@
   else { const auto r = __builtin_amdgcn_permlane32_swap (v, v, false, false); return (lane & 32) ? r[0] : r[1]; }
 }
 
+template <bool SLAB>
 __global__ __launch_bounds__ (64 * BSI_WAVES)
 void bin_sort_index_kernel (const u64 *__restrict__ in, u64 *__restrict__ out, const u32 *__restrict__ binstart, int nbins, const FinCounts *fin,
                             int min_coverage, u64 *__restrict__ cov_tab, int log2t,
                             u32 *__restrict__ binctx, u32 *__restrict__ tstart, u32 *__restrict__ tend, const FinPlan *__restrict__ plan = nullptr,
-                            int cov_direct = 0)
+                            int cov_direct = 0, const u32 *__restrict__ fine_cnt = nullptr, int fine_bits = 0, u32 slab_cap = 0)
 {
   __shared__ alignas (16) u32 hd[BSI_WAVES][BS_RANK_MAX];
   __shared__ u32 sz[BSI_WAVES][BS_RANK_MAX];
+  __shared__ alignas (16) u32 src[SLAB ? BSI_WAVES : 1][SLAB ? BS_RANK_MAX : 4];
   const int lane = threadIdx.x & 63, wave = threadIdx.x >> 6;
   const int bin0 = (int) blockIdx.x * BSI_WAVES + wave;
   u32 st0 = 0, en0 = 0;
   if (bin0 < nbins) { st0 = binstart[bin0]; en0 = binstart[bin0 + 1]; }
   if (plan) { if (!plan->ok) return; nbins = plan->nbins; log2t = plan->log2t; cov_direct = (int) plan->cov_direct; }
   if (fin->sort_fallback) return;
-  u32 *H = hd[wave], *E = sz[wave];
+  if (SLAB && plan->slab_ovf) return;
+  u32 *H = hd[wave], *E = sz[wave], *S = src[SLAB ? wave : 0];
+  const int fshift = SLAB ? fine_bits - plan->nbits : 0;
   for (int bin = bin0; bin < nbins; bin += gridDim.x * BSI_WAVES) {
-    const u32 st = (bin == bin0) ? st0 : binstart[bin], s = ((bin == bin0) ? en0 : binstart[bin + 1]) - st;
+    const u32 st = (bin == bin0) ? st0 : binstart[bin];
+    u32 s = ((bin == bin0) ? en0 : binstart[bin + 1]) - st;
     if (s == 0) { if (lane == 0) binctx[bin] = 0; continue; }
     const u64 *R = in + 3 * (u64) st;
+    if constexpr (SLAB) {
+      const u32 f0 = (u32) bin << fshift, run = 1u << fshift;
+      u32 carry = 0;
+      for (u32 j0 = 0; j0 < run; j0 += 64) {
+        const u32 f = f0 + j0 + (u32) lane;
+        const u32 cn = (j0 + (u32) lane < run) ? min (fine_cnt[f], slab_cap) : 0u;
+        const u32 incl = wave_inclusive_scan (cn);
+        const u32 o = carry + incl - cn;
+        for (u32 r = 0; r < cn && o + r < (u32) BS_RANK_MAX; r++) S[o + r] = f * slab_cap + r;
+        carry += (u32) __builtin_amdgcn_readlane ((int) incl, 63);
+      }
+      asm volatile ("s_waitcnt lgkmcnt(0)" ::: "memory");
+      __builtin_amdgcn_wave_barrier ();
+      s = min (s, carry);
+    }
+    auto rec = [&] (u32 t) { return SLAB ? in + 3 * (u64) S[t] : R + 3 * t; };
     u32 nkeep = 0;
     if (s <= 64u) {
       const bool valid = (u32) lane < s;
       u64 a0 = 0, a1 = 0, am = 0;
-      if (valid) { a0 = R[3 * lane]; a1 = R[3 * lane + 1]; am = R[3 * lane + 2]; }
+      if (valid) { const u64 *p = rec ((u32) lane); a0 = p[0]; a1 = p[1]; am = p[2]; }
       const int w = meta_count (am);
       u64 cas_a = 0, cas_b = 0;
       if (!cov_direct && valid) cov_add2_issue ((u32) (a0 & 0x7FFFFFFFull), (u32) (a1 & 0x7FFFFFFFull), w, cov_tab, log2t, cas_a, cas_b);
@@ -2999,7 +3082,8 @@
       const u32 t = t0 + lane;
       bool keep = false;
       if (t < s) {
-        const u64 a0 = R[3 * t], a1 = R[3 * t + 1], am = R[3 * t + 2];
+        const u64 *pa = rec (t);
+        const u64 a0 = pa[0], a1 = pa[1], am = pa[2];
         u32 rank = 0, ctx_before = 0, ctx_size = 0;
         int depth = 0;
         const u32 abase = (u32) am & 1u, alen = ((u32) (am >> TJ_META_LEN_SHIFT) & 0x3FFu) ^ 0x200u;
@@ -3008,7 +3092,8 @@
 #pragma unroll
           for (int i = 0; i < 4; i++) {
             const u32 jj = (j0 + (u32) i < s) ? j0 + (u32) i : s - 1u;
-            b0[i] = R[3 * jj]; b1[i] = R[3 * jj + 1]; bm[i] = R[3 * jj + 2];
+            const u64 *pb = SLAB ? in + 3 * (u64) (u32) __builtin_amdgcn_readfirstlane ((int) S[jj]) : R + 3 * jj;
+            b0[i] = pb[0]; b1[i] = pb[1]; bm[i] = pb[2];
           }
 #pragma unroll
           for (int i = 0; i < 4; i++) {
@@ -3065,7 +3150,7 @@
 {
   __shared__ WgScanLds L;
   u32 vmax;
-  if (plan) { if (!plan->ok) return; nbins = plan->nbins; }
+  if (plan) { if (!plan->ok || plan->slab_ovf) return; nbins = plan->nbins; }
   const u32 total = wg_exclusive_scan (binctx, nbins, binout, nullptr, L, vmax);
   if (threadIdx.x == 0 && !fin->sort_fallback) { fin->n_idx = total; fin->coverage = INT_MIN; }
 }
@@ -3076,7 +3161,7 @@
                            const u64 *__restrict__ cov_tab, long t, FinCounts *fin, const FinPlan *__restrict__ plan = nullptr)
 {
   __shared__ int s_best[4];
-  if (plan) { if (!plan->ok) return; nbins = plan->nbins; t = plan->t; }
+  if (plan) { if (!plan->ok || plan->slab_ovf) return; nbins = plan->nbins; t = plan->t; }
   if (fin->sort_fallback) return;
   const int lane = threadIdx.x & 63, wave = threadIdx.x >> 6;
   for (int bin = blockIdx.x * 4 + wave; bin < nbins; bin += gridDim.x * 4) {
@@ -3346,6 +3431,10 @@
   unsigned scan_seq = 0;
   size_t piece_target = TJ_SCAN_PIECE_TARGET;
   int scan_grid_cap = 0;
+  int slab_cap_env = 0;
+  u32 fin_slab_cap = 0;
+  long slab_runs = 0, slab_fallbacks = 0;
+  long radix_runs = 0;
   bool buckets_clean = false;
   long plan_mismatches = 0;
   bool ctr_clean = false;
@@ -3394,6 +3483,8 @@
   if (fm && atoi (fm) >= 0 && atoi (fm) <= 2) c->fast_mode = atoi (fm);
   const char *sg = getenv ("TATAJUBA_AMD_SCAN_GRID");
   if (sg && atoi (sg) >= 1) c->scan_grid_cap = atoi (sg);
+  const char *sc = getenv ("TATAJUBA_AMD_SLAB_CAP");
+  if (sc && atoi (sc) >= 1) c->slab_cap_env = atoi (sc);
   const char *sl = getenv ("TATAJUBA_AMD_BUCKET_SLACK");
   if (sl && atof (sl) >= 1.0) c->slack = atof (sl);
   HIPCHK_NULL (hipStreamCreateWithFlags (&c->own_stream, hipStreamNonBlocking));
@@ -3476,7 +3567,8 @@
     hipLaunchKernelGGL (clear_buckets_kernel, dim3 (TJ_P), dim3 (256), 0, c->stream, c->d_cursors, c->d_ctr,
                         (u32 *) (c->maxj ? c->table.p : nullptr), c->maxj, c->ch_shift, c->d_fin, (u32 *) c->bins.p, c->bins.p ? BS_MAXBINS : 0,
                         snapshot ? &c->d_state->snap_ctr : (DevCounters *) nullptr, snapshot ? c->d_state->snap_cursors : (u32 *) nullptr,
-                        snapshot ? &c->d_state->plan : (FinPlan *) nullptr, fused ? (u32 *) c->fine.p : (u32 *) nullptr, fine_bin_bits (c->k));
+                        snapshot ? &c->d_state->plan : (FinPlan *) nullptr, fused ? (u32 *) c->fine.p : (u32 *) nullptr, fine_bin_bits (c->k),
+                        fused && c->fin_slab_cap ? (u32 *) c->fine.p + BS_MAXBINS : (u32 *) nullptr);
     HIPCHK (hipGetLastError ());
     c->buckets_clean = true;
     c->ctr_clean = true;
@@ -3887,6 +3979,24 @@
   return (long) c->h_ctr->lc[(c->scan_seq - 1u) & 1u].n_slow;
 }
 
+extern "C" int tjamd_debug_slab_stats (tjamd_counter *c, long out[4])
+{
+  if (!c || !out) return set_err (TJAMD_ERR_ARG, "null argument");
+  out[0] = (long) c->fin_slab_cap; out[1] = c->slab_runs; out[2] = c->slab_fallbacks; out[3] = c->radix_runs;
+  return TJAMD_OK;
+}
+
+extern "C" long tjamd_debug_fine_counts (tjamd_counter *c, unsigned *out, long n)
+{
+  if (!c || !out) return -set_err (TJAMD_ERR_ARG, "null argument");
+  if (hipSetDevice (c->device) != hipSuccess) return -set_err (TJAMD_ERR_HIP, "hipSetDevice failed");
+  if (!c->fine.p) return 0;
+  const long nf = 1l << fine_bin_bits (c->k);
+  if (hipStreamSynchronize (c->stream) != hipSuccess) return -set_err (TJAMD_ERR_HIP, "hipStreamSynchronize failed");
+  if (hipMemcpy (out, c->fine.p, (size_t) std::min (n, nf) * 4, hipMemcpyDeviceToHost) != hipSuccess) return -set_err (TJAMD_ERR_HIP, "hipMemcpy failed");
+  return nf;
+}
+
 extern "C" long tjamd_undefined_runs (tjamd_counter *c)
 {
   if (tjamd_raw_count (c) < 0) return -1;
@@ -4061,6 +4171,7 @@
   const long t = 1l << log2t;
   const bool fused = planned && c->bins_counted;
   c->bins_counted = false;
+  const bool slabs = fused && c->fin_slab_cap > 0;
   int rc = ensure (c->alt, (size_t) n1 * 24, c->stream);
   if (!rc && !c->bins.p) { rc = ensure (c->bins, (size_t) (BS_MAXBINS + 1) * 4, c->stream); c->bins_zeroed = false; }
   if (!rc) rc = ensure (c->binstart, (size_t) (nbins + 1) * 4, c->stream);
@@ -4080,12 +4191,17 @@
   const unsigned g1 = planned ? std::min<unsigned> (grid_for (n1), 2048u) : grid_for (n1);
   if (!fused) hipLaunchKernelGGL (bin_count_kernel, dim3 (g1), dim3 (256), 0, st, (const u64 *) c->kept.p, n1, c->k, nbits, bins,
                                   (uint4 *) c->cov.p, (long) (t / 2), 0, plan);
-  hipLaunchKernelGGL (bin_scan_kernel, dim3 (1), dim3 (1024), 0, st, bins, nbins, binstart, c->bin_rank_max, c->d_fin, plan);
-  hipLaunchKernelGGL (bin_scatter_kernel, dim3 (g1), dim3 (256), 0, st, (const u64 *) c->kept.p, (u64 *) c->alt.p, n1, c->k, nbits, bins, plan,
-                      fused ? (uint4 *) c->cov.p : (uint4 *) nullptr);
-  hipLaunchKernelGGL (bin_sort_index_kernel, dim3 ((unsigned) std::min (nbins / BSI_WAVES + 1, 16384)), dim3 (64 * BSI_WAVES), 0, st,
-                      (const u64 *) c->alt.p, (u64 *) c->kept.p, (const u32 *) binstart, nbins, (const FinCounts *) c->d_fin, min_coverage,
-                      ctab, log2t, binctx, tstart, tend, plan, cov_direct);
+  hipLaunchKernelGGL (bin_scan_kernel, dim3 (slabs ? 256 : 1), dim3 (1024), 0, st, bins, nbins, binstart, c->bin_rank_max, c->d_fin, plan,
+                      slabs ? (uint4 *) c->cov.p : (uint4 *) nullptr);
+  if (!slabs) hipLaunchKernelGGL (bin_scatter_kernel, dim3 (g1), dim3 (256), 0, st, (const u64 *) c->kept.p, (u64 *) c->alt.p, n1, c->k, nbits, bins, plan,
+                                  fused ? (uint4 *) c->cov.p : (uint4 *) nullptr);
+  const dim3 gs ((unsigned) std::min (nbins / BSI_WAVES + 1, 16384));
+  if (slabs) hipLaunchKernelGGL (bin_sort_index_kernel<true>, gs, dim3 (64 * BSI_WAVES), 0, st,
+                                 (const u64 *) c->alt.p, (u64 *) c->kept.p, (const u32 *) binstart, nbins, (const FinCounts *) c->d_fin, min_coverage,
+                                 ctab, log2t, binctx, tstart, tend, plan, cov_direct, (const u32 *) c->fine.p + BS_MAXBINS, fine_bin_bits (c->k), c->fin_slab_cap);
+  else hipLaunchKernelGGL (bin_sort_index_kernel<false>, gs, dim3 (64 * BSI_WAVES), 0, st,
+                           (const u64 *) c->alt.p, (u64 *) c->kept.p, (const u32 *) binstart, nbins, (const FinCounts *) c->d_fin, min_coverage,
+                           ctab, log2t, binctx, tstart, tend, plan, cov_direct, (const u32 *) nullptr, 0, 0u);
   hipLaunchKernelGGL (bin_ctx_scan_kernel, dim3 (1), dim3 (1024), 0, st, (const u32 *) binctx, nbins, binout, c->d_fin, plan);
   hipLaunchKernelGGL (bin_ctx_write_kernel, dim3 (256), dim3 (256), 0, st, (const u32 *) binstart, (const u32 *) binctx, (const u32 *) binout, nbins,
                       (const u32 *) tstart, (const u32 *) tend, (int *) c->idx_i.p, (int *) c->idx_f.p, (const u64 *) ctab, t, c->d_fin, plan);
@@ -4153,7 +4269,7 @@
   u32 *fine = nullptr;
   if (plan_ahead && getenv ("TATAJUBA_AMD_NO_FUSED_BINS") == nullptr) {
     const bool fresh = c->fine.p == nullptr;
-    rc = ensure (c->fine, (size_t) BS_MAXBINS * 4, c->stream);
+    rc = ensure (c->fine, (size_t) 2 * BS_MAXBINS * 4, c->stream);
     if (rc) return rc;
     if (fresh || c->fine_dirty) HIPCHK (hipMemsetAsync (c->fine.p, 0, (size_t) BS_MAXBINS * 4, c->stream));
     if (!c->bins.p) { rc = ensure (c->bins, (size_t) (BS_MAXBINS + 1) * 4, c->stream); c->bins_zeroed = false; if (rc) return rc; }
@@ -4161,10 +4277,20 @@
     c->fine_dirty = true;
   }
   const int fbits = fine_bin_bits (c->k);
+  c->fin_slab_cap = 0;
+  if (fine && getenv ("TATAJUBA_AMD_NO_SLABS") == nullptr) {
+    u64 per = std::max<u64> ((u64) plan_cap >> fbits, TJ_SLAB_MIN);
+    if (c->slab_cap_env >= 1) per = std::min<u64> (per, (u64) c->slab_cap_env);
+    rc = ensure (c->alt, (size_t) std::max<u64> ((u64) plan_cap, per << fbits) * 24, c->stream);
+    if (rc) return rc;
+    c->fin_slab_cap = (u32) per;
+  }
+  u64 *const slab = c->fin_slab_cap ? (u64 *) c->alt.p : nullptr;
+  const u32 slab_cap = c->fin_slab_cap;
   switch (c->W) {
-    case 1: hipLaunchKernelGGL (aggregate1_kernel, dim3 (TJ_P), dim3 (AG_BLOCK), 0, c->stream, BK, (u64 *) c->ovf.p, c->k, remove_biased, (u64 *) c->kept.p, kept_cap, c->d_fin, plan_cap, d_plan, fine, fbits); break;
-    case 2: hipLaunchKernelGGL (aggregate2_kernel, dim3 (TJ_P), dim3 (AG_BLOCK), 0, c->stream, BK, (u64 *) c->ovf.p, c->k, remove_biased, (u64 *) c->kept.p, kept_cap, c->d_fin, plan_cap, d_plan, fine, fbits); break;
-    default: hipLaunchKernelGGL (aggregate4_kernel, dim3 (TJ_P), dim3 (AG_BLOCK), 0, c->stream, BK, (u64 *) c->ovf.p, c->k, remove_biased, (u64 *) c->kept.p, kept_cap, c->d_fin, plan_cap, d_plan, fine, fbits); break;
+    case 1: hipLaunchKernelGGL (aggregate1_kernel, dim3 (TJ_P), dim3 (AG_BLOCK), 0, c->stream, BK, (u64 *) c->ovf.p, c->k, remove_biased, (u64 *) c->kept.p, kept_cap, c->d_fin, plan_cap, d_plan, fine, fbits, slab, slab_cap); break;
+    case 2: hipLaunchKernelGGL (aggregate2_kernel, dim3 (TJ_P), dim3 (AG_BLOCK), 0, c->stream, BK, (u64 *) c->ovf.p, c->k, remove_biased, (u64 *) c->kept.p, kept_cap, c->d_fin, plan_cap, d_plan, fine, fbits, slab, slab_cap); break;
+    default: hipLaunchKernelGGL (aggregate4_kernel, dim3 (TJ_P), dim3 (AG_BLOCK), 0, c->stream, BK, (u64 *) c->ovf.p, c->k, remove_biased, (u64 *) c->kept.p, kept_cap, c->d_fin, plan_cap, d_plan, fine, fbits, slab, slab_cap); break;
   }
   HIPCHK (hipGetLastError ());
   rc = plan_ahead ? TJAMD_OK : queue_counter_copies (c);
@@ -4203,8 +4329,10 @@
   }
 
   c->n_kept = n1;
-  if (!(plan_ahead && c->h_state->plan.ok)) rc = finalise_binned (c, n1, min_coverage);
-  if (!rc && c->h_fin->sort_fallback) rc = finalise_radix (c, n1, min_coverage);
+  const bool slab_failed = plan_ahead && c->fin_slab_cap && c->h_state->plan.slab_ovf;
+  if (plan_ahead && c->fin_slab_cap && c->h_state->plan.ok) { if (slab_failed) c->slab_fallbacks++; else c->slab_runs++; }
+  if (!(plan_ahead && c->h_state->plan.ok && !slab_failed)) rc = finalise_binned (c, n1, min_coverage);
+  if (!rc && c->h_fin->sort_fallback) { c->radix_runs++; rc = finalise_radix (c, n1, min_coverage); }
   if (rc) return rc;
   c->n_idx = (int) c->h_fin->n_idx;
   if (c->n_idx == 0) { c->status = 3; if (status) *status = 3; return TJAMD_OK; }
```

Result: no change. 11.47 billion, median of 5 (+0.9%).
